# bderembl/msom

Measured on AMD Instinct MI355X. Metric: grid-point-updates/s (timesteps/s x N^2 x nl), multi-layer QG RK2 step at 4096x4096x6 per GPU, higher is better.
Workload: dtype f64; 1 GPU; C4: msqg double gyre (Verron 1992 params), 4096x4096x6 fp64, tiles 1x1 of 4096x4096, TOLERANCE 1e-3, RK2 step = 2 inversions + 2 tendencies + 2 advances; mg_nrelax=4

## Files before the change

include/msom.h:

```cpp
#ifndef MSOM_H
#define MSOM_H

#ifdef __cplusplus
extern "C" {
#endif

#define MSOM_OK 0
#define MSOM_ERR_ARG (-1)
#define MSOM_ERR_IO (-2)
#define MSOM_ERR_CONFIG (-3)
#define MSOM_ERR_HIP (-4)
#define MSOM_ERR_COMM (-5)
#define MSOM_ERR_STATE (-6)

#define MSOM_MAXNL 16
#define MSOM_FASTNL 8

enum {
  MSOM_PSI = 0,
  MSOM_Q = 1,
  MSOM_ZETA = 2,
  MSOM_PSIPG = 3,
  MSOM_ZETAPG = 4,
  MSOM_QFORC = 5,
// ... 89 lines not shown
int msom_modes_energy(msom_t *m, double *ke, double *pe);
int msom_modes_set_rd(msom_t *m, int mode);

int msom_modes_mgstats(msom_t *m, int mode, msom_mgstats *st);

int msom_spec_layout(int nx, int ny, int *nbins, long *count);
int msom_spec_bins(msom_t *m);
int msom_spec_kr(msom_t *m, double *kr);
int msom_spec_2d(msom_t *m, const double *a, const double *b, int layers, double *out);
int msom_spec_cross(msom_t *m, const double *a, const double *b, int layers, double *spec, double *flux);
int msom_spec_fields(msom_t *m, int field_a, int field_b, double *spec, double *flux);
int msom_spec_energy(msom_t *m, double *ke, double *pe);

int msom_step(msom_t *m, double *dt_used);
int msom_set_tnext(msom_t *m, double tnext);
double msom_time(msom_t *m);
int msom_iter(msom_t *m);
double msom_ke(msom_t *m);
int msom_last_mgstats(msom_t *m, msom_mgstats *st);
int msom_run(msom_t *m, const char *workdir, long nsteps_max);

int msom_write_bas(msom_t *m, int field, const char *path);
int msom_read_bas(msom_t *m, int field, const char *path);

int msom_write_nc(msom_t *m, const char *path);
int msom_read_nc(msom_t *m, int field, const char *path, const char *varname, int record);

int msom_wavelet_filter(msom_t *m, double dtflt);
int msom_energy_tend(msom_t *m, double dt);
int msom_filter_de(msom_t *m, int pm_field, double dtflt);
int msom_reset_de(msom_t *m);
int pystep_de(msom_t *m, const double *po_py, int len1, int len2, int len3, double *de_bf_py, int len4, int len5, int len6,
              double *de_vd_py, int len7, int len8, int len9, double *de_j1_py, int len10, int len11, int len12,
              double *de_j2_py, int len13, int len14, int len15, double *de_j3_py, int len16, int len17, int len18,
              double *de_ft_py, int len19, int len20, int len21, int onlyKE);

int msom_dbg_wavelet_levels(msom_t *m);
int msom_dbg_siglev(msom_t *m, int level, double *out);
int msom_dbg_wavelet_apply(msom_t *m, int field);

msom_t *msom_create_newqg(const char *params_path);
msom_t *msom_create_newqg_str(const char *params_text);

int msom_set_device(int device);

int msom_comm_unique_id(void *id128);
msom_t *msom_create_tiled(const char *params_text, int px, int py, int rank, const void *id128);
int msom_tile_info(msom_t *m, int *px, int *py, int *ix, int *iy, int *nx_local, int *ny_local);

int msom_dbg_nlevels(msom_t *m);
int msom_dbg_level_dims(msom_t *m, int lev, int *nx, int *ny);
int msom_dbg_relax(msom_t *m, int lev, double *da, const double *res, int nsweeps);
int msom_dbg_residual(msom_t *m, const double *a, const double *b, double *res, double *maxres);
int msom_dbg_helm_relax(msom_t *m, int lev, double *da, const double *res, int nhalf, const int *count_per_mode);
int msom_dbg_helm_residual(msom_t *m, const double *a, const double *b, double *res, double *maxres_per_mode);
int msom_dbg_restrict(msom_t *m, int lev_fine, const double *fine, double *coarse);
int msom_dbg_prolong(msom_t *m, int lev_coarse, const double *coarse, double *fine);
int msom_dbg_op(msom_t *m, const char *op, int f_in, int f_out, double add, double fac);

int msom_profile_read(msom_t *m, const char *kernel, double *avg_ms, long *launches);
int msom_profile_reset(msom_t *m);
int msom_sync(msom_t *m);
int msom_bench_kernel(msom_t *m, const char *kernel, int reps, double *avg_ms);
int msom_dbg_rccl_selftest(void);

enum {
  MSOMN_PSI = 0,
  MSOMN_Q = 1,
  MSOMN_ZETA = 2,
  MSOMN_TMP = 3,
  MSOMN_PSIPG = 4,
  MSOMN_S2 = 5,
  MSOMN_TOPO = 6,
  MSOMN_QFORC = 7,
  MSOMN_MASK = 8,
  MSOMN_DQ = 9,
  MSOMN_QPRED = 10,
  MSOMN_QFORC3D = 11,
  MSOMN_BS = 12,
  MSOMN_S2S = 13,
  MSOMN_PSIF = 14,
  MSOMN_NFIELDS = 15
};
typedef struct msomn msomn_t;

msomn_t *msomn_create(const char *params_path);
msomn_t *msomn_create_str(const char *params_text);
void msomn_destroy(msomn_t *m);
int msomn_set_option(msomn_t *m, const char *key, double value);
double msomn_get_param(msomn_t *m, const char *key);
int msomn_field_layers(msomn_t *m, int field);
int msomn_set_field(msomn_t *m, int field, const double *a);
int msomn_get_field(msomn_t *m, int field, double *a);
int msomn_set_const(msomn_t *m);
int msomn_update(msomn_t *m, int qfield, int dqfield, double dtmax, double *dt_out);
int msomn_advance(msomn_t *m, int out, int in, int dq, double dt);
int msomn_invert_q(msomn_t *m, int qfield, msom_mgstats *stats);
int msomn_comp_q(msomn_t *m, int psifield, int qfield);
int msomn_rhs_pv(msomn_t *m, int qfield, int dqfield);
int msomn_forcing(msomn_t *m);
int msomn_step(msomn_t *m, int with_forcing_event);
int msomn_set_tnext(msomn_t *m, double tnext);
double msomn_time(msomn_t *m);
double msomn_dt(msomn_t *m);
int msomn_iter(msomn_t *m);
int msomn_ke(msomn_t *m, double *ke);
// ... 25 lines not shown
```

msom_amd/api.py:

```python
import ctypes as C
import os

import numpy as np

_HERE = os.path.dirname(os.path.abspath(__file__))
_LIBDIR = os.path.join(_HERE, "lib")

FIELDS = dict(PSI=0, Q=1, ZETA=2, PSIPG=3, ZETAPG=4, QFORC=5, TMP=6, FR=7, S=8, DQ=9, RO=10, TOPO=11,
              QPRED=12, NOISE=13, SIGMA=14, PTR=15, PTR_RELAX=16, DPTR=17, PTR_PRED=18, RD=19, QOF=20,
              DE_BF=21, DE_VD=22, DE_J1=23, DE_J2=24, DE_J3=25, DE_FT=26, TMP2=27, PO_MFT=28,
              BFN_F1=29, BFN_F2=30, BFN_F3=31, BFN_OBS=32, BFN_GAIN=33)

STATS = dict(PSI=0, Q=1, PSI2=2, Q2=3, KE=4, UQ=5, VQ=6, NACC=7, EKE=16, UQ_EDDY=17, VQ_EDDY=18, QME=32)

MODES = dict(IBU=0, RD=1, M2L=2, L2M=3, N=4)


class MsomError(RuntimeError):
    pass


class MGStats(C.Structure):
    _fields_ = [("i", C.c_int), ("resb", C.c_double), ("resa", C.c_double), ("sum", C.c_double), ("nrelax", C.c_int)]

# ... 31 lines not shown
        "msom_remove_mean": (ci, [vp, ci]),
        "msom_set_const": (ci, [vp]),
        "msom_read_inputs": (ci, [vp, cs]),
        "msom_update": (cd, [vp, vp, vp, cd]),
        "msom_advance": (ci, [vp, vp, vp, vp, cd]),
        "msom_invertq": (ci, [vp, vp, vp, C.POINTER(MGStats)]),
        "msom_comp_q": (ci, [vp, vp, vp]),
        "pystep_bfn": (ci, [vp, vp, ci, ci, ci, vp, ci, ci, ci, cd, ci]),
        "pyq2p": (ci, [vp, vp, ci, ci, ci, vp, ci, ci, ci]),
        "pyp2q": (ci, [vp, vp, ci, ci, ci, vp, ci, ci, ci]),
        "msom_bfn_begin": (ci, [vp]),
        "msom_bfn_steps": (ci, [vp, ci, cd, cd, cd]),
        "msom_bfn_misfit": (ci, [vp, _dp]),
        "msom_stats_begin": (ci, [vp, C.c_uint]),
        "msom_stats_accumulate": (ci, [vp, cd]),
        "msom_stats_weight": (ci, [vp, _dp]),
        "msom_stats_get": (ci, [vp, ci, vp]),
        "msom_time_filter": (ci, [vp, cd]),
        "msom_modes_compute": (ci, [vp]),
        "msom_modes_layers": (ci, [vp, ci]),
        "msom_modes_get": (ci, [vp, ci, vp]),
        "msom_modes_project": (ci, [vp, ci, vp, vp]),
        "msom_modes_energy": (ci, [vp, _dp, _dp]),
        "msom_modes_set_rd": (ci, [vp, ci]),
        "msom_modes_mgstats": (ci, [vp, ci, C.POINTER(MGStats)]),
        "msom_spec_layout": (ci, [ci, ci, C.POINTER(ci), C.POINTER(C.c_long)]),
        "msom_spec_bins": (ci, [vp]),
        "msom_spec_kr": (ci, [vp, _dp]),
        "msom_spec_2d": (ci, [vp, vp, vp, ci, vp]),
        "msom_spec_cross": (ci, [vp, vp, vp, ci, _dp, _dp]),
        "msom_spec_fields": (ci, [vp, ci, ci, _dp, _dp]),
        "msom_spec_energy": (ci, [vp, _dp, _dp]),
        "msom_dbg_helm_relax": (ci, [vp, ci, vp, vp, ci, C.POINTER(ci)]),
        "msom_dbg_helm_residual": (ci, [vp, vp, vp, vp, _dp]),
        "msom_step": (ci, [vp, _dp]),
        "msom_set_tnext": (ci, [vp, cd]),
        "msom_time": (cd, [vp]),
        "msom_iter": (ci, [vp]),
        "msom_ke": (cd, [vp]),
        "msom_last_mgstats": (ci, [vp, C.POINTER(MGStats)]),
        "msom_run": (ci, [vp, cs, C.c_long]),
        "msom_write_bas": (ci, [vp, ci, cs]),
        "msom_read_bas": (ci, [vp, ci, cs]),
        "msom_write_nc": (ci, [vp, cs]),
        "msom_read_nc": (ci, [vp, ci, cs, cs, ci]),
        "msom_set_device": (ci, [ci]),
        "msom_comm_unique_id": (ci, [vp]),
        "msom_create_tiled": (vp, [cs, ci, ci, ci, vp]),
        "msom_tile_info": (ci, [vp] + [C.POINTER(ci)] * 6),
        "msom_dbg_nlevels": (ci, [vp]),
        "msom_dbg_level_dims": (ci, [vp, ci, C.POINTER(ci), C.POINTER(ci)]),
        "msom_dbg_relax": (ci, [vp, ci, vp, vp, ci]),
        "msom_dbg_residual": (ci, [vp, vp, vp, vp, _dp]),
        "msom_dbg_restrict": (ci, [vp, ci, vp, vp]),
        "msom_dbg_prolong": (ci, [vp, ci, vp, vp]),
        "msom_dbg_op": (ci, [vp, cs, ci, ci, cd, cd]),
        "msom_profile_read": (ci, [vp, cs, _dp, C.POINTER(C.c_long)]),
        "msom_profile_reset": (ci, [vp]),
        "msom_sync": (ci, [vp]),
        "msom_bench_kernel": (ci, [vp, cs, ci, _dp]),
        "msom_dbg_rccl_selftest": (ci, []),
        "msom_wavelet_filter": (ci, [vp, cd]),
        "msom_energy_tend": (ci, [vp, cd]),
        "msom_filter_de": (ci, [vp, ci, cd]),
        "msom_reset_de": (ci, [vp]),
        "pystep_de": (ci, [vp] + [vp, ci, ci, ci] * 7 + [ci]),
        "msom_dbg_wavelet_levels": (ci, [vp]),
        "msom_dbg_siglev": (ci, [vp, ci, vp]),
        "msom_dbg_wavelet_apply": (ci, [vp, ci]),
        "msomn_create": (vp, [cs]),
        "msomn_create_str": (vp, [cs]),
        "msomn_destroy": (None, [vp]),
        "msomn_set_option": (ci, [vp, cs, cd]),
        "msomn_get_param": (cd, [vp, cs]),
        "msomn_field_layers": (ci, [vp, ci]),
        "msomn_set_field": (ci, [vp, ci, vp]),
        "msomn_get_field": (ci, [vp, ci, vp]),
        "msomn_set_const": (ci, [vp]),
        "msomn_update": (ci, [vp, ci, ci, cd, _dp]),
        "msomn_advance": (ci, [vp, ci, ci, ci, cd]),
        "msomn_invert_q": (ci, [vp, ci, C.POINTER(MGStats)]),
        "msomn_comp_q": (ci, [vp, ci, ci]),
        "msomn_rhs_pv": (ci, [vp, ci, ci]),
        "msomn_forcing": (ci, [vp]),
        "msomn_step": (ci, [vp, ci]),
        "msomn_set_tnext": (ci, [vp, cd]),
        "msomn_time": (cd, [vp]),
        "msomn_dt": (cd, [vp]),
        "msomn_iter": (ci, [vp]),
        "msomn_ke": (ci, [vp, _dp]),
        "msomn_last_mgstats": (ci, [vp, C.POINTER(MGStats)]),
        "msomn_profile_read": (ci, [vp, cs, _dp, C.POINTER(C.c_long)]),
        "msomn_profile_reset": (ci, [vp]),
        "msomn_diag1d": (ci, [vp, _dp]),
        "msomn_write_nc": (ci, [vp, cs]),
        "msomn_read_nc": (ci, [vp, ci, cs, cs, ci]),
        "msomn_run": (ci, [vp, cs, C.c_long]),
        "msomn_dbg_relax": (ci, [vp, ci, vp, vp, ci]),
        "msomn_dbg_residual": (ci, [vp, vp, vp, vp, _dp]),
        "msomn_dbg_restrict": (ci, [vp, ci, vp, vp]),
        "msomn_dbg_prolong": (ci, [vp, ci, vp, vp]),
        "msomn_dbg_level_mask": (ci, [vp, ci, vp]),
        "msomn_dbg_del2_zeta": (ci, [vp]),
        "msomn_dbg_noise": (ci, [vp, vp, ci, vp]),
        "msomn_dbg_csig": (ci, [vp, ci, vp]),
        "msomn_noise_draw": (ci, [vp, ci]),
# ... 310 lines not shown
        arrs = [_f64(po, (self.nl, self.ny, self.nx))] + [a for a in (bf, vd, j1, j2, j3, ft)]
        args = []
        for a in arrs:
            args += [_ptr(a), self.nl, self.ny, self.nx]
        self._chk(self.L.pystep_de(self.h, *args, int(onlyKE)))

    def wavelet_levels(self):
        n = self.L.msom_dbg_wavelet_levels(self.h)
        if n < 0:
            self._chk(n)
        return n

    def siglev(self, level):
        a = np.empty((1, self.ny >> level, self.nx >> level))
        self._chk(self.L.msom_dbg_siglev(self.h, level, _ptr(a)))
        return a

    def wavelet_apply(self, field):
        self._chk(self.L.msom_dbg_wavelet_apply(self.h, field))

    def write_bas(self, field, path):
        self._chk(self.L.msom_write_bas(self.h, field, path.encode()))

    def read_bas(self, field, path):
        self._chk(self.L.msom_read_bas(self.h, field, path.encode()))

    def write_nc(self, path):
        self._chk(self.L.msom_write_nc(self.h, path.encode()))

    def read_nc(self, field, path, varname, record=-1):
        self._chk(self.L.msom_read_nc(self.h, field, path.encode(), varname.encode(), record))

    def nlevels(self):
        return self.L.msom_dbg_nlevels(self.h)

    def level_dims(self, lev):
        nx, ny = C.c_int(), C.c_int()
        self._chk(self.L.msom_dbg_level_dims(self.h, lev, C.byref(nx), C.byref(ny)))
        return nx.value, ny.value

    def relax(self, lev, da, res, nsweeps=1):
        da = np.array(da, dtype=np.float64, order="C")
        res = _f64(res)
        self._chk(self.L.msom_dbg_relax(self.h, lev, _ptr(da), _ptr(res), nsweeps))
        return da

    def residual(self, a, b):
        a, b = _f64(a), _f64(b)
        res = np.empty_like(a)
        m = C.c_double()
        self._chk(self.L.msom_dbg_residual(self.h, _ptr(a), _ptr(b), _ptr(res), C.byref(m)))
        return res, m.value

    def restrict(self, lev_fine, fine):
        fine = _f64(fine)
        nl, ny, nx = fine.shape
        coarse = np.empty((nl, ny // 2, nx // 2))
        self._chk(self.L.msom_dbg_restrict(self.h, lev_fine, _ptr(fine), _ptr(coarse)))
        return coarse

    def prolong(self, lev_coarse, coarse):
        coarse = _f64(coarse)
        nl, ny, nx = coarse.shape
        fine = np.empty((nl, ny * 2, nx * 2))
        self._chk(self.L.msom_dbg_prolong(self.h, lev_coarse, _ptr(coarse), _ptr(fine)))
        return fine

    def op(self, name, f_in, f_out, add=0.0, fac=1.0):
        self._chk(self.L.msom_dbg_op(self.h, name.encode(), f_in, f_out, add, fac))

    def profile_read(self, kernel):
        ms, n = C.c_double(), C.c_long()
        self._chk(self.L.msom_profile_read(self.h, kernel.encode(), C.byref(ms), C.byref(n)))
        return ms.value, n.value

    def profile_reset(self):
        self._chk(self.L.msom_profile_reset(self.h))

    def sync(self):
        self._chk(self.L.msom_sync(self.h))

    def bench_kernel(self, kernel, reps=20):
        ms = C.c_double()
        self._chk(self.L.msom_bench_kernel(self.h, kernel.encode(), reps, C.byref(ms)))
        return ms.value


class NewQG:

    FIELD_IDS = tuple(FIELDS[k] for k in ("PSI", "Q", "ZETA", "DQ", "QPRED", "QFORC"))

    def __init__(self, params=None, path=None, strict=False):
        self.L = load_library(strict)
        self.h = self.L.msom_create_newqg(path.encode()) if path is not None else self.L.msom_create_newqg_str(params.encode())
        if not self.h:
            raise MsomError(self.L.msom_last_error().decode())
        self.nl = 1
        self.nx, self.ny = int(self.param("nx")), int(self.param("ny"))

    close, __del__, _chk = QG.close, QG.__del__, QG._chk
    param, option = QG.param, QG.option
    set_const = QG.set_const
    update, advance, invertq, comp_q = QG.update, QG.advance, QG.invertq, QG.comp_q
    step, set_tnext, t, iter, ke, mgstats = QG.step, QG.set_tnext, QG.t, QG.iter, QG.ke, QG.mgstats
    write_nc, read_nc = QG.write_nc, QG.read_nc
    profile_read, profile_reset, sync, bench_kernel = QG.profile_read, QG.profile_reset, QG.sync, QG.bench_kernel
# ... 281 lines not shown
```

msom_amd/csrc/kernels.h:

```cpp
#ifndef MSOM_KERNELS_H
#define MSOM_KERNELS_H

#include <stdio.h>
#include <stdlib.h>

#include <type_traits>
#include <utility>

#include "msom_internal.h"
#include "modes_inl.h"

template <int LO, int HI, class F>
static inline bool with_int(int v, F &&f) {
  if constexpr (LO > HI) return false;
  else {
    if (v == LO) { f(std::integral_constant<int, LO>{}); return true; }
    return with_int<LO + 1, HI>(v, std::forward<F>(f));
  }
}
template <class F>
static inline void with_bool(bool b, F &&f) {
  if (b) f(std::true_type{});
  else f(std::false_type{});
}
// ... 56 lines not shown
void launch_bfn_ab3(hipStream_t st, double *q, double *f1, const double *f2, const double *f3, const double *obs, const double *gain,
                    const NatGeom &g, int nl, double dt12, double k);
int bfn_misfit_blocks(const NatGeom &g);
void launch_bfn_misfit(hipStream_t st, const double *q, const double *obs, const double *gain, double *partial, double *out2, const NatGeom &g,
                       int nl);
struct StatsAcc {
  double *s[MSOM_ST_NACC];
};
void launch_stats_acc(hipStream_t st, unsigned mask, const double *psi, const double *q, const StatsAcc &a, const NatGeom &g, int nl,
                      const double *w_dev, double w, double D2, double *W);
void launch_stats_mean(hipStream_t st, double *out, const double *s, const double *W, const NatGeom &g, int nl);
void launch_stats_derive(hipStream_t st, double *out, const double *pm, const double *sa, const double *sq, const double *W, const NatGeom &g,
                         int nl, int which, double D2);
void launch_time_filter(hipStream_t st, double *me, const double *q, const NatGeom &g, int nl, double a);
int partial_count(const NatGeom &g);
void launch_sum_final(hipStream_t st, const double *partial, double *out, int n);
void launch_ke(hipStream_t st, const double *po, double *partial, double *out, const NatGeom &g, double D);
void launch_sum_layers(hipStream_t st, const double *f, double *partial, double *out, const NatGeom &g, int nl);
void launch_sub_layer_const(hipStream_t st, double *f, const double *sums, const NatGeom &g, int nl, double inv_count);
void launch_make_S(hipStream_t st, const double *Fr, const double *Ro, double *S, const NatGeom &g, int nlm);

void launch_noise(hipStream_t st, double *n, const double *sigma, const NatGeom &g, int nl, double amp, unsigned seed, unsigned draw, int gx0,
                  int gy0, int gnx);

void launch_ptr_rhs(hipStream_t st, const double *psi, const double *c, const double *rel, double *dp, const NatGeom &g, int nl, int np,
                    const double *iPe, const double *ptr_ir, double D);

void launch_advection_de(hipStream_t st, const double *zeta, const double *psi, const double *psipg, const double *zetapg, const double *S, double *j1,
                         double *j2, double *j3, const NatGeom &g, int nl, double D, double beta, double dt, double ediag, const LayerCoef &lc);
void launch_dissip_de(hipStream_t st, const double *p4, const double *str, const double *po, double *dq, const NatGeom &g, int nl, double iRe,
                      double iRe4, double dt, double ediag, double D, int stage);
void launch_ekman_de(hipStream_t st, const double *zeta, const double *po, double *dq, const NatGeom &g, int nl, double cs, double cb, double dt,
                     double ediag);
void launch_running_mean(hipStream_t st, double *pm, const double *po, const NatGeom &g, int nl, int n);
void launch_filter_de(hipStream_t st, double *ft, const double *tmp2, double *pm, const NatGeom &g, int nl, double dtflt, double ediag);

struct RhsResid {
  double *res, *res_c;
  double *res_max;
  double *bsum_partial;
  SplitGeom sg, cg;
};
int rhs_fused_blocks(const NatGeom &g);
void launch_rhs_fused(hipStream_t st, const KernelOpts &o, const double *psi, const double *S, const double *qforc, const double *wind, double *dq,
                      double *umax_partial, double *umax_out, const NatGeom &g, int nl, int walls, int uniformS, const double *Su,
                      int have_qforc, double D, double beta, double iRe, double iRe4, double cs, double cb, double slip_c,
                      const LayerCoef &lc, int variant, const double *q_in = nullptr, double *q_out = nullptr, double dt = 0.,
                      const RhsResid *rr = nullptr, int region = 0, const double *dt_ptr = nullptr);
int rhs_pipe_blocks(const NatGeom &g);
void launch_rhs_lpw(hipStream_t st, const KernelOpts &o, const double *psi, const double *S, const double *qforc, const double *wind, double *dq,
                    const NatGeom &g, int nl, int walls, int uniformS, const double *Su, int have_qforc, double D, double beta, double iRe, double iRe4,
                    double cs, double cb, double slip_c, const LayerCoef &lc, const double *q_in, double *q_out, double dt, int stoch = 0,
                    const double *q_stage = nullptr, const double *noise = nullptr, double crelax = 0., double dts = 0., int region = 0,
                    const double *dt_ptr = nullptr);

#define MGC_MAXLEV 8
#define MGC_MAXDIM 32
#define MGC_NT 512
struct CoarseLev { double *da, *res; const double *S; SplitGeom g; RelaxCoef rc; };
struct CoarseArgs { CoarseLev lev[MGC_MAXLEV]; int n, walls, prolong_fused, lds; };
void launch_mg_coarse(hipStream_t st, const CoarseArgs *d_args, int nrelax, int nl, int uniformS, int lean = 0);
size_t mg_coarse_lean_doubles(const CoarseArgs &h, int nl);
#define MGC_POOL 19200
size_t mg_coarse_static_lds();
void launch_nat_to_split(hipStream_t st, const double *nat, const NatGeom &g, double *sp, const SplitGeom &sg, int nl);
void launch_split_to_nat(hipStream_t st, const double *sp, const SplitGeom &sg, double *nat, const NatGeom &g, int nl);
void launch_split_pack(hipStream_t st, const double *src, double *sp, const SplitGeom &sg, int nl, int bc, int walls);
void launch_split_unpack(hipStream_t st, const double *sp, const SplitGeom &sg, double *dst, int nl);
void launch_residual(hipStream_t st, const double *a, const double *b, const double *S, const NatGeom &g, double *res, const SplitGeom &sg,
                     int nl, const RelaxCoef &rc, int uniformS, double *maxres, double *sum_partial, int want_sum);
int residual2_blocks(const NatGeom &g);
void launch_residual2(hipStream_t st, const KernelOpts &o, int mode, const double *a, const double *da, double *a_out, const double *b, const double *S,
                      const NatGeom &g, double *res, const SplitGeom &sg, double *res_c, const SplitGeom &cg, int nl, const RelaxCoef &rc,
                      int uniformS, int walls, double *maxres, double *sum_partial, int want_sum, double *umax_partial, double *umax_out,
                      int umax_clean = 0,
                      double *res_c2 = nullptr, const SplitGeom *cg2 = nullptr);
void launch_restrict(hipStream_t st, const double *fine, const SplitGeom &fg, double *coarse, const SplitGeom &cg, int nl);
void launch_restrict_pyramid(hipStream_t st, const double *fine, double *const *out, const SplitGeom *g, int n, int nl);
void launch_prolong(hipStream_t st, const double *coarse, const SplitGeom &cg, double *fine, const SplitGeom &fg, int nl, int walls);
void launch_relax_color(hipStream_t st, double *da, const double *res, const double *S, const SplitGeom &sg, int nl, const RelaxCoef &rc,
                        int uniformS, int color, int walls, int fine, int region = 0);
void launch_relax_ring(hipStream_t st, double *da, const double *res, const double *S, const SplitGeom &sg, int nl, const RelaxCoef &rc,
                       int uniformS, int color, int walls);
int launch_relax_block8(hipStream_t st, const KernelOpts &o, const double *da_in, const double *coarse, const SplitGeom &cg, const double *res, double *da_out,
                        const SplitGeom &sg, int nl, const RelaxCoef &rc, int walls, int nh, int c0, const double *S = nullptr);
void launch_relax_block2(hipStream_t st, const KernelOpts &o, const double *da_in, const double *coarse, const SplitGeom &cg, const double *res, double *da_out,
                         const SplitGeom &sg, int nl, const RelaxCoef &rc, int walls, int fine);
void launch_relax_red_prolong(hipStream_t st, const KernelOpts &o, double *da, const double *coarse, const SplitGeom &cg, const double *res, const double *S,
                              const SplitGeom &sg, int nl, const RelaxCoef &rc, int uniformS, int walls);
void launch_correct(hipStream_t st, double *a, const NatGeom &g, const double *da, const SplitGeom &sg, int nl, int walls);

struct VisitRingBands { int s0[4], ns[4], c0[4], nc[4], n; };
struct MarchCorrect { const double *psi; double *psi_out; NatGeom g; };
struct MarchHalo { const double *in_s, *in_n, *res_s, *res_n; size_t ls; int rows; };
int launch_relax_march(hipStream_t st, const KernelOpts &o, const double *in, double *out, const double *res, const SplitGeom &sg, int nl, const RelaxCoef &rc, int c1,
                       int K, int walls, int chunk_rows = 0, const MarchHalo *h = nullptr, const double *coarse = nullptr, const SplitGeom *cg = nullptr,
                       const MarchCorrect *mc = nullptr, int more_follow = 0, const MarchHalo *coarse_halo = nullptr, int region = 0,
                       const int *skip = nullptr, int skip_compact = 0);
int launch_relax_visit(hipStream_t st, const KernelOpts &o, double *da, double *da_alt, const double *res, const SplitGeom &sg, int nl, const RelaxCoef &rc,
                       int walls, const double *coarse, const SplitGeom &cg, const MarchCorrect &mc);
bool relax_visit_fits(int nl, const SplitGeom &sg, int rows, int pairs);
extern "C" int msom_visit_ring(int hk, int ny, int march_rows, int visit_rows, int pairs, int corr, int *geom, int *bands);
bool march_lean_fits(int nl, const SplitGeom &sg, const NatGeom *ng);

struct ModeCoef {
  double m2l[MSOM_MAXNL * MSOM_MAXNL], ibu[MSOM_MAXNL];
};
// ... 128 lines not shown
```

msom_amd/csrc/kernels_fused.hip:

```cpp
#include "rhs_inl.h"

#define FTX 64
#define PW (FTX + 6)
#define ZW (FTX + 4)
#define TW (FTX + 2)

struct RhsArgs {
  const double *psi, *S, *qforc, *wind, *q_in;
  double *dq, *umax_partial, *q_out;
  double dt;
  int dbg;
  NatGeom g;
  int nl, walls, uniformS, have_qforc;
  double D, beta, iRe, iRe4, cs, cb, slip_c;
  LayerCoef lc;
  double Su[MSOM_MAXNL];
  double *res, *res_c, *res_max, *bsum_partial;
  SplitGeom sg, cg;
};

__device__ __forceinline__ double lane_next(double v) {
  const long long b = __double_as_longlong(v);
  const int lo = __builtin_amdgcn_update_dpp(0, (int)b, 0x101, 0xf, 0xf, true);
  const int hi = __builtin_amdgcn_update_dpp(0, (int)(b >> 32), 0x101, 0xf, 0xf, true);
// ... 486 lines not shown
  __syncthreads();
  for (int l = 0; l < nl; l++) {
    const double *P0 = sP[l % 3], *P1 = sP[(l + 1) % 3];
    const double *Z = sZ[l & 1], *T = sT[l & 1];
    const bool more = l + 1 < nl;
    if (qdma) asm volatile("s_waitcnt vmcnt(0)" ::: "memory");
    if (qdma && l > 0) q_prefetch(l - 1, 1);
    if (!late) {
      if (l + 2 < nl) fetch(l + 2);
      if (more) lds_lap<ZW, ZH, 2, PW, 3, FNT>(sZ[(l + 1) & 1], P1, bc, x0, y0, nx, ny, a.walls, a.slip_c, D2, rD2);
      if (l + 2 < nl) stash(sP[(l + 2) % 3]);
    }
    centre(l, 0, P0, P1, Z, T);
    if (late) {
      if (l + 2 < nl) fetch(l + 2);
      if (more) lds_lap<ZW, ZH, 2, PW, 3, FNT>(sZ[(l + 1) & 1], P1, bc, x0, y0, nx, ny, a.walls, a.slip_c, D2, rD2);
      if (l + 2 < nl) stash(sP[(l + 2) % 3]);
    }
    __syncthreads();
    if (qdma) {
      asm volatile("s_waitcnt vmcnt(0)" ::: "memory");
      if (more) q_prefetch(l, 0);
    }
    if (!late && more) lds_lap<TW, TH, 1, ZW, 2, FNT>(sT[(l + 1) & 1], sZ[(l + 1) & 1], bc, x0, y0, nx, ny, a.walls, a.slip_c, D2, rD2);
    centre(l, HALF, P0, P1, Z, T);
    if (late && more) lds_lap<TW, TH, 1, ZW, 2, FNT>(sT[(l + 1) & 1], sZ[(l + 1) & 1], bc, x0, y0, nx, ny, a.walls, a.slip_c, D2, rD2);
    __syncthreads();
  }
  if (want_res) {
    double *red = sT[0];
    const double wm = wave_max_f(res_m);
    double ws = res_bs;
    for (int o = 32; o > 0; o >>= 1) ws += __shfl_down(ws, o, 64);
    if (lane == 0) { red[wv] = wm; red[NW + wv] = ws; }
    __syncthreads();
    if (tid == 0) {
      double mm = red[0], ss = red[NW];
      for (int k = 1; k < NW; k++) { mm = fmax(mm, red[k]); ss += red[NW + k]; }
      atomicMax((unsigned long long *)a.res_max, (unsigned long long)__double_as_longlong(mm));
      a.bsum_partial[blockIdx.y * gridDim.x + blockIdx.x] = ss;
    }
  }
}

int rhs_pipe_blocks(const NatGeom &g) { return ((g.nx + FTX - 1) / FTX) * ((g.ny + 31) / 32); }
int rhs_fused_blocks(const NatGeom &g) { return ((g.nx + FTX - 1) / FTX) * ((g.ny + 7) / 8); }

void launch_rhs_fused(hipStream_t st, const KernelOpts &o, const double *psi, const double *S, const double *qforc, const double *wind, double *dq,
                      double *umax_partial, double *umax_out, const NatGeom &g, int nl, int walls, int uniformS, const double *Su,
                      int have_qforc, double D, double beta, double iRe, double iRe4, double cs, double cb, double slip_c,
                      const LayerCoef &lc, int variant, const double *q_in, double *q_out, double dt, const RhsResid *rr, int region, const double *dt_ptr) {
  if (variant == 6) {
    launch_rhs_lpw(st, o, psi, S, qforc, wind, dq, g, nl, walls, uniformS, Su, have_qforc, D, beta, iRe, iRe4, cs, cb, slip_c, lc, q_in, q_out, dt,
                   0, nullptr, nullptr, 0., 0., region, dt_ptr);
    return;
  }
  RhsArgs a;
  a.dbg = o.rhs_dbg;
  a.res = a.res_c = a.res_max = a.bsum_partial = nullptr;
  if (rr && variant == 1 && q_out) {
    a.res = rr->res; a.res_c = rr->res_c; a.res_max = rr->res_max; a.bsum_partial = rr->bsum_partial; a.sg = rr->sg; a.cg = rr->cg;
    (void)hipMemsetAsync(rr->res_max, 0, sizeof(double), st);
  } else {
    a.sg = SplitGeom(); a.cg = SplitGeom();
  }
  a.q_in = q_in; a.q_out = q_out; a.dt = dt;
  a.psi = psi; a.S = S; a.qforc = qforc; a.wind = wind; a.dq = dq; a.umax_partial = umax_partial;
  a.g = g; a.nl = nl; a.walls = walls; a.uniformS = uniformS; a.have_qforc = have_qforc;
  a.D = D; a.beta = beta; a.iRe = iRe; a.iRe4 = iRe4; a.cs = cs; a.cb = cb; a.slip_c = slip_c; a.lc = lc;
  for (int l = 0; l < MSOM_MAXNL; l++) a.Su[l] = Su ? Su[l] : 0.;
  int fty = (variant == 2 || variant == 4) ? 16 : (variant == 3 || variant == 5) ? 8 : 32;
  dim3 gr((g.nx + FTX - 1) / FTX, (g.ny + fty - 1) / fty);
  switch (variant) {
    case 1:
      if (a.res) hipLaunchKernelGGL((k_rhs_fused_pipe<32, 512, true>), gr, dim3(512), 0, st, a);
      else hipLaunchKernelGGL((k_rhs_fused_pipe<32, 512, false>), gr, dim3(512), 0, st, a);
      break;
    case 2: hipLaunchKernelGGL((k_rhs_fused<16, 512, 2>), gr, dim3(512), 0, st, a); break;
    case 3: hipLaunchKernelGGL((k_rhs_fused<8, 256, 2>), gr, dim3(256), 0, st, a); break;
    case 4: hipLaunchKernelGGL((k_rhs_fused<16, 512, 4>), gr, dim3(512), 0, st, a); break;
    case 5: hipLaunchKernelGGL((k_rhs_fused<8, 256, 4>), gr, dim3(256), 0, st, a); break;
    default: hipLaunchKernelGGL((k_rhs_fused<32, 512, 2>), gr, dim3(512), 0, st, a); break;
  }
  if (umax_partial) {
    (void)hipMemsetAsync(umax_out, 0, nl * sizeof(double), st);
    hipLaunchKernelGGL(k_max_final2, dim3(64), dim3(256), 0, st, umax_partial, umax_out, (int)(gr.x * gr.y), nl);
  }
}
```

msom_amd/csrc/kernels_lpw.hip:

```cpp
#include "rhs_inl.h"

#pragma clang fp contract(off)

#define LPW_W 58
#define LPW_R 4
#ifdef MSOM_STRICT
#define LPW_NV 3
#define LPW_MAXW 8
#else
#define LPW_NV 2
#define LPW_MAXW 12
#endif

struct LpwArgs {
  const double *psi, *S, *qforc, *wind, *q_in;
  const double *q_stage, *noise;
  double crelax, dts;
  double *dq, *q_out;
  double dt;
  const double *dt_ptr;
  NatGeom g;
  int nl, walls, uniformS, have_qforc, H, NS;
  int noedge_off;
  int region;
  int dbg;
  double D, beta, iRe, iRe4, cs, cb, slip_c;
  LayerCoef lc;
  double Su[MSOM_MAXNL];
};

template <int R, bool UNI, bool QF, bool ADV, bool STOCH, bool EDGE>
__device__ __forceinline__ void lpw_body(const LpwArgs &a, double (&ring)[2][LPW_MAXW][R][LPW_NV][64]) {
  const int lane = threadIdx.x & 63;
  const int wv = __builtin_amdgcn_readfirstlane((int)(threadIdx.x >> 6));
  const int nl = a.nl, nx = a.g.nx, ny = a.g.ny;
  const int l = wv % nl;
  const ptrdiff_t pitch = a.g.pitch;
  const int strip = blockIdx.x * a.NS + wv / nl, nstrips = (nx + LPW_W - 1) / LPW_W;
  const int x0 = min(strip, nstrips - 1) * LPW_W, y0 = blockIdx.y * a.H, y1 = min(ny, y0 + a.H);
  const int gi = x0 - 3 + lane, gic = min(gi, nx + 2);
  const double dtv = a.dt_ptr ? *a.dt_ptr : a.dt;
  const double D = a.D, D2 = D * D, rD2 = 1. / D2, D12 = 12. * D * D, rD12 = 1. / D12, D2x = 2 * D, rD2x = 1. / D2x;
  const bool lower = l + 1 < nl, upper = l > 0;
  const int lW = ((a.walls & WALL_W) && x0 == 0) ? 2 : -1;
  const int eL = nx - x0 + 3;
  const int lE = ((a.walls & WALL_E) && eL <= 63) ? eL : -1;
  const bool bcx = EDGE && (lW >= 0 || lE >= 0);
  const bool south = (a.walls & WALL_S) != 0, north = (a.walls & WALL_N) != 0;
  const bool slip = a.slip_c > 0.;
  const bool out_ok = lane >= 3 && lane <= 60 && gi < nx && strip < nstrips;
  const double *pP = a.psi + nat_idx(a.g, l, 0, gic);
  const double *pQ = lower ? pP + a.g.ls : pP;
  const double idh0 = a.lc.idh0[l], idh1 = a.lc.idh1[l];
  const double su0 = (nl > 1 && upper) ? a.Su[l - 1] : 0., su1 = (nl > 1 && lower) ? a.Su[l] : 0.;
  const double windv = l == 0 ? a.wind[min(y0 + lane, ny - 1)] : 0.;
  auto wind_row = [&](int j) -> double {
    const long long b = __double_as_longlong(windv);
    const int lo = __builtin_amdgcn_readlane((int)b, j - y0), hi = __builtin_amdgcn_readlane((int)(b >> 32), j - y0);
    return __longlong_as_double(((long long)hi << 32) | (unsigned int)lo);
  };

  double P[5], PL[4], PR[4], Z[4], ZL[4], ZR[4], T[3], TL[2], TR[2], Q[3], QL[3], QR[3];
#pragma unroll
  for (int k = 0; k < 5; k++) P[k] = 0.;
#pragma unroll
  for (int k = 0; k < 4; k++) PL[k] = PR[k] = Z[k] = ZL[k] = ZR[k] = 0.;
#pragma unroll
  for (int k = 0; k < 3; k++) T[k] = Q[k] = QL[k] = QR[k] = 0.;
  TL[0] = TL[1] = TR[0] = TR[1] = 0.;

#ifdef MSOM_STRICT
  double abA[R], jdA[R], lapTA[R], zcA[R], tcA[R];
#else
  double tlA[R];
#endif
  double pnext[R], qnext[R], qreg[R], fqreg[R], qsreg[STOCH ? R : 1], nzreg[STOCH ? R : 1];
#pragma unroll
  for (int r = 0; r < R; r++) {
#ifdef MSOM_STRICT
    abA[r] = jdA[r] = lapTA[r] = zcA[r] = tcA[r] = 0.;
#else
    tlA[r] = 0.;
#endif
    pnext[r] = qnext[r] = qreg[r] = fqreg[r] = 0.;
  }

  auto ld = [&](const double *base, int j) -> double { return base[(ptrdiff_t)((a.dbg & 2) ? y0 : (EDGE ? min(j, ny + 2) : j)) * pitch]; };
#ifdef MSOM_STRICT
  auto lap5 = [&](double c, double w, double e, double n, double s) -> double { return DIVC(e + w + n + s - 4 * c, D2, rD2); };
#else
  auto lap5 = [&](double c, double w, double e, double n, double s) -> double { return fma(-4., c, e + w + n + s) * rD2; };
#endif
  auto xfix = [&](double raw, double so, double sw, double se) -> double {
    if (bcx) {
      if (slip) {
        if (lane == lW) raw = a.slip_c * (se - so);
        if (lane == lE) raw = a.slip_c * (sw - so);
      } else {
        const double re = lane_above(raw), rw = lane_below(raw);
        if (lane == lW) raw = -re;
        if (lane == lE) raw = -rw;
      }
    }
    return raw;
  };
  auto yghost = [&](double dm, double dmw, double dme, double sm, double sg) -> double {
    double v = slip ? a.slip_c * (sm - sg) : -dm;
    if (lane == lW) v = dme;
    if (lane == lE) v = dmw;
    return v;
  };

  auto row = [&](int j, double pnew, double qnew, bool centre, bool yedge, int b, int r) {
#pragma unroll
    for (int k = 0; k < 4; k++) P[k] = P[k + 1];
    P[4] = pnew;
#pragma unroll
    for (int k = 0; k < 3; k++) { PL[k] = PL[k + 1]; PR[k] = PR[k + 1]; Z[k] = Z[k + 1]; ZL[k] = ZL[k + 1]; ZR[k] = ZR[k + 1]; }
    T[0] = T[1]; T[1] = T[2]; TL[0] = TL[1]; TR[0] = TR[1];
#pragma unroll
    for (int k = 0; k < 2; k++) { Q[k] = Q[k + 1]; QL[k] = QL[k + 1]; QR[k] = QR[k + 1]; }
    Q[2] = qnew; QL[2] = lane_below(qnew); QR[2] = lane_above(qnew);
    PL[3] = lane_below(P[3]); PR[3] = lane_above(P[3]);
    double z = xfix(lap5(P[3], PL[3], PR[3], P[4], P[2]), P[3], PL[3], PR[3]);
    if (yedge && north && j + 2 == ny) z = yghost(Z[2], ZL[2], ZR[2], P[2], P[3]);
    Z[3] = z; ZL[3] = lane_below(z); ZR[3] = lane_above(z);
    if (yedge && south && j + 2 == 0) {
      Z[2] = yghost(Z[3], ZL[3], ZR[3], P[3], P[2]);
      ZL[2] = lane_below(Z[2]); ZR[2] = lane_above(Z[2]);
    }
    double t = xfix(lap5(Z[2], ZL[2], ZR[2], Z[3], Z[1]), Z[2], ZL[2], ZR[2]);
    if (yedge && north && j + 1 == ny) t = yghost(T[1], TL[0], TR[0], Z[1], Z[2]);
    T[2] = t; TL[1] = lane_below(t); TR[1] = lane_above(t);
    if (yedge && south && j + 1 == 0) T[1] = yghost(T[2], TL[1], TR[1], Z[2], Z[1]);
    if (!centre) return;

    double p[3][3], zz[3][3], p1[3][3];
#pragma unroll
    for (int k = 0; k < 3; k++) {
      p[k][0] = PL[k]; p[k][1] = P[k]; p[k][2] = PR[k];
      zz[k][0] = ZL[k]; zz[k][1] = Z[k]; zz[k][2] = ZR[k];
      p1[k][0] = QL[k]; p1[k][1] = Q[k]; p1[k][2] = QR[k];
    }
    const double adv = (STOCH && l == 0) ? 0. : mjac9(p, zz, D12, rD12);
    const double be = DIVC(a.beta * (p[1][0] - p[1][2]), D2x, rD2x);
    const double jd = (lower && !STOCH) ? mjac9(p, p1, D12, rD12) : 0.;
    const double zc = Z[1], tc = T[1];
    const double lapT = lap5(tc, TL[0], TR[0], T[2], T[0]);
#ifdef MSOM_STRICT
    abA[r] = adv + be; jdA[r] = jd; lapTA[r] = lapT; zcA[r] = zc; tcA[r] = tc;
    ring[b][wv][r][0][lane] = zc;
    ring[b][wv][r][1][lane] = tc;
    ring[b][wv][r][2][lane] = jd;
#else
    double tl = fma(tc, a.iRe, fma(a.iRe4, lapT, adv + be));
    if (l == 0) tl -= fma(a.cs, zc, wind_row(j));
    if (l == nl - 1) tl = fma(-a.cb, zc, tl);
    tlA[r] = tl;
    ring[b][wv][r][0][lane] = fma(a.iRe, zc, a.iRe4 * tc);
    ring[b][wv][r][1][lane] = jd;
#endif
  };

  auto finish = [&](int j, int b, int r, double s0, double s1, double fq) -> double {
#ifdef MSOM_STRICT
    const double zc = zcA[r], tc = tcA[r];
    double zm = 0., tm = 0., zp = 0., tp = 0., ju = 0.;
    if (upper) { zm = ring[b][wv - 1][r][0][lane]; tm = ring[b][wv - 1][r][1][lane]; ju = -ring[b][wv - 1][r][2][lane]; }
    if (lower) { zp = ring[b][wv + 1][r][0][lane]; tp = ring[b][wv + 1][r][1][lane]; }
    double t = abA[r];
    if (nl > 1) {
      if (upper) t = t + s0 * ju * idh0;
      if (lower) t = t + s1 * jdA[r] * idh1;
    }
    t = 0. + t;
    double dq = t;
    auto stretch = [&](double fac, double pm, double pc, double pp) -> double {
      if (l == 0) return fac * s1 * (pp - pc) * idh1;
      if (l < nl - 1) return fac * (s0 * (pm - pc) * idh0 + s1 * (pp - pc) * idh1);
      return fac * s0 * (pm - pc) * idh0;
    };
    if (a.iRe != 0.) {
      if (nl > 1) dq = 1. * dq + stretch(a.iRe, zm, zc, zp);
      dq += tc * a.iRe;
    }
    if (a.iRe4 != 0.) {
      if (nl > 1) dq = 1. * dq + stretch(a.iRe4, tm, tc, tp);
      dq = 1. * dq + a.iRe4 * lapTA[r];
    }
    if (l == 0) dq -= a.cs * zc;
    if (l == nl - 1) dq -= a.cb * zc;
    if (l == 0) dq -= wind_row(j);
#else
    double dq = tlA[r];
    const double xc = ring[b][wv][r][0][lane];
    if (nl > 1) {
      if (upper) dq = fma(s0 * idh0, (ring[b][wv - 1][r][0][lane] - xc) - ring[b][wv - 1][r][1][lane], dq);
      if (lower) dq = fma(s1 * idh1, (ring[b][wv + 1][r][0][lane] - xc) + ring[b][wv][r][1][lane], dq);
    }
#endif
    if (QF) dq += fq;
#ifdef MSOM_STRICT
    if (STOCH) return (qreg[r] + qsreg[r] * a.crelax + nzreg[r] * a.dts) + dq * a.dt;
    return ADV ? qreg[r] + dq * dtv : dq;
#else
    if (STOCH) return fma(dq, a.dt, fma(nzreg[r], a.dts, fma(qsreg[r], a.crelax, qreg[r])));
    return ADV ? fma(dq, dtv, qreg[r]) : dq;
#endif
  };

#pragma unroll
  for (int r = 0; r < R; r++) {
    pnext[r] = ld(pP, y0 + r + 3);
    qnext[r] = ld(pQ, y0 + r + 1);
  }
  {
    double wp[6], wq[2];
#pragma unroll
    for (int k = 0; k < 6; k++) wp[k] = ld(pP, y0 - 3 + k);
    wq[0] = ld(pQ, y0 - 1); wq[1] = ld(pQ, y0);
#pragma unroll
    for (int k = 0; k < 6; k++) row(y0 - 6 + k, wp[k], k >= 4 ? wq[k - 4] : 0., false, EDGE, 0, 0);
  }

  double *const outp = ADV ? a.q_out : a.dq;
  const int nblk = (y1 - y0 + R - 1) / R;
  __builtin_amdgcn_s_waitcnt(0x0F70);
  for (int k = 0; k <= nblk; k++) {
    const int b = k & 1;
    if (k > 0) {
      const int jb = y0 + (k - 1) * R;
      double s0[R], s1[R], val[R];
#pragma unroll
      for (int r = 0; r < R; r++) {
        s0[r] = su0; s1[r] = su1;
        if (!UNI && nl > 1) {
          const size_t c = nat_idx(a.g, l, min(jb + r, ny - 1), gic);
          if (upper) s0[r] = a.S[c - a.g.ls];
          if (lower) s1[r] = a.S[c];
        }
      }
#pragma unroll
      for (int r = 0; r < R; r++) {
        val[r] = finish(jb + r, b ^ 1, r, s0[r], s1[r], fqreg[r]);
        asm volatile("" : "+v"(val[r]));
      }
#pragma unroll
      for (int r = 0; r < R; r++)
        if (out_ok && jb + r < y1 && !(a.dbg & 1)) outp[nat_idx(a.g, l, jb + r, gic)] = val[r];
    }
    if (k < nblk) {
      const int j0 = y0 + k * R;
      const bool yedge = EDGE && j0 + R + 2 > ny;
#pragma unroll
      for (int r = 0; r < R; r++) {
        const size_t c = nat_idx(a.g, l, (a.dbg & 2) ? y0 : (EDGE ? min(j0 + r, ny - 1) : j0 + r), gic);
        if (ADV) qreg[r] = a.q_in[c];
        if (QF) fqreg[r] = a.qforc[c];
        if (STOCH) { qsreg[r] = a.q_stage[c]; nzreg[r] = a.noise[c]; }
      }
#pragma unroll
      for (int r = 0; r < R; r++) {
        const int j = j0 + r;
        double pn, qn;
        asm volatile("v_mov_b64 %0, %1" : "=v"(pn) : "v"(pnext[r]));
        asm volatile("v_mov_b64 %0, %1" : "=v"(qn) : "v"(qnext[r]));
        pnext[r] = ld(pP, j + R + 3);
        qnext[r] = ld(pQ, j + R + 1);
        row(j, pn, qn, true, yedge, b, r);
      }
    }
    __syncthreads();
  }
}

template <int R, bool UNI, bool QF, bool ADV, bool STOCH = false>
__global__ void __launch_bounds__(64 * LPW_MAXW) k_rhs_lpw(LpwArgs a) {
  __shared__ double ring[2][LPW_MAXW][R][LPW_NV][64];
  const int wv = __builtin_amdgcn_readfirstlane((int)(threadIdx.x >> 6));
  const int nx = a.g.nx, ny = a.g.ny;
  const int strip = blockIdx.x * a.NS + wv / a.nl, nstrips = (nx + LPW_W - 1) / LPW_W;
  const int x0 = min(strip, nstrips - 1) * LPW_W, y0 = blockIdx.y * a.H, y1 = min(ny, y0 + a.H);
  const bool xwall = ((a.walls & WALL_W) && x0 == 0) || ((a.walls & WALL_E) && nx - x0 + 3 <= 63);
  const int nblk = (y1 - y0 + R - 1) / R;
  const bool ywall = y0 == 0 || y0 + nblk * R + R > ny;
  if (a.region) {
    const bool inner = strip < nstrips && x0 - 3 >= 0 && x0 + 60 < nx && y0 - 3 >= 0 && y0 + nblk * R + R + 2 < ny;
    if ((a.region == 1) != inner) return;
  }
  if (xwall || ywall || a.noedge_off) lpw_body<R, UNI, QF, ADV, STOCH, true>(a, ring);
  else lpw_body<R, UNI, QF, ADV, STOCH, false>(a, ring);
}

void launch_rhs_lpw(hipStream_t st, const KernelOpts &o, const double *psi, const double *S, const double *qforc, const double *wind, double *dq,
                    const NatGeom &g, int nl, int walls, int uniformS, const double *Su, int have_qforc, double D, double beta, double iRe, double iRe4,
                    double cs, double cb, double slip_c, const LayerCoef &lc, const double *q_in, double *q_out, double dt, int stoch,
                    const double *q_stage, const double *noise, double crelax, double dts, int region, const double *dt_ptr) {
  LpwArgs a;
  a.region = region;
  a.dt_ptr = dt_ptr;
  a.q_stage = q_stage; a.noise = noise; a.crelax = crelax; a.dts = dts;
  a.psi = psi; a.S = S; a.qforc = qforc; a.wind = wind; a.q_in = q_in; a.dq = dq; a.q_out = q_out; a.dt = dt;
  a.dbg = o.lpw_dbg & 3;
  a.noedge_off = (o.lpw_dbg & 4) != 0;
  a.g = g; a.nl = nl; a.walls = walls; a.uniformS = uniformS; a.have_qforc = have_qforc;
  a.D = D; a.beta = beta; a.iRe = iRe; a.iRe4 = iRe4; a.cs = cs; a.cb = cb; a.slip_c = slip_c; a.lc = lc;
  for (int l = 0; l < MSOM_MAXNL; l++) a.Su[l] = Su ? Su[l] : 0.;
  const int strips = (g.nx + LPW_W - 1) / LPW_W;
  int H = o.rhs_dbg >> 8;
  a.NS = LPW_MAXW / nl < 1 ? 1 : LPW_MAXW / nl;
  if (a.NS > strips) a.NS = strips;
  if (H <= 0) {
    const int ncu = device_cu_count();
    const int wgx = (strips + a.NS - 1) / a.NS;
    double best = -1.;
    for (int h = 64; h >= 8; h -= 8) {
      const double r = (double)wgx * ((g.ny + h - 1) / h) / ncu, cost = (r <= 3. ? ceil(r) : r + 0.5) * (h + 6);
      if (best < 0. || cost < best) { best = cost; H = h; }
    }
  }
  if (H < 8) H = 8;
  a.H = H;
  const dim3 gr((strips + a.NS - 1) / a.NS, (g.ny + H - 1) / H), bl(64 * nl * a.NS);
  if (stoch && !q_out) {
    fprintf(stderr, "msom: launch_rhs_lpw: stochastic variant needs q_out\n");
    abort();
  }
  with_bool(uniformS, [&](auto U) {
    with_bool(have_qforc, [&](auto Q) {
      constexpr bool UNI = decltype(U)::value, QF = decltype(Q)::value;
      if (stoch) hipLaunchKernelGGL((k_rhs_lpw<LPW_R, UNI, QF, true, true>), gr, bl, 0, st, a);
      else if (q_out) hipLaunchKernelGGL((k_rhs_lpw<LPW_R, UNI, QF, true>), gr, bl, 0, st, a);
      else hipLaunchKernelGGL((k_rhs_lpw<LPW_R, UNI, QF, false>), gr, bl, 0, st, a);
    });
  });
}
```

msom_amd/csrc/msom_api.hip:

```cpp
#include <math.h>
#include <stdio.h>
#include <stdlib.h>
#include <string.h>
#include <sys/stat.h>
#include <sys/types.h>
#include <time.h>

#include <algorithm>
#include <cmath>
#include <string>
#include <utility>
#include <functional>
#include <map>
#include <vector>

#include "comm.h"
#include "kernels.h"
#include "spec_inl.h"
#include "helm_inl.h"

#define HIPCHK(x)                                                                          \
  do {                                                                                     \
    hipError_t e__ = (x);                                                                  \
    if (e__ != hipSuccess) {                                                               \
      msom_set_error("HIP error %s at %s:%d (%s)", hipGetErrorString(e__), __FILE__, __LINE__, #x); \
      return MSOM_ERR_HIP;                                                                 \
    }                                                                                      \
  } while (0)

enum { SC_BSUM = 2, SC_KE = 3, SC_SCRATCH = 4, SC_RES0 = 6, SC_RES1 = 7, SC_UMAX = 8 , SC_RESF = 8 + MSOM_MAXNL , SC_LSUM = 32 , SC_SPEC = 48 , SC_COUNT = 64 };
static_assert(SC_RESF < SC_LSUM && SC_LSUM + MSOM_MAXNL <= SC_SPEC && SC_SPEC + 4 <= SC_COUNT, "scalar slots overlap");

#define MARCH_HALO 4
struct ProfSlot {
  std::vector<hipEvent_t> ev;
  size_t used = 0;
  double total_ms = 0;
  long launches = 0;
};

struct msom {
  Params p;
  std::string params_text;
  int px = 1, py = 1, ix = 0, iy = 0, rank = 0, nranks = 1;
  int gnx = 0, gny = 0;
  int nx = 0, ny = 0;
  int walls = WALL_ALL;
  Comm *comm = nullptr;
  int sticky = MSOM_OK;
  int comm_hold = 0;
  int dbg_nosync = 0;
  KernelOpts opt;
  int async_solve = 1;
  int step_sync = -1;
  std::function<void(const std::function<void()> &)> spec_hook;
  int spec_launched = 0, spec_valid = 0;
  hipEvent_t ev_spec = nullptr;
  double *h_pub = nullptr, *d_pub = nullptr;
  long pub_seq = 0;
  double *q_alt = nullptr;
  double *adv_out_override = nullptr;
  const double *dt_dev = nullptr;
  int nb[8];
  int nl = 1, nlm = 1;
  int bc = BC_DIRICHLET0;
  double dhf[MSOM_MAXARR], dhc[MSOM_MAXARR];
  LayerCoef lc;
  NatGeom g;
  double *f[MSOM_NFIELDS];
  int flayers[MSOM_NFIELDS];
  int fbc[MSOM_NFIELDS];
  int nlev = 0;
  std::vector<SplitGeom> sg;
  std::vector<double *> da, da_alt, res, S;
  std::vector<double *> mh_da_s, mh_da_n, mh_res_s, mh_res_n;
  std::vector<RelaxCoef> rc;
  size_t max_split = 0;
  int agg_level = -1, agglomerate = 1, agg_size = 256;
  int mg_global_sum = 0;
  std::vector<SplitGeom> gsg;
  std::vector<double *> gda, gda_alt, gres;
  double *agg_send = nullptr, *agg_recv = nullptr;
  double *staging = nullptr;
  double *partial = nullptr;
  double *partial_rr = nullptr;
  double *partial_umax = nullptr;
  double *d_scal = nullptr, *h_scal = nullptr;
  double *d_wind = nullptr;
  double umax_pg[MSOM_MAXNL];
  int umax_ready = 0;
  hipStream_t st = nullptr;
  hipStream_t st2 = nullptr;
  hipEvent_t ev_c2x = nullptr, ev_x2c = nullptr;
  int overlap = 1;
  int const_set = 0, flag_topo = 0, have_pg = 0, have_zpg = 0, have_qforc = 0;
  int fr_uniform = 1, uniformS = 0, uniform_opt = -1 ;
  int stochastic = 0, corrector_step = 0, noise_mode = 0, stoch_fused = 1;
  int prolong_fused = 1;
  int block_sweeps = 0;
  int restrict_pyr = 1;
  int restrict2 = 1;
  int block8 = 1;
  int block8_max = 1024;
  int block_small = 0;
  int march = 1;
  int march_k = 4;
  int use_graph = 0;
  std::map<long, hipGraphExec_t> cyc_graph;
  int march_partial = 1;
  int march_min_tiled = 22;
  int march_min = 23;
  int march_correct = 1;
  int corr_req = 0, corr_done = 0;
  int march_visit = 1;
  int march_visit_min = 25;
  int march_prolong = 1;
  int mg_fused = 1;
  double *psi_alt = nullptr;
  int rhs_variant = 6;
  int fused = 1;
  unsigned seed = 1, noise_draw = 0;
  int quiet = 0;
  int wv_nlev = 0, wv_ready = 0;
  int wv_kt = 0, wv_gx = 0, wv_gy = 0;
  std::vector<std::vector<double>> wv_top_sig;
  double *wv_gsend = nullptr, *wv_grecv = nullptr;
  int nme_ft = 0;
  CoarseArgs *d_cargs = nullptr;
  int mgc_dim = MGC_MAXDIM;
  int mgc_pfused = 1;
  int umax_clean = 0;
  int mgc_first = -1, mgc_opt = 4;
  int mgc_lean = 0;
  int res_ready = -1;
  int adv_fused = 1;
  int rhs_resid = 0;
  int bfn_begun = 0;
  int bfn_obs_set = 0, bfn_gain_set = 0;
  double *bfn_partial = nullptr;
  unsigned stats_mask = 0;
  StatsAcc stats = {};
  double *stats_W = nullptr;
  double *stats_qme = nullptr;
  int stats_on = 0, stats_every = 1;
  long stats_count = 0;
  long stats_ndev = 0;
  double tau_f = 20;
  int modes_ready = 0;
  int modes_compact = 0;
  int modes_compact_opt = -1;
  ModeCoef modes_mc = {};
  double *modes_md = nullptr;
  double *modes_dev = nullptr;
  int *modes_flag = nullptr;
  double *modes_partial = nullptr;
  int mode_pv_invert = 0;
  std::vector<double *> helm_ibu;
  double *helm_pm = nullptr, *helm_qm = nullptr;
  double *helm_scal = nullptr;
  double *helm_partial = nullptr;
  HelmSolve helm = {};
  int helm_solved = 0;
  ProfSlot prof_helm_relax, prof_helm_resid, prof_helm_coarse;
  int spc_batch = 0;
  int spc_smax = 0;
  double2 *spc_z = nullptr, *spc_zt = nullptr;
  double2 *spc_tw = nullptr;
  double *spc_v = nullptr;
  double *spc_te = nullptr, *spc_res = nullptr;
  double *spc_hin = nullptr;
  double *spc_o2d = nullptr;
  size_t spc_bytes = 0;
  std::vector<long> spc_count;
  int s_zero = 0;
  std::vector<NatGeom> wv_g;
  std::vector<double *> wv_s, wv_r, wv_sig;
  int model = 0;
  NewqgParams nq = {};
  int nq_fused = 1;
  int nq_adv_fused = 1;
  int nq_rows = 0;
  double t = 0, dt = 1., tnext = HUGE_VAL, previous = 0;
  int iter = 0;
  msom_mgstats mg = {0, 0, 0, 0, 0};
  int profile = 0;
  ProfSlot prof_sweep, prof_resid, prof_block, prof_march[5];
  ProfSlot prof_march_pl;
  ProfSlot prof_march_visit;
  ProfSlot prof_march_corr, prof_resmax;
// ... 270 lines not shown
    HIPCHK(hipDeviceGetStreamPriorityRange(&lo, &hi));
    HIPCHK(hipStreamCreateWithPriority(&m->st2, hipStreamNonBlocking, hi));
    HIPCHK(hipEventCreateWithFlags(&m->ev_c2x, hipEventDisableTiming));
    HIPCHK(hipEventCreateWithFlags(&m->ev_x2c, hipEventDisableTiming));
  }
  m->g = make_nat(m->nx, m->ny);
  for (int k = 0; k < MSOM_NFIELDS; k++) {
    m->f[k] = nullptr;
    m->flayers[k] = m->nl;
    m->fbc[k] = m->bc;
  }
  m->flayers[MSOM_FR] = m->flayers[MSOM_S] = m->nlm;
  m->flayers[MSOM_RO] = m->flayers[MSOM_TOPO] = 1;
  m->fbc[MSOM_FR] = m->fbc[MSOM_S] = m->fbc[MSOM_RO] = m->fbc[MSOM_TOPO] = m->bc == BC_PERIODIC ? BC_PERIODIC : BC_NEUMANN;
  if (m->bc == BC_PERIODIC) m->fbc[MSOM_PSIPG] = BC_DIRICHLET_LIN;
  for (int k = MSOM_PTR; k <= MSOM_PTR_PRED; k++) {
    m->flayers[k] = m->nl * (m->p.nptr > 0 ? m->p.nptr : 1);
    m->fbc[k] = m->bc == BC_PERIODIC ? BC_PERIODIC : BC_NEUMANN;
  }
  m->flayers[MSOM_RD] = 1;
  m->fbc[MSOM_RD] = m->bc == BC_PERIODIC ? BC_PERIODIC : BC_NEUMANN;
  for (int k = 0; k < MSOM_NFIELDS; k++) {
    if (k == MSOM_NOISE || k == MSOM_SIGMA || k == MSOM_QOF || k >= MSOM_DE_BF) continue;
    if (k >= MSOM_PTR && k <= MSOM_PTR_PRED && m->p.nptr <= 0) continue;
    if (m->model && !nq_has_field(k)) continue;
    size_t bytes = m->g.ls * m->flayers[k] * sizeof(double);
    HIPCHK(hipMalloc(&m->f[k], bytes));
    HIPCHK(hipMemsetAsync(m->f[k], 0, bytes, m->st));
  }
  int n = 0;
  while ((m->nx >> n) >= 2 && (m->ny >> n) >= 2 && ((m->nx >> n) << n) == m->nx && ((m->ny >> n) << n) == m->ny) n++;
  if (m->p.mglevels > 0 && m->p.mglevels < n) n = m->p.mglevels;
  m->nlev = n;
  m->sg.resize(n); m->da.resize(n); m->da_alt.resize(n); m->res.resize(n); m->S.resize(n); m->rc.resize(n);
  for (int k = 0; k < n; k++) {
    m->sg[k] = make_split(m->nx >> k, m->ny >> k);
    size_t bytes = m->sg[k].ls * m->nl * sizeof(double);
    HIPCHK(hipMalloc(&m->da[k], bytes));
    HIPCHK(hipMalloc(&m->res[k], bytes));
    HIPCHK(hipMemsetAsync(m->da[k], 0, bytes, m->st));
    HIPCHK(hipMemsetAsync(m->res[k], 0, bytes, m->st));
    if (m->model) continue;
    HIPCHK(hipMalloc(&m->da_alt[k], bytes));
    HIPCHK(hipMemsetAsync(m->da_alt[k], 0, bytes, m->st));
    HIPCHK(hipMalloc(&m->S[k], m->sg[k].ls * m->nlm * sizeof(double)));
    HIPCHK(hipMemsetAsync(m->S[k], 0, m->sg[k].ls * m->nlm * sizeof(double), m->st));
  }
  if (!m->model) {
    HIPCHK(hipMalloc(&m->psi_alt, m->g.ls * m->nl * sizeof(double)));
    HIPCHK(hipMemsetAsync(m->psi_alt, 0, m->g.ls * m->nl * sizeof(double), m->st));
  }
  HIPCHK(hipMalloc(&m->staging, (size_t)m->nl * (m->p.nptr > 1 ? m->p.nptr : 1) * m->nx * m->ny * sizeof(double)));
  HIPCHK(hipMalloc(&m->partial, ((size_t)partial_count(m->g) * m->nl + 64) * sizeof(double)));
  HIPCHK(hipMalloc(&m->partial_rr, ((size_t)rhs_pipe_blocks(m->g) + 64) * sizeof(double)));
  {
    size_t nb = (size_t)rhs_fused_blocks(m->g);
    if (nb < 2048) nb = 2048;
    HIPCHK(hipMalloc(&m->partial_umax, nb * MSOM_MAXNL * sizeof(double)));
  }
  HIPCHK(hipMalloc(&m->d_scal, SC_COUNT * sizeof(double)));
  HIPCHK(hipMemsetAsync(m->d_scal, 0, SC_COUNT * sizeof(double), m->st));
  HIPCHK(hipHostMalloc(&m->h_scal, SC_COUNT * sizeof(double)));
  HIPCHK(hipMalloc(&m->d_wind, (size_t)m->ny * sizeof(double)));
  return MSOM_OK;
}

static int set_vars(msom *m) {
  const Params &p = m->p;
  for (int l = 0; l < m->nl; l++) m->dhf[l] = p.dhu[l];
  std::vector<double> h((size_t)m->nl * m->nx * m->ny);
  const double D = p.L0 / m->gnx;
  for (int l = 0; l < m->nlm; l++)
    for (size_t k = 0; k < (size_t)m->nx * m->ny; k++) h[(size_t)l * m->nx * m->ny + k] = l < m->nl - 1 ? p.Frm[l] : 0.;
  int r = msom_set_field(m, MSOM_FR, h.data());
  if (r) return r;
  m->fr_uniform = 1;
  m->have_pg = 0;
  for (int l = 0; l < m->nl; l++) {
    if (p.upg[l] != 0 || p.vpg[l] != 0) m->have_pg = 1;
    for (int j = 0; j < m->ny; j++)
      for (int i = 0; i < m->nx; i++) {
        const double x = (m->ix * m->nx + i + 0.5) * D, y = (m->iy * m->ny + j + 0.5) * D;
        h[((size_t)l * m->ny + j) * m->nx + i] = p.vpg[l] * x - p.upg[l] * y;
      }
  }
  int hp = m->have_pg;
  r = msom_set_field(m, MSOM_PSIPG, h.data());
  if (r) return r;
  m->have_pg = hp;
  for (size_t k = 0; k < (size_t)m->nx * m->ny; k++) h[k] = p.Rom;
  r = msom_set_field(m, MSOM_RO, h.data());
  if (r) return r;
  for (size_t k = 0; k < (size_t)m->nx * m->ny; k++) h[k] = 1.;
  r = msom_set_field(m, MSOM_RD, h.data());
  m->fr_uniform = 1;
  return r;
}

static int nq_alloc(msom *m);
static msom *create_common(const Params &p0, int px, int py, int rank, const void *id128, const NewqgParams *nq = nullptr) {
  Params p = p0;
  if (p.Ny <= 0) p.Ny = p.N;
  msom_params_derive(&p);
  if (p.nl < 1 || p.nl > MSOM_MAXNL) {
    msom_set_error("nl = %d outside the supported range 1..%d", p.nl, MSOM_MAXNL);
    return nullptr;
  }
// ... 90 lines not shown
  for (size_t k = 0; k < m->wv_sig.size(); k++) {
    if (k == 0) { if (m->wv_gsend) hipFree(m->wv_gsend); if (m->wv_grecv) hipFree(m->wv_grecv); }
    if (k > 0 && m->wv_s[k]) hipFree(m->wv_s[k]);
    if (k > 0 && m->wv_r[k]) hipFree(m->wv_r[k]);
    if (m->wv_sig[k]) hipFree(m->wv_sig[k]);
  }
  if (m->psi_alt) hipFree(m->psi_alt);
  if (m->q_alt) hipFree(m->q_alt);
  if (m->ev_spec) hipEventDestroy(m->ev_spec);
  if (m->h_pub) hipHostFree(m->h_pub);
  if (m->staging) hipFree(m->staging);
  if (m->partial) hipFree(m->partial);
  if (m->partial_rr) hipFree(m->partial_rr);
  if (m->bfn_partial) hipFree(m->bfn_partial);
  stats_drop(m);
  modes_drop(m);
  spec_drop(m);
  if (m->modes_dev) hipFree(m->modes_dev);
  if (m->modes_flag) hipFree(m->modes_flag);
  if (m->modes_partial) hipFree(m->modes_partial);
  for (double *p : {m->helm_pm, m->helm_qm, m->helm_scal, m->helm_partial})
    if (p) hipFree(p);
  if (m->d_cargs) hipFree(m->d_cargs);
  if (m->partial_umax) hipFree(m->partial_umax);
  if (m->d_scal) hipFree(m->d_scal);
  if (m->h_scal) hipHostFree(m->h_scal);
  if (m->d_wind) hipFree(m->d_wind);
  for (auto *ps : {&m->prof_sweep, &m->prof_resid, &m->prof_block, &m->prof_march[2], &m->prof_march[3], &m->prof_march[4], &m->prof_rhs, &m->prof_redprol, &m->prof_rescorr, &m->prof_respre, &m->prof_march_pl, &m->prof_march_corr, &m->prof_march_visit, &m->prof_resmax, &m->prof_helm_relax, &m->prof_helm_resid, &m->prof_helm_coarse})
    for (auto e : ps->ev) hipEventDestroy(e);
  if (m->comm) comm_destroy(m->comm);
  if (m->ev_c2x) hipEventDestroy(m->ev_c2x);
  if (m->ev_x2c) hipEventDestroy(m->ev_x2c);
  if (m->st2) hipStreamDestroy(m->st2);
  if (m->st) hipStreamDestroy(m->st);
  delete m;
  return MSOM_OK;
}

static int build_coefs(msom *m);
static void free_agglomeration(msom *m);

static void clear_graphs(msom *m);
static int *kernel_opt(KernelOpts &o, const char *key) {
#define KOPT(f) {#f, &KernelOpts::f}
  static const struct { const char *key; int KernelOpts::*f; } keys[] = {
      KOPT(march_rows), KOPT(march_xcd), KOPT(march_flip), KOPT(march_dbg), KOPT(march_lean), KOPT(march_dma),
      KOPT(march_visit_rows), KOPT(march_visit_pairs), KOPT(march_visit_ring), KOPT(march_visit_split), KOPT(resmax_rows), KOPT(block_variant), KOPT(rhs_dbg), KOPT(lpw_dbg)};
#undef KOPT
  for (const auto &k : keys)
    if (!strcmp(key, k.key)) return &(o.*k.f);
  return nullptr;
}
extern "C" int msom_set_option(msom_t *m, const char *key, double v) {
  if (!m || !key) return MSOM_ERR_ARG;
  if (m->model) return nq_set_option(m, key, v);
  clear_graphs(m);
  if (!strcmp(key, "graph")) { m->use_graph = (int)v; return MSOM_OK; }
  if (!strcmp(key, "TOLERANCE")) m->p.tolerance = v;
  else if (!strcmp(key, "NITERMAX")) m->p.nitermax = (int)v;
  else if (!strcmp(key, "NITERMIN")) m->p.nitermin = (int)v;
  else if (!strcmp(key, "DT")) m->p.DT = v;
  else if (!strcmp(key, "flag_topo")) m->flag_topo = (int)v;
  else if (!strcmp(key, "quiet")) m->quiet = (int)v;
  else if (!strcmp(key, "uniform_S")) {
    m->uniform_opt = (int)v;
    if (m->const_set) return build_coefs(m);
  }
  else if (!strcmp(key, "profile")) m->profile = (int)v;
  else if (!strcmp(key, "fused")) m->fused = (int)v;
  else if (!strcmp(key, "mg_fused")) m->mg_fused = (int)v;
  else if (!strcmp(key, "march")) m->march = (int)v;
  else if (!strcmp(key, "march_min")) m->march_min = (int)v;
  else if (!strcmp(key, "march_min_tiled")) m->march_min_tiled = (int)v;
  else if (!strcmp(key, "march_partial")) m->march_partial = (int)v;
  else if (!strcmp(key, "march_prolong")) m->march_prolong = (int)v;
  else if (!strcmp(key, "march_correct")) m->march_correct = (int)v;
  else if (!strcmp(key, "march_visit")) m->march_visit = (int)v;
  else if (!strcmp(key, "march_visit_min")) m->march_visit_min = (int)v;
  else if (!strcmp(key, "dbg_nosync")) m->dbg_nosync = (int)v;
  else if (!strcmp(key, "async_solve")) m->async_solve = (int)v;
  else if (!strcmp(key, "step_sync")) m->step_sync = (int)v;
  else if (!strcmp(key, "march_k")) m->march_k = (int)v < 2 ? 2 : ((int)v > 4 ? 4 : (int)v);
  else if (!strcmp(key, "block_small")) m->block_small = (int)v;
  else if (!strcmp(key, "block8")) m->block8 = (int)v;
  else if (!strcmp(key, "restrict2")) m->restrict2 = (int)v;
  else if (!strcmp(key, "restrict_pyr")) m->restrict_pyr = (int)v;
  else if (!strcmp(key, "block8_max")) m->block8_max = (int)v;
  else if (!strcmp(key, "block_sweeps")) { m->block_sweeps = (int)v; if (m->const_set) return build_coefs(m); }
  else if (!strcmp(key, "mg_global_sum")) m->mg_global_sum = (int)v;
  else if (!strcmp(key, "agglomerate")) { m->agglomerate = (int)v; if (m->const_set) return build_coefs(m); }
  else if (!strcmp(key, "agg_size")) { m->agg_size = (int)v; if (m->const_set) return build_coefs(m); }
  else if (!strcmp(key, "prolong_fused")) { m->prolong_fused = (int)v; if (m->const_set) return build_coefs(m); }
  else if (!strcmp(key, "mg_coarse")) { m->mgc_opt = (int)v; if (m->const_set) return build_coefs(m); }
  else if (!strcmp(key, "mgc_pfused")) { m->mgc_pfused = (int)v; if (m->const_set) return build_coefs(m); }
  else if (!strcmp(key, "mg_coarse_dim")) { m->mgc_dim = (int)v; if (m->const_set) return build_coefs(m); }
  else if (int *o = kernel_opt(m->opt, key)) *o = (int)v;
  else if (!strcmp(key, "rhs_variant")) m->rhs_variant = (int)v;
  else if (!strcmp(key, "adv_fused")) m->adv_fused = (int)v;
  else if (!strcmp(key, "overlap")) m->overlap = (int)v;
  else if (!strcmp(key, "rhs_resid")) { m->rhs_resid = (int)v; m->res_ready = -1; }
  else if (!strcmp(key, "seed")) { m->seed = (unsigned)v; srand(m->seed); }
  else if (!strcmp(key, "noise_mode")) m->noise_mode = (int)v;
  else if (!strcmp(key, "stoch_fused")) m->stoch_fused = (int)v;
  else if (!strcmp(key, "stats")) {
    if ((int)v && !m->stats_mask) { msom_set_error("option stats = 1 before msom_stats_begin"); return MSOM_ERR_STATE; }
    m->stats_on = (int)v != 0;
  }
  else if (!strcmp(key, "stats_every")) {
    if (!(v >= 1)) { msom_set_error("option stats_every = %g", v); return MSOM_ERR_ARG; }
    m->stats_every = (int)v;
  }
  else if (!strcmp(key, "tau_f")) {
    if (!(v > 0) || !std::isfinite(v)) { msom_set_error("option tau_f = %g", v); return MSOM_ERR_ARG; }
    m->tau_f = v;
  }
  else if (!strcmp(key, "modes_compact")) {
    if ((int)v != -1 && (int)v != 0) { msom_set_error("option modes_compact = %g (-1 or 0)", v); return MSOM_ERR_ARG; }
    m->modes_compact_opt = (int)v;
  }
  else if (!strcmp(key, "mode_pv_invert")) {
    if ((int)v != 0 && (int)v != 1) { msom_set_error("option mode_pv_invert = %g (0 or 1)", v); return MSOM_ERR_ARG; }
    if ((int)v && m->nranks > 1) {
      msom_set_error("option mode_pv_invert: the modal inversion runs on a single tile, this handle is one of %d", m->nranks);
      return MSOM_ERR_CONFIG;
    }
    m->mode_pv_invert = (int)v;
    m->res_ready = -1;
  }
  else if (!strcmp(key, "stochastic")) {
    m->stochastic = (int)v;
    if (m->stochastic && !m->f[MSOM_NOISE]) {
      for (int k : {MSOM_NOISE, MSOM_SIGMA}) {
        size_t bytes = m->g.ls * m->nl * sizeof(double);
        HIPCHK(hipMalloc(&m->f[k], bytes));
        HIPCHK(hipMemsetAsync(m->f[k], 0, bytes, m->st));
      }
    }
  } else {
    msom_set_error("unknown option %s", key);
    return MSOM_ERR_ARG;
  }
  return MSOM_OK;
}

static int march_levels(const msom *m);
static int march_kmax(const msom *m);
static bool march_lean_fine(const msom *m);
static bool fine_visit_fused(const msom *m);
static int level_path(const msom *m, int k);
static bool restrict2_ok(const msom *m);
extern "C" double msom_get_param(msom_t *m, const char *key) {
  if (!m || !key) return NAN;
  if (!strcmp(key, "model")) return m->model;
  if (m->model) return nq_get_param(m, key);
  const Params &p = m->p;
  if (!strcmp(key, "N") || !strcmp(key, "nx")) return m->gnx;
  if (!strcmp(key, "ny")) return m->gny;
  if (!strcmp(key, "nl")) return m->nl;
  if (!strcmp(key, "nptr")) return p.nptr;
  if (!strcmp(key, "L0")) return p.L0;
  if (!strcmp(key, "DT")) return p.DT;
  if (!strcmp(key, "iRe")) return p.iRe;
  if (!strcmp(key, "iRe4")) return p.iRe4;
  if (!strcmp(key, "CFL")) return p.CFL;
  if (!strcmp(key, "Rom")) return p.Rom;
  if (!strcmp(key, "tend")) return p.tend;
  if (!strcmp(key, "dtout")) return p.dtout;
  if (!strcmp(key, "beta")) return p.beta;
  if (!strcmp(key, "tau0")) return p.tau0;
  if (!strcmp(key, "Ekb")) return p.Ekb;
  if (!strcmp(key, "Eks")) return p.Eks;
  if (!strcmp(key, "sbc")) return p.sbc;
  if (!strcmp(key, "TOLERANCE")) return p.tolerance;
  if (!strcmp(key, "nlevels")) return m->nlev;
  if (!strcmp(key, "uniform_S")) return m->uniformS;
  if (!strcmp(key, "agg_level")) return m->agg_level;
  if (!strcmp(key, "overlap")) return m->overlap;
  if (!strcmp(key, "stats_mask")) return m->stats_mask;
  if (!strcmp(key, "stats_dev_samples")) return (double)m->stats_ndev;
  if (!strcmp(key, "stats_bytes")) {
    int n = m->stats_qme ? 1 : 0;
    for (int k = 0; k < MSOM_ST_NACC; k++) n += m->stats.s[k] ? 1 : 0;
    return (double)n * m->nl * m->nx * m->ny * sizeof(double);
  }
  if (!strcmp(key, "mode_pv_invert")) return m->mode_pv_invert;
  if (!strcmp(key, "modes_ready")) return m->const_set && m->modes_ready;
  if (!strcmp(key, "modes_compact")) return m->const_set && m->modes_ready ? m->modes_compact : (m->modes_compact_opt != 0 && m->fr_uniform);
  if (!strcmp(key, "spec_bytes")) return (double)m->spc_bytes;
  if (!strcmp(key, "spec_batch")) return m->spc_batch;
  if (!strcmp(key, "modes_bytes"))
    return m->modes_md ? (double)(m->nl * m->nl + m->nl) * m->nx * m->ny * sizeof(double) : 0.;
  if (!strcmp(key, "resmax_marching")) return m->uniformS && m->nl <= MSOM_FASTNL && m->g.nx >= 64 && m->g.ny >= 16 && m->opt.resmax_rows >= 0;
  if (!strcmp(key, "march_visit_ring")) return !fine_visit_fused(m) ? -1 : (m->opt.march_visit_ring >= 2 ? 2 : (m->opt.march_visit_ring == 1 ? 1 : 0));
  if (const int *o = kernel_opt(m->opt, key)) return *o;
  if (!strcmp(key, "restrict2")) return restrict2_ok(m);
  if (!strcmp(key, "mg_coarse_lean")) return m->mgc_first >= 0 && m->mgc_lean;
  if (!strcmp(key, "march_levels")) return march_levels(m);
  if (!strcmp(key, "march_min")) return m->march_min;
  if (!strcmp(key, "march_kmax")) return march_kmax(m);
  if (!strcmp(key, "march_lean_fine")) return march_lean_fine(m);
  if (!strcmp(key, "march_visit")) return fine_visit_fused(m);
  if (!strncmp(key, "relax_path_", 11)) { const int k = atoi(key + 11); return k >= 0 && k < m->nlev ? level_path(m, k) : NAN; }
  if (!strcmp(key, "split_ls")) return m->nlev > 0 ? (double)m->sg[0].ls : NAN;
  auto idx = [](const char *s, int n) { const int k = atoi(s); return k >= 0 && k < n ? k : -1; };
  if (!strncmp(key, "idh0_", 5)) { const int k = idx(key + 5, MSOM_MAXNL); return k < 0 ? NAN : m->lc.idh0[k]; }
  if (!strncmp(key, "idh1_", 5)) { const int k = idx(key + 5, MSOM_MAXNL); return k < 0 ? NAN : m->lc.idh1[k]; }
  if (!strncmp(key, "Fr_", 3)) { const int k = idx(key + 3, MSOM_MAXARR); return k < 0 ? NAN : p.Frm[k]; }
  if (!strncmp(key, "dh_", 3)) { const int k = idx(key + 3, MSOM_MAXARR); return k < 0 ? NAN : m->dhf[k]; }
  return NAN;
}


static int check_field(msom *m, int field) {
  if (!m || field < 0 || field >= MSOM_NFIELDS || !m->f[field]) {
    msom_set_error("bad field id %d", field);
    return MSOM_ERR_ARG;
  }
  return MSOM_OK;
}

static int fill_bc(msom *m, int field) {
  if (m->nranks > 1 && field != MSOM_Q && field != MSOM_DQ && field != MSOM_QPRED && field != MSOM_NOISE && field != MSOM_SIGMA &&
      !(field >= MSOM_BFN_F1 && field <= MSOM_BFN_GAIN)) {
    int r = exch_nat(m, m->f[field], m->flayers[field], m->fbc[field], 1);
    if (!r && m->fbc[field] == BC_DIRICHLET_LIN) {
      const int sides = (m->ix == 0 ? WALL_W : 0) | (m->ix == m->px - 1 ? WALL_E : 0) | (m->iy == 0 ? WALL_S : 0) | (m->iy == m->py - 1 ? WALL_N : 0);
      launch_fill_lin_dirichlet(m->st, m->f[field], m->g, m->flayers[field], m->p.upg, m->p.vpg, m->p.L0 / m->gnx, m->p.L0,
                                m->p.L0 * m->gny / m->gnx, m->ix * m->nx, m->iy * m->ny, sides);
    }
    return r;
  }
  if (m->fbc[field] == BC_PERIODIC) launch_fill_periodic(m->st, m->f[field], m->g, m->flayers[field], 1);
  else if (m->fbc[field] == BC_DIRICHLET_LIN)
    launch_fill_lin_dirichlet(m->st, m->f[field], m->g, m->flayers[field], m->p.upg, m->p.vpg, m->p.L0 / m->gnx, m->p.L0,
                              m->p.L0 * m->gny / m->gnx);
  else launch_fill_ghost(m->st, m->f[field], m->g, m->flayers[field], m->fbc[field], m->walls);
  return MSOM_OK;
}

static int upload(msom *m, int field, const double *a) {
  m->res_ready = -1;
  const size_t n = (size_t)m->flayers[field] * m->nx * m->ny;
  HIPCHK(hipMemcpyAsync(m->staging, a, n * sizeof(double), hipMemcpyDefault, m->st));
  launch_pack(m->st, m->staging, m->f[field], m->g, m->flayers[field]);
  fill_bc(m, field);
  return MSOM_OK;
}
// ... 170 lines not shown
  memset(&m->lc, 0, sizeof m->lc);
  for (int l = 0; l < nl - 1; l++) m->dhc[l] = 0.5 * (m->dhf[l] + m->dhf[l + 1]);
  if (nl > 1) {
    m->lc.idh0[0] = 0.;
    m->lc.idh1[0] = 1. / (m->dhc[0] * m->dhf[0]);
    for (int l = 1; l < nl - 1; l++) {
      m->lc.idh0[l] = 1. / (m->dhc[l - 1] * m->dhf[l]);
      m->lc.idh1[l] = 1. / (m->dhc[l] * m->dhf[l]);
    }
    m->lc.idh0[nl - 1] = 1. / (m->dhc[nl - 2] * m->dhf[nl - 1]);
    m->lc.idh1[nl - 1] = 0.;
  }
  const double D = p.L0 / m->gnx;
  if (p.varRo > 0) {
    std::vector<double> h((size_t)m->nx * m->ny);
    for (int j = 0; j < m->ny; j++) {
      const double y = (m->iy * m->ny + j + 0.5) * D;
      for (int i = 0; i < m->nx; i++) h[(size_t)j * m->nx + i] = p.Rom / (1 + p.Rom * p.beta * (y - 0.5 * p.L0));
    }
    int r = upload(m, MSOM_RO, h.data());
    if (r) return r;
    m->fr_uniform = 0;
  }
  launch_make_S(m->st, m->f[MSOM_FR], m->f[MSOM_RO], m->f[MSOM_S], m->g, m->nlm);
  if (m->s_zero) HIPCHK(hipMemsetAsync(m->f[MSOM_S], 0, m->g.ls * m->nlm * sizeof(double), m->st));
  fill_bc(m, MSOM_S);
  launch_nat_to_split(m->st, m->f[MSOM_S], m->g, m->S[0], m->sg[0], m->nlm);
  for (int k = 1; k < m->nlev; k++) launch_restrict(m->st, m->S[k - 1], m->sg[k - 1], m->S[k], m->sg[k], m->nlm);
#ifdef MSOM_STRICT
  const int auto_uniform = 0;
#else
  const int auto_uniform = 1;
#endif
  m->uniformS = (m->uniform_opt < 0 ? auto_uniform : m->uniform_opt) && m->fr_uniform && nl > 1;
  for (int k = 0; k < m->nlev; k++) make_relax_coef(m, k);
  {
    int r = setup_agglomeration(m);
    if (r) return r;
    if ((r = setup_mg_coarse(m))) return r;
  }
  {
    std::vector<double> w(m->ny);
    for (int j = 0; j < m->ny; j++) {
      const double y = (m->iy * m->ny + j + 0.5) * D;
      w[j] = p.tau0 / (p.Rom * m->dhf[0]) * sin(2 * M_PI * y / p.L0) * sin(M_PI * y / p.L0);
    }
    HIPCHK(hipMemcpyAsync(m->d_wind, w.data(), m->ny * sizeof(double), hipMemcpyHostToDevice, m->st));
    HIPCHK(hipStreamSynchronize(m->st));
  }
  return MSOM_OK;
}

extern "C" int msom_set_const(msom_t *m) {
  if (!m) return MSOM_ERR_ARG;
  if (m->model) return nq_set_const(m);
  m->s_zero = 0;
  int rr = build_coefs(m);
  if (rr) return rr;
  m->wv_ready = 0;
  const Params &p = m->p;
  const int nl = m->nl;
  const double D = p.L0 / m->gnx;
  launch_del2(m->st, m->f[MSOM_PSI], m->f[MSOM_Q], m->g, nl, 0., 1., D);
  launch_stretch(m->st, m->f[MSOM_PSI], m->f[MSOM_Q], m->f[MSOM_S], m->g, nl, 1., 1., m->lc);
  fill_bc(m, MSOM_Q);
  if (p.flsrv == 1) {
    launch_del2(m->st, m->f[MSOM_PSIPG], m->f[MSOM_ZETAPG], m->g, nl, 0., 1., D);
    fill_bc(m, MSOM_ZETAPG);
    m->have_zpg = 1;
  }
  for (int l = 0; l < MSOM_MAXNL; l++) m->umax_pg[l] = 0.;
  if (m->have_pg) {
    launch_umax(m->st, m->f[MSOM_PSIPG], m->partial_umax, m->d_scal + SC_UMAX, m->g, nl, D);
    int r = reduce_scal(m, SC_UMAX, nl, RED_MAX);
    if (r) return r;
    for (int l = 0; l < nl; l++) m->umax_pg[l] = m->h_scal[SC_UMAX + l];
  }
  m->const_set = 1;
  m->bfn_begun = 0;
  stats_drop(m);
  modes_drop(m);
  spec_drop(m);
  m->helm_solved = 0;
  if (m->helm_pm) HIPCHK(hipMemsetAsync(m->helm_pm, 0, m->g.ls * nl * sizeof(double), m->st));
  if (m->mode_pv_invert) {
    if ((rr = msom_modes_compute(m))) return rr;
    if (nl > 1 && (rr = msom_modes_set_rd(m, 1))) return rr;
  }
  return sync_stream(m);
}


struct Lev {
  double **da, **da_alt;
  double *res;
  const double *S;
  const SplitGeom *sg;
  const RelaxCoef *rc;
  int walls;
  bool tiled;
  bool fine;
  int k;
};
static Lev tile_lev(const msom *m, int k) {
  return Lev{const_cast<double **>(&m->da[k]), const_cast<double **>(&m->da_alt[k]), m->res[k], m->S[k], &m->sg[k], &m->rc[k], m->walls, m->nranks > 1, k == 0, k};
}
static Lev glob_lev(const msom *m, int k) {
  const int q = k - m->agg_level;
  return Lev{const_cast<double **>(&m->gda[q]), const_cast<double **>(&m->gda_alt[q]), m->gres[q], nullptr, &m->gsg[q], &m->rc[k], m->bc == BC_PERIODIC ? WALL_PER : WALL_ALL, false, false, -1};
}

enum { RP_COLOUR = 0, RP_BLOCK2 = 1, RP_BLOCK8 = 2, RP_MARCH = 3, RP_COARSE = 4, RP_GATHERED = 8 };
static bool layered_fusions(const msom *m) { return !m->mode_pv_invert; }
static int sweep_path(const msom *m, const Lev &L) {
  const SplitGeom &g = *L.sg;
  if (!layered_fusions(m)) return RP_COLOUR;
  if (m->march && !m->block_sweeps && (m->uniformS || m->nl == 1) && m->nl <= MSOM_FASTNL && g.nx >= 512 && g.ny >= 64 &&
      (L.tiled || L.walls == WALL_ALL || (L.walls == WALL_PER && L.k >= 0)) &&
      (m->march >= 2 || (size_t)g.nx * g.ny * m->nl >= ((size_t)1 << (L.tiled ? m->march_min_tiled : m->march_min))))
    return RP_MARCH;
  if (m->block8 && !m->block_sweeps && (m->uniformS || m->nl == 1 || L.S) && m->nl <= MSOM_FASTNL && !L.tiled && g.nx >= 64 && g.ny >= 16 &&
      g.nx <= m->block8_max && (L.walls == WALL_ALL || (L.walls == WALL_PER && L.k >= 0 && g.ny >= 64)))
    return RP_BLOCK8;
  if ((m->block_sweeps || (m->block_small && g.nx <= m->block_small)) && m->uniformS && m->nl <= MSOM_FASTNL && !L.tiled &&
      !(m->walls & WALL_PER) && g.nx >= 64 && g.ny >= 16)
    return RP_BLOCK2;
  return RP_COLOUR;
}
static int level_path(const msom *m, int k) {
  if (m->mgc_first >= 0 && k >= m->mgc_first) return RP_COARSE;
  if (m->agg_level >= 0 && k >= m->agg_level) return RP_GATHERED + sweep_path(m, glob_lev(m, k));
  return sweep_path(m, tile_lev(m, k));
}
static int march_levels(const msom *m) {
  int n = 0;
  for (int k = 0; k < m->nlev; k++) n += level_path(m, k) == RP_MARCH;
  return n;
}
static bool march_lean_fine(const msom *m) {
  return m->nlev > 0 && m->opt.march_lean && level_path(m, 0) == RP_MARCH && march_lean_fits(m->nl, m->sg[0], &m->g);
}
static bool fuse_prolong(const msom *m, const Lev &L, int nrelax) {
  const int path = sweep_path(m, L);
  if (path == RP_BLOCK2 && nrelax >= 2) return true;
  if (path == RP_BLOCK8 && nrelax >= 1) return true;
  return m->prolong_fused && m->nl <= MSOM_FASTNL && nrelax >= 1 && L.sg->nx >= 4 && L.sg->ny >= 4;
}
static bool corr_wanted(const msom *m) { return m->mg_fused && m->nlev > 1 && m->march_correct; }

static int march_kmax(const msom *m) { return m->nl >= 7 && m->march_k > 3 ? 3 : m->march_k; }

enum { MA_DONE, MA_VISIT, MA_PL, MA_REDPROL, MA_PASS, MA_HALF };
struct MarchAct { int kind, K; bool corr, partial; };
static MarchAct march_next(const msom *m, const Lev &L, const Lev *coarse, int n, bool corr_req) {
  const int kmax = march_kmax(m), nl = m->nl;
  const bool deep = L.tiled || (L.walls & WALL_PER);
  auto pass = [&](int kind, int kmin, bool corr_ok) {
    int K = n < kmax ? n : kmax;
    if (n - K == 1 && K > kmin) K--;
    return MarchAct{kind, K, corr_ok && n == K, m->march_partial && n - K >= 1};
  };
  if (coarse && n > 0) {
    const bool pl_tiled = coarse->k >= 0 && nl <= 6 && m->march_prolong >= 1 && coarse->sg->nx >= 2 * MARCH_HALO && coarse->sg->ny >= 2 * MARCH_HALO;
    if (n < 3 || kmax < 3 || !m->march_prolong || (deep && !pl_tiled)) return MarchAct{MA_REDPROL, 1, false, false};
    if (n == 8 && kmax == 4 && L.fine && corr_req && m->march_visit && m->opt.march_dma && m->uniformS && nl >= 2 && m->march_partial &&
        (m->march_visit >= 2 || (size_t)L.sg->nx * L.sg->ny * nl >= ((size_t)1 << m->march_visit_min)) && !L.tiled && L.walls == WALL_ALL &&
// ... 257 lines not shown
static bool restrict2_ok(const msom *m) { return m->restrict2 && m->mg_fused && m->nlev > 2 && m->g.ny % 4 == 0 && m->sg[0].hk % 2 == 0; }
static void residual2(msom *m, int mode, const double *b, int slot, int want_sum) {
  ProfSlot &which = (mode & 8) ? m->prof_resmax : (mode & 1) ? m->prof_rescorr : m->prof_respre;
  if (m->profile) { prof_begin(m, m->prof_resid); prof_begin(m, which); }
  const bool r2 = (mode & 4) && restrict2_ok(m);
  launch_residual2(m->st, m->opt, mode, m->f[MSOM_PSI], m->da[0], m->psi_alt, b, m->f[MSOM_S], m->g, m->res[0], m->sg[0],
                   m->nlev > 1 ? m->res[1] : nullptr, m->sg[m->nlev > 1 ? 1 : 0], m->nl, m->rc[0], m->uniformS, m->walls, m->d_scal + slot,
                   m->partial, want_sum, m->partial_umax, m->d_scal + SC_UMAX, m->umax_clean, r2 ? m->res[2] : nullptr, r2 ? &m->sg[2] : nullptr);
  if (mode & (1 | 8)) m->umax_clean = 0;
  if (m->profile) { prof_end(m, m->prof_resid); prof_end(m, which); }
}

static int read_residuals(msom *m) {
  if (m->nranks == 1) {
    if (m->dbg_nosync) return MSOM_OK;
    if (m->spec_launched) {
      volatile long *seq = reinterpret_cast<volatile long *>(m->h_pub + SC_COUNT);
      const double t0 = wall_seconds();
      while (*seq != m->pub_seq) {
        if (wall_seconds() - t0 > 5.) {
          HIPCHK(hipStreamSynchronize(m->st));
          if (*seq != m->pub_seq) { msom_set_error("the device did not publish the solver's scalars"); return MSOM_ERR_HIP; }
        }
      }
      __atomic_thread_fence(__ATOMIC_ACQUIRE);
      memcpy(m->h_scal, m->h_pub, SC_COUNT * sizeof(double));
      return MSOM_OK;
    }
    HIPCHK(hipMemcpyAsync(m->h_scal, m->d_scal, SC_COUNT * sizeof(double), hipMemcpyDeviceToHost, m->st));
    HIPCHK(hipStreamSynchronize(m->st));
    return MSOM_OK;
  }
  int r = reduce_scal(m, SC_RES0, 2 + m->nl, RED_MAX);
  if (r) return r;
  if (m->nranks > 1 && !m->mg_global_sum) {
    HIPCHK(hipMemcpyAsync(m->h_scal + SC_BSUM, m->d_scal + SC_BSUM, sizeof(double), hipMemcpyDeviceToHost, m->st));
    HIPCHK(hipStreamSynchronize(m->st));
    return MSOM_OK;
  }
  return reduce_scal(m, SC_BSUM, 1, RED_SUM);
}

static int mg_solve(msom *m, const double *b, msom_mgstats *s) {
  const Params &p = m->p;
  const bool fused = m->mg_fused && m->nlev > 1;
  s->i = 0; s->nrelax = 4;
  HIPCHK(hipMemsetAsync(m->d_scal, 0, (SC_UMAX + MSOM_MAXNL) * sizeof(double), m->st));
  m->umax_clean = 1;
  m->umax_ready = 0;
  const bool have_res = fused && m->res_ready >= 0 && b == m->f[m->res_ready];
  m->res_ready = -1;
  if (have_res) {
    HIPCHK(hipMemcpyAsync(m->d_scal + SC_RES0, m->d_scal + SC_RESF, sizeof(double), hipMemcpyDeviceToDevice, m->st));
    launch_sum_final(m->st, m->partial_rr, m->d_scal + SC_BSUM, rhs_pipe_blocks(m->g));
  } else if (fused) {
    residual2(m, 2 | 4, b, SC_RES0, 1);
    launch_sum_final(m->st, m->partial, m->d_scal + SC_BSUM, residual2_blocks(m->g));
  } else {
    residual(m, m->f[MSOM_PSI], b, SC_RES0, 1);
    launch_sum_final(m->st, m->partial, m->d_scal + SC_BSUM, partial_count(m->g));
  }
  bool have_first = false;
  double resb = 0;
  if (p.nitermin < 1) {
    int rr = read_residuals(m);
    if (rr) return rr;
    resb = s->resb = s->resa = m->h_scal[SC_RES0];
    s->sum = m->h_scal[SC_BSUM];
    have_first = true;
  }
  for (s->i = 0; s->i < p.nitermax && (s->i < p.nitermin || s->resa > p.tolerance); s->i++) {
    m->corr_req = corr_wanted(m);
    m->corr_done = 0;
    mg_cycle(m, s->nrelax, fused ? ((restrict2_ok(m) && !(have_res && s->i == 0)) ? 3 : 2) : 1);
    m->corr_req = 0;
    if (s->i > 0) HIPCHK(hipMemsetAsync(m->d_scal + SC_RES1, 0, sizeof(double), m->st));
    if (m->corr_done) {
      std::swap(m->f[MSOM_PSI], m->psi_alt);
      if (m->nranks > 1) STICKY(m, exch_nat(m, m->f[MSOM_PSI], m->nl, m->bc, 1));
      else if (m->bc == BC_PERIODIC) launch_fill_periodic(m->st, m->f[MSOM_PSI], m->g, m->nl, 1);
      else launch_fill_ghost(m->st, m->f[MSOM_PSI], m->g, m->nl, m->bc, m->walls);
      residual2(m, 8, b, SC_RES1, 0);
      m->umax_ready = 1;
    } else if (fused) {
      residual2(m, 1, b, SC_RES1, 0);
      std::swap(m->f[MSOM_PSI], m->psi_alt);
      m->umax_ready = 1;
      if (m->nranks > 1) STICKY(m, exch_nat(m, m->f[MSOM_PSI], m->nl, m->bc, 1));
    } else {
      launch_correct(m->st, m->f[MSOM_PSI], m->g, m->da[0], m->sg[0], m->nl, m->walls);
      if (m->nranks > 1) STICKY(m, exch_nat(m, m->f[MSOM_PSI], m->nl, m->bc, 1));
      residual(m, m->f[MSOM_PSI], b, SC_RES1, 0);
    }
    if (s->i == 0 && m->spec_hook && m->umax_ready && m->nranks == 1) {
      m->spec_hook([&]() {});
      m->spec_launched = 1;
    }
    int rr = read_residuals(m);
    if (rr) { m->spec_launched = 0; return rr; }
    if (m->spec_launched) {
      const double ra = m->h_scal[SC_RES1];
      m->spec_valid = !(s->i + 1 < p.nitermax && (s->i + 1 < p.nitermin || ra > p.tolerance));
      m->spec_launched = 0;
    }
    if (!have_first) {
      resb = s->resb = m->h_scal[SC_RES0];
      s->sum = m->h_scal[SC_BSUM];
// ... 169 lines not shown
  int r = helm_ensure(m);
  if (r) return r;
  m->res_ready = -1;
  m->umax_ready = 0;
  m->spec_valid = 0;
  if ((r = helm_project(m, q, m->helm_qm, 1))) return r;
  if ((r = helm_run(m, m->helm_pm, m->helm_qm))) return r;
  m->helm_solved = 1;
  if ((r = helm_project(m, m->helm_pm, m->f[MSOM_PSI], 0))) return r;
  fill_bc(m, MSOM_PSI);
  return m->sticky;
}

static int invertq(msom *m, const double *q) {
  if (m->mode_pv_invert) return helm_solve(m, q);
  return mg_solve(m, q, &m->mg);
}


static double limiter(msom *m, double umax, double dtmax) {
  const double D = m->p.L0 / m->gnx;
  dtmax /= m->p.CFL;
  if (umax != 0.) {
    const double dt = D / umax;
    if (dt < dtmax) dtmax = dt;
  }
  dtmax *= m->p.CFL;
  if (dtmax > m->previous) dtmax = (m->previous + 0.1 * dtmax) / 1.1;
  m->previous = dtmax;
  return dtmax;
}

static void comp_del2(msom *m, int in, int out, double add, double fac) {
  const double D = m->p.L0 / m->gnx;
  launch_del2(m->st, m->f[in], m->f[out], m->g, m->nl, add, fac, D);
  fill_bc(m, out);
  if (m->p.sbc > 0) launch_slip_bc(m->st, m->f[in], m->f[out], m->g, m->nl, m->p.sbc / ((0.5 * m->p.sbc + 1) * D * D), m->walls);
}
static void comp_stretch(msom *m, int in, int out, double add, double fac) {
  launch_stretch(m->st, m->f[in], m->f[out], m->f[MSOM_S], m->g, m->nl, add, fac, m->lc);
  fill_bc(m, out);
}

static int stoch_prepare(msom *m, double dt, double *dts);
static int rhs_terms(msom *m, int qfield, int dqfield, int with_qforcing, double iRe, double iRe4, double Eks, double Ekb, int adv_out = -1,
                     int adv_in = -1, double adv_dt = 0., int *advanced = nullptr) {
  if (advanced) *advanced = 0;
  const Params &p = m->p;
  const double D = p.L0 / m->gnx;
  const int nl = m->nl;
#ifdef MSOM_STRICT
  const bool stoch_fused = false;
#else
  const bool stoch_fused = m->stochastic && m->stoch_fused && m->adv_fused && adv_out >= 0 && m->rhs_variant == 6 && !m->rhs_resid;
#endif
  if (m->fused && m->nl <= MSOM_FASTNL && !m->have_pg && !m->have_zpg && !m->flag_topo && (!m->stochastic || stoch_fused) &&
      (m->nranks == 1 || (m->nx >= 4 && m->ny >= 4))) {
    if (m->bc == BC_PERIODIC && m->nranks == 1) launch_fill_periodic(m->st, m->f[MSOM_PSI], m->g, nl, 3);
    if (!m->adv_fused) adv_out = -1;
    const int variant = (m->rhs_resid && m->rhs_variant == 6) ? 1 : m->rhs_variant;
    const bool use_rr = adv_out >= 0 && layered_fusions(m) && m->rhs_resid && variant == 1 && m->mg_fused && m->nlev > 1 && m->bc != BC_PERIODIC;
    RhsResid rr;
    if (use_rr) {
      rr.res = m->res[0]; rr.res_c = m->res[1]; rr.res_max = m->d_scal + SC_RESF; rr.bsum_partial = m->partial_rr;
      rr.sg = m->sg[0]; rr.cg = m->sg[1];
    }
    auto with_psi_halo = [&](bool splittable, auto launch) {
      if (m->nranks > 1 && m->overlap && splittable) {
        comm_begin(m); m->comm_hold = 1;
        launch(1);
        STICKY(m, exch_nat(m, m->f[MSOM_PSI], nl, m->bc, 3));
        m->comm_hold = 0; comm_end(m);
        launch(2);
      } else {
        if (m->nranks > 1) STICKY(m, exch_nat(m, m->f[MSOM_PSI], nl, m->bc, 3));
        launch(0);
      }
    };
    if (stoch_fused) {
      double dts;
      int r = stoch_prepare(m, adv_dt, &dts);
      if (r) return r;
      m->res_ready = -1;
      prof_begin(m, m->prof_rhs);
      with_psi_halo(true, [&](int region) {
        launch_rhs_lpw(m->st, m->opt, m->f[MSOM_PSI], m->f[MSOM_S], m->f[MSOM_QFORC], m->d_wind, nullptr, m->g, nl, m->walls & WALL_ALL, m->uniformS,
                       m->rc[0].S, with_qforcing && m->have_qforc, D, p.beta, iRe, iRe4, Eks / (p.Rom * 2 * m->dhf[0]),
                       Ekb / (p.Rom * 2 * m->dhf[nl - 1]), p.sbc > 0 ? p.sbc / ((0.5 * p.sbc + 1) * D * D) : 0., m->lc, m->f[adv_in],
                       m->f[adv_out], adv_dt, 1, m->f[qfield], m->f[MSOM_NOISE], -adv_dt * p.itr_stoch, dts, region);
      });
      prof_end(m, m->prof_rhs);
      if (advanced) *advanced = 1;
      return MSOM_OK;
    }
    prof_begin(m, m->prof_rhs);
    with_psi_halo(variant == 6, [&](int region) {
      launch_rhs_fused(m->st, m->opt, m->f[MSOM_PSI], m->f[MSOM_S], m->f[MSOM_QFORC], m->d_wind, m->f[dqfield], nullptr,
                       nullptr, m->g, nl, m->walls & WALL_ALL, m->uniformS, m->rc[0].S, with_qforcing && m->have_qforc, D, p.beta, iRe,
                       iRe4, Eks / (p.Rom * 2 * m->dhf[0]), Ekb / (p.Rom * 2 * m->dhf[nl - 1]),
                       p.sbc > 0 ? p.sbc / ((0.5 * p.sbc + 1) * D * D) : 0., m->lc, variant, adv_out >= 0 ? m->f[adv_in] : nullptr,
                       adv_out >= 0 ? (m->adv_out_override ? m->adv_out_override : m->f[adv_out]) : nullptr, adv_dt, use_rr ? &rr : nullptr, region,
                       variant == 6 ? m->dt_dev : nullptr);
    });
    prof_end(m, m->prof_rhs);
    if (use_rr) m->res_ready = adv_out;
    if (advanced && adv_out >= 0) *advanced = 1;
    return MSOM_OK;
  }
  HIPCHK(hipMemsetAsync(m->f[dqfield], 0, m->g.ls * nl * sizeof(double), m->st));
  comp_del2(m, MSOM_PSI, MSOM_ZETA, 0., 1.0);
  launch_advection(m->st, m->f[MSOM_ZETA], m->f[MSOM_PSI], m->f[MSOM_PSIPG], m->f[MSOM_ZETAPG], m->f[MSOM_S], m->f[qfield], m->f[dqfield],
                   m->g, nl, m->have_pg, m->have_zpg, m->stochastic, D, p.beta, p.itr_stoch, m->lc);
  if (iRe != 0) comp_stretch(m, MSOM_ZETA, dqfield, 1., iRe);
  if (iRe != 0 || iRe4 != 0) comp_del2(m, MSOM_ZETA, MSOM_TMP, 0., 1.);
  if (iRe != 0) launch_axpy(m->st, m->f[dqfield], m->f[MSOM_TMP], m->g, nl, iRe);
  if (iRe4 != 0) {
    comp_stretch(m, MSOM_TMP, dqfield, 1., iRe4);
    comp_del2(m, MSOM_TMP, dqfield, 1., iRe4);
  }
  launch_forcing(m->st, m->f[MSOM_ZETA], m->f[MSOM_PSI], m->f[MSOM_QFORC], m->f[MSOM_TOPO], m->f[MSOM_RO], m->d_wind, m->f[dqfield], m->g,
                 nl, with_qforcing && m->have_qforc, m->flag_topo, Eks / (p.Rom * 2 * m->dhf[0]), Ekb / (p.Rom * 2 * m->dhf[nl - 1]), D,
                 m->dhf[nl - 1]);
  return MSOM_OK;
}

static int tracer_update(msom *m, int cfield);

struct StepDtArgs { double umax_pg[MSOM_MAXNL]; double D, CFL, previous, dtmax, t, tnext; int nl, with_dt; long seq; };
__global__ void __launch_bounds__(64) k_step_dt(double *scal, StepDtArgs a, double *pub) {
#pragma clang fp contract(off)
  if (threadIdx.x == 0 && a.with_dt) {
  const double *umax = scal + SC_UMAX;
  double *out = scal + SC_SPEC;
  double dtmax = a.dtmax, previous = a.previous;
  for (int k = 0; k < 2 * a.nl; k++) {
    const double u = (k & 1) ? a.umax_pg[k >> 1] : umax[k >> 1];
    dtmax /= a.CFL;
    if (u != 0.) {
      const double dt = a.D / u;
      if (dt < dtmax) dtmax = dt;
    }
    dtmax *= a.CFL;
    if (dtmax > previous) dtmax = (previous + 0.1 * dtmax) / 1.1;
    previous = dtmax;
  }
  double dt = dtmax, tnext = a.tnext;
  if (tnext != HUGE_VAL && tnext > a.t) {
    const unsigned int n = (unsigned int)((tnext - a.t) / dt);
    if (n == 0) dt = tnext - a.t;
    else {
      const double dt1 = (tnext - a.t) / n;
      if (dt1 > dt * (1. + 1e-9)) dt = (tnext - a.t) / (n + 1);
      else if (dt1 < dt) dt = dt1;
      tnext = a.t + dt;
    }
  } else
    tnext = a.t + dt;
  out[0] = dtmax; out[1] = dt; out[2] = tnext; out[3] = dt / 2.;
// ... 47 lines not shown
      for (int l = 0; l < nl; l++) {
        const double a = sqrt(-2. * log(((double)(rand()) + 1.) / ((double)(RAND_MAX) + 2.)));
        const double nn = a * cos(2 * M_PI * rand() / (double)RAND_MAX);
        const size_t k = ((size_t)l * ny + j) * nx + i;
        n[k] = m->p.amp_stoch * sig[k] * nn;
      }
  return upload(m, MSOM_NOISE, n.data());
}

static int stoch_prepare(msom *m, double dt, double *dts) {
  if (m->noise_mode == 0 && m->nranks > 1) {
    msom_set_error("stochastic forcing on tiles: the serial rand() stream (noise_mode = 0) exists on a single tile only, use noise_mode = 1");
    return MSOM_ERR_STATE;
  }
  m->corrector_step = (m->corrector_step + 1) % 2;
  float fdts = sqrt(dt);
  if (m->corrector_step) {
    if (m->noise_mode == 0) {
      int r = generate_noise_host(m);
      if (r) return r;
    } else
      launch_noise(m->st, m->f[MSOM_NOISE], m->f[MSOM_SIGMA], m->g, m->nl, m->p.amp_stoch, m->seed, m->noise_draw++, m->ix * m->nx,
                   m->iy * m->ny, m->gnx);
    fdts = fdts / sqrt(2);
  }
  *dts = fdts;
  return MSOM_OK;
}

static int advance_qg(msom *m, int out, int in, int dq, double dt) {
  m->res_ready = -1;
  const double *noise = nullptr;
  double dts = 0;
  if (m->stochastic) {
    int r = stoch_prepare(m, dt, &dts);
    if (r) return r;
    noise = m->f[MSOM_NOISE];
  }
  launch_advance(m->st, m->f[out], m->f[in], m->f[dq], noise, m->g, m->nl, dt, dts);
  fill_bc(m, out);
  return MSOM_OK;
}

#define NEED_CONST(m)                                                    \
  do {                                                                   \
    if (!(m)) return MSOM_ERR_ARG;                                       \
    if (!(m)->const_set) {                                               \
      int r__ = msom_set_const(m);                                       \
      if (r__) return r__;                                               \
    }                                                                    \
  } while (0)

extern "C" double msom_update(msom_t *m, const double *q, double *dqdt, double dtmax) {
  if (!m) return -1;
  if (m->model) return nq_update(m, q, dqdt, dtmax);
  if (!m->const_set && msom_set_const(m)) return -1;
  int qf = MSOM_Q;
  if (q) {
    if (upload(m, MSOM_QPRED, q)) return -1;
    qf = MSOM_QPRED;
  }
  double d = update_qg(m, qf, MSOM_DQ, dtmax);
  if (d < 0) return d;
  if (dqdt && download(m, MSOM_DQ, dqdt)) return -1;
  return d;
}

extern "C" int msom_advance(msom_t *m, double *qout, const double *qin, const double *dqdt, double dt) {
  if (m && m->model) return nq_advance(m, qout, qin, dqdt, dt);
  NEED_CONST(m);
  int in = MSOM_Q, out = MSOM_Q, r;
  if (qin) {
    if ((r = upload(m, MSOM_QPRED, qin))) return r;
    in = out = MSOM_QPRED;
  }
  if (dqdt && (r = upload(m, MSOM_DQ, dqdt))) return r;
  if ((r = advance_qg(m, out, in, MSOM_DQ, dt))) return r;
  if (qout) return download(m, out, qout);
  return sync_stream(m);
}

extern "C" int msom_invertq(msom_t *m, const double *q, double *psi, msom_mgstats *st) {
  if (m && m->model) return nq_invertq(m, q, psi, st);
  NEED_CONST(m);
  int qf = MSOM_Q, r;
  if (q) {
    if ((r = upload(m, MSOM_QPRED, q))) return r;
    qf = MSOM_QPRED;
  }
  if (psi && (r = upload(m, MSOM_PSI, psi))) return r;
  if ((r = invertq(m, m->f[qf]))) return r;
  if (st) *st = m->mg;
  if (psi) return download(m, MSOM_PSI, psi);
  return sync_stream(m);
}

extern "C" int msom_comp_q(msom_t *m, const double *psi, double *q) {
  if (m && m->model) return nq_comp_q_api(m, psi, q);
  NEED_CONST(m);
  int r;
  if (psi && (r = upload(m, MSOM_PSI, psi))) return r;
  comp_del2(m, MSOM_PSI, MSOM_Q, 0., 1.);
  comp_stretch(m, MSOM_PSI, MSOM_Q, 1., 1.);
  if (q) return download(m, MSOM_Q, q);
  return sync_stream(m);
}

extern "C" int msom_last_mgstats(msom_t *m, msom_mgstats *st) {
  if (!m || !st) return MSOM_ERR_ARG;
  *st = m->mg;
  return MSOM_OK;
}

extern "C" int msom_modes_mgstats(msom_t *m, int mode, msom_mgstats *st) {
  MSQG_ONLY(m);
  if (!m || !st) return MSOM_ERR_ARG;
  if (!m->const_set || !m->helm_solved) { msom_set_error("msom_modes_mgstats: no modal solve since msom_set_const"); return MSOM_ERR_STATE; }
  if (mode < 0 || mode >= m->nl) { msom_set_error("msom_modes_mgstats: mode %d outside 0 .. %d", mode, m->nl - 1); return MSOM_ERR_ARG; }
  *st = m->helm.s[mode];
  return MSOM_OK;
}


static int check_shape(msom *m, int a, int b, int c) {
  if (a != m->nl || b != m->ny || c != m->nx) {
    msom_set_error("array shape (%d,%d,%d) != (nl,N,N) = (%d,%d,%d)", a, b, c, m->nl, m->ny, m->nx);
    return MSOM_ERR_ARG;
  }
  return MSOM_OK;
}

extern "C" int pystep_bfn(msom_t *m, double *varin_py, int len1, int len2, int len3, double *tend_py, int len4, int len5, int len6,
                          double direction, int vartype) {
  MSQG_ONLY(m);
  NEED_CONST(m);
  if (check_shape(m, len1, len2, len3) || check_shape(m, len4, len5, len6)) return MSOM_ERR_ARG;
  Params &p = m->p;
  int r;
  if (direction > 0) {
    p.iRe = p.Re == 0 ? 0. : 1 / p.Re;
    p.iRe4 = p.Re4 == 0 ? 0. : -1 / p.Re4;
    p.Eks = fabs(p.Eks); p.Ekb = fabs(p.Ekb);
  } else {
    p.iRe = p.Re == 0 ? 0. : -1 / p.Re;
    p.iRe4 = p.Re4 == 0 ? 0. : 1 / p.Re4;
    p.Eks = -fabs(p.Eks); p.Ekb = -fabs(p.Ekb);
  }
  if (vartype != 1) HIPCHK(hipMemsetAsync(m->f[MSOM_DQ], 0, m->g.ls * m->nl * sizeof(double), m->st));
  if (vartype == 1) {
    if ((r = upload(m, MSOM_Q, varin_py))) return r;
    if (solve_and_dt(m, MSOM_Q, p.DT) < 0) return MSOM_ERR_HIP;
    if ((r = rhs_terms(m, MSOM_Q, MSOM_DQ, 0, p.iRe, p.iRe4, p.Eks, p.Ekb))) return r;
  } else if (!m->quiet)
    fprintf(stdout, "temporary disabled psi tendency\n");
  return download(m, MSOM_DQ, tend_py);
}
extern "C" int pyq2p(msom_t *m, double *po_py, int len7, int len8, int len9, double *qo_py, int len10, int len11, int len12) {
  MSQG_ONLY(m);
  NEED_CONST(m);
  if (check_shape(m, len7, len8, len9) || check_shape(m, len10, len11, len12)) return MSOM_ERR_ARG;
  int r;
  HIPCHK(hipMemsetAsync(m->f[MSOM_PSI], 0, m->g.ls * m->nl * sizeof(double), m->st));
  if ((r = upload(m, MSOM_Q, qo_py))) return r;
  if ((r = invertq(m, m->f[MSOM_Q]))) return r;
  return download(m, MSOM_PSI, po_py);
}
extern "C" int pyp2q(msom_t *m, double *po_py, int len13, int len14, int len15, double *qo_py, int len16, int len17, int len18) {
  MSQG_ONLY(m);
  NEED_CONST(m);
  if (check_shape(m, len13, len14, len15) || check_shape(m, len16, len17, len18)) return MSOM_ERR_ARG;
  return msom_comp_q(m, po_py, qo_py);
}


static int ensure_field(msom *m, int field);
extern "C" int msom_bfn_begin(msom_t *m) {
  MSQG_ONLY(m);
  NEED_CONST(m);
  int r;
  for (int k = MSOM_BFN_F1; k <= MSOM_BFN_F3; k++) {
    if ((r = ensure_field(m, k))) return r;
    HIPCHK(hipMemsetAsync(m->f[k], 0, m->g.ls * m->nl * sizeof(double), m->st));
  }
  m->bfn_begun = 1;
  return sync_stream(m);
}

extern "C" int msom_bfn_steps(msom_t *m, int nsteps, double dt, double direction, double k) {
  MSQG_ONLY(m);
  if (!m) return MSOM_ERR_ARG;
  if (nsteps < 0) { msom_set_error("msom_bfn_steps: nsteps = %d", nsteps); return MSOM_ERR_ARG; }
  if (!m->const_set || !m->bfn_begun) { msom_set_error("msom_bfn_steps before msom_bfn_begin"); return MSOM_ERR_STATE; }
  if (k != 0 && !m->bfn_obs_set) { msom_set_error("msom_bfn_steps: k != 0 and MSOM_BFN_OBS was never set"); return MSOM_ERR_STATE; }
  if (nsteps == 0) return MSOM_OK;
  Params &p = m->p;
  int r;
  if (direction > 0) {
    p.iRe = p.Re == 0 ? 0. : 1 / p.Re;
    p.iRe4 = p.Re4 == 0 ? 0. : -1 / p.Re4;
    p.Eks = fabs(p.Eks); p.Ekb = fabs(p.Ekb);
  } else {
    p.iRe = p.Re == 0 ? 0. : -1 / p.Re;
    p.iRe4 = p.Re4 == 0 ? 0. : 1 / p.Re4;
    p.Eks = -fabs(p.Eks); p.Ekb = -fabs(p.Ekb);
  }
  const double dt12 = dt / 12;
  const double *obs = k != 0 ? m->f[MSOM_BFN_OBS] : nullptr, *gain = (k != 0 && m->bfn_gain_set) ? m->f[MSOM_BFN_GAIN] : nullptr;
  for (int n = 0; n < nsteps; n++) {
    if (solve_and_dt(m, MSOM_Q, p.DT) < 0) return m->sticky ? m->sticky : MSOM_ERR_HIP;
    if ((r = rhs_terms(m, MSOM_Q, MSOM_BFN_F1, 0, p.iRe, p.iRe4, p.Eks, p.Ekb))) return r;
    launch_bfn_ab3(m->st, m->f[MSOM_Q], m->f[MSOM_BFN_F1], m->f[MSOM_BFN_F2], m->f[MSOM_BFN_F3], obs, gain, m->g, m->nl, dt12, k);
    fill_bc(m, MSOM_Q);
    m->res_ready = -1;
    m->umax_ready = 0;
    m->spec_valid = 0;
    double *f1 = m->f[MSOM_BFN_F1];
    m->f[MSOM_BFN_F1] = m->f[MSOM_BFN_F3];
    m->f[MSOM_BFN_F3] = m->f[MSOM_BFN_F2];
    m->f[MSOM_BFN_F2] = f1;
  }
  return sync_stream(m);
}

extern "C" int msom_bfn_misfit(msom_t *m, double *misfit) {
  MSQG_ONLY(m);
  if (!m || !misfit) return MSOM_ERR_ARG;
  if (!m->bfn_obs_set) { msom_set_error("msom_bfn_misfit: MSOM_BFN_OBS was never set"); return MSOM_ERR_STATE; }
  if (!m->bfn_partial) HIPCHK(hipMalloc(&m->bfn_partial, 2 * ((size_t)bfn_misfit_blocks(m->g) + 64) * sizeof(double)));
  launch_bfn_misfit(m->st, m->f[MSOM_Q], m->f[MSOM_BFN_OBS], m->bfn_gain_set ? m->f[MSOM_BFN_GAIN] : nullptr, m->bfn_partial,
                    m->d_scal + SC_LSUM, m->g, m->nl);
  int r = reduce_scal(m, SC_LSUM, 2, RED_SUM);
  if (r) return r;
  *misfit = sqrt(m->h_scal[SC_LSUM] / m->h_scal[SC_LSUM + 1]);
  return MSOM_OK;
}


static void stats_drop(msom *m) {
  for (int k = 0; k < MSOM_ST_NACC; k++) {
    if (m->stats.s[k]) hipFree(m->stats.s[k]);
    m->stats.s[k] = nullptr;
  }
  if (m->stats_W) hipFree(m->stats_W);
  if (m->stats_qme) hipFree(m->stats_qme);
  m->stats_W = m->stats_qme = nullptr;
  m->stats_mask = 0;
  m->stats_count = m->stats_ndev = 0;
}
static void stats_sample(msom *m, const double *w_dev, double w) {
  launch_stats_acc(m->st, m->stats_mask, m->f[MSOM_PSI], m->f[MSOM_Q], m->stats, m->g, m->nl, w_dev, w, 2. * (m->p.L0 / m->gnx), m->stats_W);
}
#define NEED_STATS(m, fn)                                                                   \
  do {                                                                                      \
    if (!(m)->const_set || !(m)->stats_mask) {                                              \
      msom_set_error(fn ": no msom_stats_begin since msom_set_const");                      \
      return MSOM_ERR_STATE;                                                                \
    }                                                                                       \
  } while (0)

extern "C" int msom_stats_begin(msom_t *m, unsigned mask) {
  MSQG_ONLY(m);
  if (!m) return MSOM_ERR_ARG;
  if (mask == 0 || mask >> MSOM_ST_NACC) { msom_set_error("msom_stats_begin: mask 0x%x", mask); return MSOM_ERR_ARG; }
  if (!m->const_set) { msom_set_error("msom_stats_begin before msom_set_const"); return MSOM_ERR_STATE; }
  HIPCHK(hipStreamSynchronize(m->st));
  const size_t bytes = m->g.ls * m->nl * sizeof(double);
  for (int k = 0; k < MSOM_ST_NACC; k++) {
    const bool want = (mask >> k) & 1u;
    if (!want && m->stats.s[k]) { HIPCHK(hipFree(m->stats.s[k])); m->stats.s[k] = nullptr; }
    if (want && !m->stats.s[k]) HIPCHK(hipMalloc(&m->stats.s[k], bytes));
    if (want) HIPCHK(hipMemsetAsync(m->stats.s[k], 0, bytes, m->st));
  }
  if (!m->stats_W) HIPCHK(hipMalloc(&m->stats_W, sizeof(double)));
  HIPCHK(hipMemsetAsync(m->stats_W, 0, sizeof(double), m->st));
  m->stats_mask = mask;
  m->stats_count = m->stats_ndev = 0;
  return sync_stream(m);
}

extern "C" int msom_stats_accumulate(msom_t *m, double w) {
  MSQG_ONLY(m);
  if (!m) return MSOM_ERR_ARG;
  if (!std::isfinite(w)) { msom_set_error("msom_stats_accumulate: w = %g", w); return MSOM_ERR_ARG; }
  NEED_STATS(m, "msom_stats_accumulate");
  stats_sample(m, nullptr, w);
  return m->sticky;
}

extern "C" int msom_stats_weight(msom_t *m, double *W) {
  MSQG_ONLY(m);
  if (!m || !W) return MSOM_ERR_ARG;
  NEED_STATS(m, "msom_stats_weight");
  HIPCHK(hipMemcpyAsync(W, m->stats_W, sizeof(double), hipMemcpyDeviceToHost, m->st));
  return sync_stream(m);
}

extern "C" int msom_stats_get(msom_t *m, int which, double *out) {
  MSQG_ONLY(m);
  if (!m || !out) return MSOM_ERR_ARG;
  const size_t n = (size_t)m->nl * m->nx * m->ny;
  if (which == MSOM_ST_QME) {
    if (!m->const_set || !m->stats_qme) { msom_set_error("msom_stats_get: no msom_time_filter since msom_set_const"); return MSOM_ERR_STATE; }
    launch_unpack(m->st, m->stats_qme, m->staging, m->g, m->nl);
    HIPCHK(hipMemcpyAsync(out, m->staging, n * sizeof(double), hipMemcpyDefault, m->st));
    return sync_stream(m);
  }
  unsigned need;
  int sa = -1;
  if (which >= 0 && which < MSOM_ST_NACC) need = 1u << which;
  else if (which == MSOM_ST_EKE) need = 1u << MSOM_ST_PSI | 1u << (sa = MSOM_ST_KE);
  else if (which == MSOM_ST_UQ_EDDY) need = 1u << MSOM_ST_PSI | 1u << MSOM_ST_Q | 1u << (sa = MSOM_ST_UQ);
  else if (which == MSOM_ST_VQ_EDDY) need = 1u << MSOM_ST_PSI | 1u << MSOM_ST_Q | 1u << (sa = MSOM_ST_VQ);
  else { msom_set_error("msom_stats_get: unknown id %d", which); return MSOM_ERR_ARG; }
  NEED_STATS(m, "msom_stats_get");
  if ((m->stats_mask & need) != need) { msom_set_error("msom_stats_get: id %d needs accumulators 0x%x, the mask is 0x%x", which, need, m->stats_mask); return MSOM_ERR_ARG; }
  double W = 0;
  int r = msom_stats_weight(m, &W);
  if (r) return r;
  if (W == 0) { msom_set_error("msom_stats_get: the sum of the weights is 0"); return MSOM_ERR_STATE; }
  launch_stats_mean(m->st, m->f[MSOM_TMP], m->stats.s[sa < 0 ? which : MSOM_ST_PSI], m->stats_W, m->g, m->nl);
  if (sa < 0) return download(m, MSOM_TMP, out);
  if ((r = fill_bc(m, MSOM_TMP))) return r;
  launch_stats_derive(m->st, m->staging, m->f[MSOM_TMP], m->stats.s[sa], m->stats.s[MSOM_ST_Q], m->stats_W, m->g, m->nl, which,
                      2. * (m->p.L0 / m->gnx));
  HIPCHK(hipMemcpyAsync(out, m->staging, n * sizeof(double), hipMemcpyDefault, m->st));
  return sync_stream(m);
}

extern "C" int msom_time_filter(msom_t *m, double dt) {
  MSQG_ONLY(m);
  if (!m) return MSOM_ERR_ARG;
  if (!std::isfinite(dt)) { msom_set_error("msom_time_filter: dt = %g", dt); return MSOM_ERR_ARG; }
  if (!m->const_set) { msom_set_error("msom_time_filter before msom_set_const"); return MSOM_ERR_STATE; }
  if (!m->stats_qme) {
    const size_t bytes = m->g.ls * m->nl * sizeof(double);
    HIPCHK(hipMalloc(&m->stats_qme, bytes));
    HIPCHK(hipMemsetAsync(m->stats_qme, 0, bytes, m->st));
  }
  launch_time_filter(m->st, m->stats_qme, m->f[MSOM_Q], m->g, m->nl, dt / m->tau_f);
  return sync_stream(m);
}


static void modes_drop(msom *m) {
  if (m->modes_md) hipFree(m->modes_md);
  m->modes_md = nullptr;
  helm_drop_pyramid(m);
  m->modes_ready = m->modes_compact = 0;
}
static ModesLayers modes_layers(const msom *m) {
  ModesLayers l = {};
  for (int k = 0; k < m->nl; k++) l.dhf[k] = m->dhf[k];
  for (int k = 0; k < m->nl - 1; k++) l.dhc[k] = m->dhc[k];
  return l;
}
static const ModeCoef *modes_mc(const msom *m) { return m->modes_compact ? &m->modes_mc : nullptr; }
static bool is_device_ptr(const void *p) {
  hipPointerAttribute_t a;
  if (hipPointerGetAttributes(&a, p) != hipSuccess) { (void)hipGetLastError(); return false; }
  return a.type == hipMemoryTypeDevice;
}
#define NEED_MODES(m, fn)                                                                   \
  do {                                                                                      \
    if (!(m)->const_set || !(m)->modes_ready) {                                             \
      msom_set_error(fn ": no successful msom_modes_compute since msom_set_const");         \
      return MSOM_ERR_STATE;                                                                \
    }                                                                                       \
  } while (0)

extern "C" int msom_modes_compute(msom_t *m) {
  MSQG_ONLY(m);
  NEED_CONST(m);
  const int nl = m->nl, na = nl * nl + nl;
  const int compact = m->modes_compact_opt != 0 && m->fr_uniform;
  modes_drop(m);
  if (!m->modes_flag) HIPCHK(hipMalloc(&m->modes_flag, sizeof(int)));
  if (!m->modes_dev) HIPCHK(hipMalloc(&m->modes_dev, sizeof(ModeCoef)));
  HIPCHK(hipMemsetAsync(m->modes_flag, 0, sizeof(int), m->st));
  int r;
  if (compact) {
    r = launch_modes_eig(m->st, m->f[MSOM_S], m->g, nl, 1, 1, m->modes_dev, 1, 0, modes_layers(m), m->modes_flag);
  } else {
    const size_t bytes = (size_t)na * m->g.ls * sizeof(double);
    HIPCHK(hipMalloc(&m->modes_md, bytes));
    HIPCHK(hipMemsetAsync(m->modes_md, 0, bytes, m->st));
    r = launch_modes_eig(m->st, m->f[MSOM_S], m->g, nl, m->nx, m->ny, m->modes_md, m->g.ls, 1, modes_layers(m), m->modes_flag);
  }
  if (r) { modes_drop(m); msom_set_error("msom_modes_compute: no kernel for nl = %d", nl); return MSOM_ERR_CONFIG; }
  int flag = 0;
  double h[MSOM_MAXNL * MSOM_MAXNL + MSOM_MAXNL];
  HIPCHK(hipMemcpyAsync(&flag, m->modes_flag, sizeof(int), hipMemcpyDeviceToHost, m->st));
  if (compact) HIPCHK(hipMemcpyAsync(h, m->modes_dev, na * sizeof(double), hipMemcpyDeviceToHost, m->st));
  if ((r = sync_stream(m))) { modes_drop(m); return r; }
  if (flag) {
    modes_drop(m);
    if (flag & MODES_BAD_S) msom_set_error("msom_modes_compute: S = (Fr/Ro)^2 is not positive and finite on every interface: the spectrum is degenerate");
    else msom_set_error("msom_modes_compute: the Jacobi iteration did not converge within %d sweeps", MODES_MAXSWEEP);
    return MSOM_ERR_CONFIG;
  }
  if (compact) {
    memset(&m->modes_mc, 0, sizeof m->modes_mc);
    for (int k = 0; k < nl * nl; k++) m->modes_mc.m2l[k] = h[k];
    for (int k = 0; k < nl; k++) m->modes_mc.ibu[k] = h[nl * nl + k];
  }
  m->modes_compact = compact;
  m->modes_ready = 1;
  return MSOM_OK;
}

extern "C" int msom_modes_layers(msom_t *m, int which) {
  MSQG_ONLY(m);
  if (!m || which < 0 || which >= MSOM_MD_N) return MSOM_ERR_ARG;
  NEED_MODES(m, "msom_modes_layers");
  return which == MSOM_MD_IBU || which == MSOM_MD_RD ? m->nl : m->nl * m->nl;
}

extern "C" int msom_modes_get(msom_t *m, int which, double *out) {
  MSQG_ONLY(m);
  if (!m || which < 0 || which >= MSOM_MD_N || !out) return MSOM_ERR_ARG;
  NEED_MODES(m, "msom_modes_get");
  const int nl = m->nl, n = which == MSOM_MD_IBU || which == MSOM_MD_RD ? nl : nl * nl;
  const size_t cells = (size_t)m->nx * m->ny;
  for (int first = 0; first < n; first += nl) {
    const int cnt = std::min(nl, n - first);
    if (launch_modes_get(m->st, m->staging, m->modes_md, modes_mc(m), m->g, nl, modes_layers(m), which, first, cnt)) return MSOM_ERR_CONFIG;
    HIPCHK(hipMemcpyAsync(out + first * cells, m->staging, cnt * cells * sizeof(double), hipMemcpyDefault, m->st));
  }
  return sync_stream(m);
}

extern "C" int msom_modes_project(msom_t *m, int to_modes, const double *in, double *out) {
  MSQG_ONLY(m);
  if (!m || !in || !out) return MSOM_ERR_ARG;
  NEED_MODES(m, "msom_modes_project");
  const size_t bytes = (size_t)m->nl * m->nx * m->ny * sizeof(double);
  if (is_device_ptr(in) && is_device_ptr(out)) {
    if (launch_modes_project(m->st, in, out, m->modes_md, modes_mc(m), m->g, m->nl, modes_layers(m), to_modes != 0)) return MSOM_ERR_CONFIG;
    return m->sticky;
  }
  HIPCHK(hipMemcpyAsync(m->staging, in, bytes, hipMemcpyDefault, m->st));
  if (launch_modes_project(m->st, m->staging, m->staging, m->modes_md, modes_mc(m), m->g, m->nl, modes_layers(m), to_modes != 0)) return MSOM_ERR_CONFIG;
  HIPCHK(hipMemcpyAsync(out, m->staging, bytes, hipMemcpyDefault, m->st));
  return sync_stream(m);
}

static int modes_energy_launch(msom *m) {
  if (!m->modes_partial) HIPCHK(hipMalloc(&m->modes_partial, (size_t)2 * MSOM_MAXNL * modes_energy_stride(m->g) * sizeof(double)));
  if (launch_modes_energy(m->st, m->f[MSOM_PSI], m->modes_md, modes_mc(m), m->g, m->nl, modes_layers(m), m->modes_partial, m->modes_dev,
                          m->p.L0 / m->gnx))
    return MSOM_ERR_CONFIG;
  return MSOM_OK;
}
extern "C" int msom_modes_energy(msom_t *m, double *ke, double *pe) {
  MSQG_ONLY(m);
  if (!m || (!ke && !pe)) return MSOM_ERR_ARG;
  NEED_MODES(m, "msom_modes_energy");
  const int nl = m->nl;
  int r = modes_energy_launch(m);
  if (r) return r;
  double *dst[2] = {ke, pe};
  for (int part = 0; part < 2; part++) {
    HIPCHK(hipMemcpyAsync(m->d_scal + SC_LSUM, m->modes_dev + part * nl, nl * sizeof(double), hipMemcpyDeviceToDevice, m->st));
    if ((r = reduce_scal(m, SC_LSUM, nl, RED_SUM))) return r;
    if (dst[part]) for (int k = 0; k < nl; k++) dst[part][k] = m->h_scal[SC_LSUM + k];
  }
  return sync_stream(m);
}

extern "C" int msom_modes_set_rd(msom_t *m, int mode) {
  MSQG_ONLY(m);
  if (!m || mode < 1 || mode > m->nl - 1) return MSOM_ERR_ARG;
  NEED_MODES(m, "msom_modes_set_rd");
  if (launch_modes_rd(m->st, m->f[MSOM_RD], m->modes_md, modes_mc(m), m->g, m->nl, mode)) return MSOM_ERR_CONFIG;
  fill_bc(m, MSOM_RD);
  m->wv_ready = 0;
  return sync_stream(m);
}


static bool spec_pow2(int n) { return n > 0 && (n & (n - 1)) == 0; }
extern "C" int msom_spec_layout(int nx, int ny, int *nbins, long *count) {
  if (!spec_pow2(nx) || !spec_pow2(ny) || std::min(nx, ny) < SPEC_MINN || std::max(nx, ny) > 32768) {
    msom_set_error("msom_spec_layout: %d x %d: both sides must be powers of two, 8 .. 32768", nx, ny);
    return MSOM_ERR_CONFIG;
  }
  const int nmax = std::max(nx, ny), sx = nmax / nx, sy = nmax / ny, nb = nmax / 2 - 2, hx = nx / 2, hy = ny / 2;
  if (nbins) *nbins = nb;
  if (!count) return MSOM_OK;
  for (int r = 0; r < nb; r++) count[r] = 0;
  for (int i = 0; i <= hx; i++) {
    const long wi = (i == 0 || i == hx) ? 1 : 2;
    int s = i * sx;
    for (int j = 0; j <= hy; j++) {
      const long w = wi * ((j == 0 || j == hy) ? 1 : 2);
      const long R2 = (long)(i * sx) * (i * sx) + (long)(j * sy) * (j * sy);
      while ((long)(s + 1) * (s + 1) <= R2) s++;
      if (s < nb) count[s] += w;
      if ((long)s * s == R2 && s >= 1 && s - 1 < nb) count[s - 1] += w;
    }
  }
  return MSOM_OK;
}

static void spec_drop(msom *m) {
  for (void *p : {(void *)m->spc_z, (void *)m->spc_zt, (void *)m->spc_tw, (void *)m->spc_v, (void *)m->spc_te, (void *)m->spc_res, (void *)m->spc_hin,
                  (void *)m->spc_o2d})
    if (p) hipFree(p);
  m->spc_z = m->spc_zt = m->spc_tw = nullptr;
  m->spc_v = m->spc_te = m->spc_res = m->spc_hin = m->spc_o2d = nullptr;
  m->spc_batch = 0;
  m->spc_bytes = 0;
}
static int spec_guard(msom *m, const char *fn) {
  if (m->nranks > 1) { msom_set_error("%s: the spectra run on a single tile, this handle is one of %d", fn, m->nranks); return MSOM_ERR_CONFIG; }
  if (!m->const_set) { msom_set_error("%s: call msom_set_const first", fn); return MSOM_ERR_STATE; }
  if (!spec_pow2(m->nx) || !spec_pow2(m->ny) || std::min(m->nx, m->ny) < SPEC_MINN || std::max(m->nx, m->ny) > SPEC_MAXN) {
    msom_set_error("%s: %d x %d: both sides must be powers of two, %d .. %d", fn, m->nx, m->ny, SPEC_MINN, SPEC_MAXN);
    return MSOM_ERR_CONFIG;
  }
  return MSOM_OK;
}
#define SPEC_SCRATCH_CAP ((size_t)1 << 30)
// ... 154 lines not shown
  return spec_run(m, spec_in_nat(m, SPEC_IN_AB, m->f[field_a], same ? nullptr : m->f[field_b]), nullptr, nullptr, m->flayers[field_a],
                  same ? SPEC_SUM : SPEC_CROSS, nullptr, spec, flux);
}
extern "C" int msom_spec_energy(msom_t *m, double *ke, double *pe) {
  MSQG_ONLY(m);
  if (!m || (!ke && !pe)) return MSOM_ERR_ARG;
  SPEC_ENTRY(m, "msom_spec_energy");
  const int nl = m->nl, nb = spec_nbins(m);
  int r;
  if (ke) {
    if ((r = spec_run(m, spec_in_nat(m, SPEC_IN_UV, m->f[MSOM_PSI], nullptr), nullptr, nullptr, nl, SPEC_SUM, nullptr, ke, nullptr))) return r;
    for (int l = 0; l < nl; l++)
      for (int k = 0; k < nb; k++) ke[(size_t)l * nb + k] = 0.5 * ke[(size_t)l * nb + k] * m->dhf[l];
  }
  if (pe && nl > 1) {
    if ((r = spec_run(m, spec_in_nat(m, SPEC_IN_G, m->f[MSOM_PSI], m->f[MSOM_S]), nullptr, nullptr, nl - 1, SPEC_SUM, nullptr, pe, nullptr))) return r;
    for (int l = 0; l < nl - 1; l++)
      for (int k = 0; k < nb; k++) pe[(size_t)l * nb + k] = 0.5 * pe[(size_t)l * nb + k] * m->dhc[l];
  }
  return MSOM_OK;
}


static double dtnext(msom *m, double dt, double *tnext_out) {
  double tnext = m->tnext, t = m->t;
  if (tnext != HUGE_VAL && tnext > t) {
    unsigned int n = (unsigned int)((tnext - t) / dt);
    if (n == 0) dt = tnext - t;
    else {
      double dt1 = (tnext - t) / n;
      if (dt1 > dt * (1. + 1e-9)) dt = (tnext - t) / (n + 1);
      else if (dt1 < dt) dt = dt1;
      tnext = t + dt;
    }
  } else
    tnext = t + dt;
  *tnext_out = tnext;
  return dt;
}

static int tracer_update(msom *m, int cfield) {
  const int nt = m->nl * m->p.nptr;
  HIPCHK(hipMemsetAsync(m->f[MSOM_DPTR], 0, m->g.ls * nt * sizeof(double), m->st));
  launch_ptr_rhs(m->st, m->f[MSOM_PSI], m->f[cfield], m->f[MSOM_PTR_RELAX], m->f[MSOM_DPTR], m->g, m->nl, m->p.nptr, m->p.iPe, m->p.ptr_ir,
                 m->p.L0 / m->gnx);
  return MSOM_OK;
}
static int tracer_advance(msom *m, int out, int in, double dt) {
  launch_advance(m->st, m->f[out], m->f[in], m->f[MSOM_DPTR], nullptr, m->g, m->nl * m->p.nptr, dt, 0.);
  return fill_bc(m, out);
}

static bool spec_ok(msom *m) {
  return layered_fusions(m) && m->async_solve && m->nranks == 1 && m->fused && m->adv_fused && m->rhs_variant == 6 && !m->rhs_resid && m->mg_fused && m->nlev > 1 &&
         m->nl <= MSOM_FASTNL && !m->have_pg && !m->have_zpg && !m->flag_topo && !m->stochastic && m->p.nptr == 0 && m->p.nitermin >= 1 && !m->dbg_nosync;
}

extern "C" int msom_step(msom_t *m, double *dt_used) {
  if (m && m->model) return nq_step(m, dt_used);
  NEED_CONST(m);
  if (m->stats_on && !m->stats_mask) { msom_set_error("msom_step: option stats = 1 and no msom_stats_begin since msom_set_const"); return MSOM_ERR_STATE; }
  const Params &p = m->p;
  double tnext;
  int r, advanced = 0;
  const bool spec = spec_ok(m);
  int spec_rc = 0;
  if (spec) {
    m->dt_dev = m->d_scal + SC_SPEC + 3;
    m->spec_hook = [&](const std::function<void()> &host_read) {
      StepDtArgs a;
      for (int l = 0; l < MSOM_MAXNL; l++) a.umax_pg[l] = m->umax_pg[l];
      a.D = p.L0 / m->gnx; a.CFL = p.CFL; a.previous = m->previous; a.dtmax = p.DT; a.t = m->t; a.tnext = m->tnext; a.nl = m->nl;
      a.with_dt = 1; a.seq = ++m->pub_seq;
      hipLaunchKernelGGL(k_step_dt, dim3(1), dim3(64), 0, m->st, m->d_scal, a, m->d_pub);
      host_read();
      int adv = 0;
      spec_rc = rhs_terms(m, MSOM_Q, MSOM_DQ, 1, p.iRe, p.iRe4, p.Eks, p.Ekb, MSOM_QPRED, MSOM_Q, 0., &adv);
      if (!adv && !spec_rc) spec_rc = MSOM_ERR_STATE;
    };
  }
  const double d = solve_and_dt(m, MSOM_Q, p.DT);
  m->spec_hook = nullptr;
  const bool hit1 = spec && m->spec_valid && !spec_rc;
  m->dt_dev = nullptr;
  if (d < 0) return m->sticky ? m->sticky : MSOM_ERR_HIP;
  if (hit1) {
    m->dt = m->h_scal[SC_SPEC + 1];
    tnext = m->h_scal[SC_SPEC + 2];
  } else {
    m->dt = dtnext(m, d, &tnext);
    if ((r = rhs_terms(m, MSOM_Q, MSOM_DQ, 1, p.iRe, p.iRe4, p.Eks, p.Ekb, MSOM_QPRED, MSOM_Q, m->dt / 2., &advanced))) return r;
    if (!advanced && (r = advance_qg(m, MSOM_QPRED, MSOM_Q, MSOM_DQ, m->dt / 2.))) return r;
  }
  if (m->stats_on && m->stats_count++ % m->stats_every == 0) {
    stats_sample(m, hit1 ? m->d_scal + SC_SPEC + 1 : nullptr, m->dt);
    m->stats_ndev += hit1;
  }
  const bool tracers = m->p.nptr > 0;
  if (tracers && ((r = tracer_update(m, MSOM_PTR)) || (r = tracer_advance(m, MSOM_PTR_PRED, MSOM_PTR, m->dt / 2.)))) return r;
  spec_rc = 0;
  if (spec) {
    if (!m->q_alt) {
      HIPCHK(hipMalloc(&m->q_alt, m->g.ls * m->nl * sizeof(double)));
      HIPCHK(hipMemcpyAsync(m->q_alt, m->f[MSOM_Q], m->g.ls * m->nl * sizeof(double), hipMemcpyDeviceToDevice, m->st));
    }
    m->spec_hook = [&](const std::function<void()> &host_read) {
      StepDtArgs a;
      memset(&a, 0, sizeof a);
      a.with_dt = 0; a.seq = ++m->pub_seq;
      hipLaunchKernelGGL(k_step_dt, dim3(1), dim3(64), 0, m->st, m->d_scal, a, m->d_pub);
      host_read();
      int adv = 0;
      m->adv_out_override = m->q_alt;
      spec_rc = rhs_terms(m, MSOM_QPRED, MSOM_DQ, 1, p.iRe, p.iRe4, p.Eks, p.Ekb, MSOM_Q, MSOM_Q, m->dt, &adv);
      m->adv_out_override = nullptr;
      if (!adv && !spec_rc) spec_rc = MSOM_ERR_STATE;
    };
  }
  const double d2 = solve_and_dt(m, MSOM_QPRED, m->dt);
  m->spec_hook = nullptr;
  if (d2 < 0) return m->sticky ? m->sticky : MSOM_ERR_HIP;
  if (spec && m->spec_valid && !spec_rc) std::swap(m->f[MSOM_Q], m->q_alt);
  else {
    if ((r = rhs_terms(m, MSOM_QPRED, MSOM_DQ, 1, p.iRe, p.iRe4, p.Eks, p.Ekb, MSOM_Q, MSOM_Q, m->dt, &advanced))) return r;
    if (!advanced && (r = advance_qg(m, MSOM_Q, MSOM_Q, MSOM_DQ, m->dt))) return r;
  }
  if (tracers && ((r = tracer_update(m, MSOM_PTR_PRED)) || (r = tracer_advance(m, MSOM_PTR, MSOM_PTR, m->dt)))) return r;
  const bool lazy = m->step_sync == 0 || (m->step_sync < 0 && (size_t)m->g.nx * m->g.ny * m->nl < ((size_t)1 << 23));
  if (!spec || !lazy) { if ((r = sync_stream(m))) return r; }
  else if (m->sticky) return m->sticky;
  m->t = tnext;
  m->iter++;
  if (dt_used) *dt_used = m->dt;
  return MSOM_OK;
}
extern "C" int msom_sync(msom_t *m) {
  if (!m) return MSOM_ERR_ARG;
  return sync_stream(m);
}
extern "C" int msom_set_tnext(msom_t *m, double tnext) {
  if (!m) return MSOM_ERR_ARG;
  m->tnext = tnext;
  return MSOM_OK;
}
extern "C" double msom_time(msom_t *m) { return m ? m->t : NAN; }
extern "C" int msom_iter(msom_t *m) { return m ? m->iter : -1; }

extern "C" double msom_ke(msom_t *m) {
  if (!m) return NAN;
  launch_ke(m->st, m->f[MSOM_PSI], m->partial, m->d_scal + SC_KE, m->g, m->p.L0 / m->gnx);
  if (reduce_scal(m, SC_KE, 1, RED_SUM)) return NAN;
  return -m->h_scal[SC_KE];
}


static int nq_alloc(msom *m) {
  for (int k = 0; k < m->nlev; k++) {
    memset(&m->rc[k], 0, sizeof m->rc[k]);
    m->rc[k].D = m->p.L0 / (double)(m->gnx >> k);
    m->rc[k].sqD = m->rc[k].D * m->rc[k].D;
  }
  HIPCHK(hipMalloc(&m->helm_scal, HS_COUNT * sizeof(double)));
  HIPCHK(hipMalloc(&m->helm_partial, (size_t)MSOM_MAXNL * helm_partial_stride(m) * sizeof(double)));
  return MSOM_OK;
}

static msom *nq_create(NewqgParams &q, const char *text) {
  if (msom_newqg_params_derive(&q)) return nullptr;
  Params p;
  msom_params_defaults(&p);
  p.N = q.N; p.Ny = q.Ny; p.nl = 1; p.L0 = q.L0; p.DT = q.DT; p.CFL = q.CFL; p.tolerance = q.TOLERANCE;
  p.nitermax = q.nitermax; p.nitermin = q.nitermin; p.sbc = q.sbc; p.beta = q.beta; p.tau0 = q.tau0; p.tend = q.tend; p.dtout = q.dtout;
  p.dhu[0] = q.dh[0];
  msom *m = create_common(p, 1, 1, 0, nullptr, &q);
  if (m) m->params_text = text;
  return m;
// ... 484 lines not shown
    double *s = k == 0 ? f : m->wv_s[k], *out = k == 0 ? f : m->wv_r[k];
    launch_wv_recon(m->st, s, m->wv_s[k + 1], m->wv_r[k + 1], m->wv_sig[k], out, m->wv_g[k], m->wv_g[k + 1], nl);
    wv_fill(m, out, m->wv_g[k]);
  }
  HIPCHK(hipGetLastError());
  return m->sticky;
}
static int wavelet_filter(msom *m, int qof_field, double dtflt) {
  NEED_CONST(m);
  int r;
  if ((r = wavelet_setup(m)) || (r = ensure_field(m, qof_field))) return r;
  const int nl = m->nl;
  HIPCHK(hipMemcpyAsync(m->f[MSOM_TMP], m->f[MSOM_Q], m->g.ls * nl * sizeof(double), hipMemcpyDeviceToDevice, m->st));
  if ((r = invertq(m, m->f[MSOM_Q]))) return r;
  if ((r = wavelet_apply(m, m->f[MSOM_PSI]))) return r;
  m->umax_ready = 0;
  comp_del2(m, MSOM_PSI, MSOM_Q, 0., 1.);
  comp_stretch(m, MSOM_PSI, MSOM_Q, 1., 1.);
  launch_wv_qof(m->st, m->f[qof_field], m->f[MSOM_Q], m->f[MSOM_TMP], m->g, nl, dtflt, 0, dtflt < 0.0);
  if (dtflt < 0.0) fill_bc(m, MSOM_Q);
  fill_bc(m, qof_field);
  return sync_stream(m);
}
extern "C" int msom_wavelet_filter(msom_t *m, double dtflt) {
  MSQG_ONLY(m);
  return wavelet_filter(m, MSOM_QOF, dtflt);
}


static int ensure_de_fields(msom *m) {
  for (int k = MSOM_DE_BF; k <= MSOM_PO_MFT; k++) {
    int r = ensure_field(m, k);
    if (r) return r;
  }
  return MSOM_OK;
}
static int de_terms(msom *m, double dt, double ediag) {
  const Params &p = m->p;
  const int nl = m->nl;
  const double D = p.L0 / m->gnx;
  launch_advection_de(m->st, m->f[MSOM_ZETA], m->f[MSOM_PSI], m->f[MSOM_PSIPG], m->f[MSOM_ZETAPG], m->f[MSOM_S], m->f[MSOM_DE_J1], m->f[MSOM_DE_J2],
                      m->f[MSOM_DE_J3], m->g, nl, D, p.beta, dt, ediag, m->lc);
  comp_del2(m, MSOM_ZETA, MSOM_TMP, 0., 1.);
  comp_stretch(m, MSOM_ZETA, MSOM_TMP2, 0., 1.);
  launch_dissip_de(m->st, m->f[MSOM_TMP], m->f[MSOM_TMP2], m->f[MSOM_PSI], m->f[MSOM_DE_VD], m->g, nl, p.iRe, p.iRe4, dt, ediag, D, 0);
  comp_stretch(m, MSOM_TMP, MSOM_TMP2, 0., 1.);
  launch_dissip_de(m->st, m->f[MSOM_TMP], m->f[MSOM_TMP2], m->f[MSOM_PSI], m->f[MSOM_DE_VD], m->g, nl, p.iRe, p.iRe4, dt, ediag, D, 1);
  launch_ekman_de(m->st, m->f[MSOM_ZETA], m->f[MSOM_PSI], m->f[MSOM_DE_BF], m->g, nl, p.Eks / (p.Rom * 2 * m->dhf[0]),
                  p.Ekb / (p.Rom * 2 * m->dhf[nl - 1]), dt, ediag);
  HIPCHK(hipGetLastError());
  return m->sticky;
}
extern "C" int msom_energy_tend(msom_t *m, double dt) {
  MSQG_ONLY(m);
  NEED_CONST(m);
  int r;
  if ((r = ensure_de_fields(m))) return r;
  comp_del2(m, MSOM_PSI, MSOM_ZETA, 0., 1.0);
  if ((r = de_terms(m, dt, (double)m->p.ediag))) return r;
  launch_running_mean(m->st, m->f[MSOM_PO_MFT], m->f[MSOM_PSI], m->g, m->nl, m->nme_ft);
  m->nme_ft += 1;
  return sync_stream(m);
}
static int filter_de(msom *m, int pm_field, double dtflt, double ediag) {
  int r;
  if ((r = ensure_de_fields(m))) return r;
  if ((r = wavelet_filter(m, MSOM_TMP2, -dtflt))) return r;
  launch_filter_de(m->st, m->f[MSOM_DE_FT], m->f[MSOM_TMP2], m->f[pm_field], m->g, m->nl, dtflt, ediag);
  m->nme_ft = 0;
  return sync_stream(m);
}
extern "C" int msom_filter_de(msom_t *m, int pm_field, double dtflt) {
  MSQG_ONLY(m);
  NEED_CONST(m);
  if (pm_field < 0 || pm_field >= MSOM_NFIELDS || m->flayers[pm_field] != m->nl) { msom_set_error("bad field id %d", pm_field); return MSOM_ERR_ARG; }
  int r = ensure_field(m, pm_field);
  return r ? r : filter_de(m, pm_field, dtflt, (double)m->p.ediag);
}
extern "C" int msom_reset_de(msom_t *m) {
  MSQG_ONLY(m);
  if (!m) return MSOM_ERR_ARG;
  int r;
  if ((r = ensure_de_fields(m))) return r;
  for (int k = MSOM_DE_BF; k <= MSOM_DE_FT; k++) HIPCHK(hipMemsetAsync(m->f[k], 0, m->g.ls * m->nl * sizeof(double), m->st));
  return sync_stream(m);
}
extern "C" int pystep_de(msom_t *m, const double *po_py, int len1, int len2, int len3, double *de_bf_py, int len4, int len5, int len6,
                         double *de_vd_py, int len7, int len8, int len9, double *de_j1_py, int len10, int len11, int len12,
                         double *de_j2_py, int len13, int len14, int len15, double *de_j3_py, int len16, int len17, int len18,
                         double *de_ft_py, int len19, int len20, int len21, int onlyKE) {
  MSQG_ONLY(m);
  NEED_CONST(m);
  if (check_shape(m, len1, len2, len3) || check_shape(m, len4, len5, len6) || check_shape(m, len7, len8, len9) || check_shape(m, len10, len11, len12) ||
      check_shape(m, len13, len14, len15) || check_shape(m, len16, len17, len18) || check_shape(m, len19, len20, len21))
    return MSOM_ERR_ARG;
  if (!po_py) return MSOM_ERR_ARG;
  const double ediag = 1., dt = 1.;
  int r;
  if ((r = upload(m, MSOM_PSI, po_py)) || (r = msom_reset_de(m))) return r;
  m->umax_ready = 0;
  comp_del2(m, MSOM_PSI, MSOM_ZETA, 0., 1.0);
  comp_del2(m, MSOM_PSI, MSOM_Q, 0., 1.);
  comp_stretch(m, MSOM_PSI, MSOM_Q, 1., 1.);
  if (onlyKE == 1 && !m->s_zero) {
    m->s_zero = 1;
    if ((r = build_coefs(m))) return r;
  }
  if ((r = de_terms(m, dt, ediag)) || (r = filter_de(m, MSOM_PSI, m->p.dtflt, ediag))) return r;
  double *outs[6] = {de_bf_py, de_vd_py, de_j1_py, de_j2_py, de_j3_py, de_ft_py};
  for (int k = 0; k < 6; k++)
    if (outs[k] && (r = download(m, MSOM_DE_BF + k, outs[k]))) return r;
  return MSOM_OK;
}

extern "C" int msom_dbg_wavelet_levels(msom_t *m) {
  MSQG_ONLY(m);
  if (!m) return MSOM_ERR_ARG;
  int r = wavelet_setup(m);
  return r ? r : m->wv_nlev;
}
extern "C" int msom_dbg_siglev(msom_t *m, int level, double *out) {
  MSQG_ONLY(m);
  if (!m || !out) return MSOM_ERR_ARG;
  int r = wavelet_setup(m);
  if (r) return r;
  if (level < 0 || level >= (int)m->wv_g.size()) { msom_set_error("bad level %d (tiles: only the levels that live on the tile)", level); return MSOM_ERR_ARG; }
  const NatGeom &g = m->wv_g[level];
  HIPCHK(hipMemcpy2DAsync(out, g.nx * sizeof(double), m->wv_sig[level] + nat_idx(g, 0, 0, 0), g.pitch * sizeof(double), g.nx * sizeof(double), g.ny,
                          hipMemcpyDefault, m->st));
  return sync_stream(m);
}
extern "C" int msom_dbg_wavelet_apply(msom_t *m, int field) {
  MSQG_ONLY(m);
  NEED_CONST(m);
  if (field < 0 || field >= MSOM_NFIELDS || !m->f[field] || m->flayers[field] != m->nl) { msom_set_error("bad field id %d", field); return MSOM_ERR_ARG; }
  int r = wavelet_apply(m, m->f[field]);
  return r ? r : sync_stream(m);
}


static int gather_global(msom *m, int field, std::vector<double> &g) {
  const int nlf = m->flayers[field];
  const size_t cnt = (size_t)nlf * m->nx * m->ny;
  g.resize((size_t)nlf * m->gnx * m->gny);
  if (m->nranks == 1) return download(m, field, g.data());
  double *recv = nullptr;
  HIPCHK(hipMalloc(&recv, cnt * m->nranks * sizeof(double)));
  launch_unpack(m->st, m->f[field], m->staging, m->g, nlf);
  comm_begin(m);
  int r = comm_allgather(m->comm, m->staging, recv, cnt);
  comm_end(m);
  std::vector<double> h(cnt * m->nranks);
  if (!r) {
    hipError_t e = hipMemcpyAsync(h.data(), recv, h.size() * sizeof(double), hipMemcpyDeviceToHost, m->st);
    if (e == hipSuccess) e = hipStreamSynchronize(m->st);
    if (e != hipSuccess) { msom_set_error("HIP error %s in gather_global", hipGetErrorString(e)); r = MSOM_ERR_HIP; }
  }
  (void)hipFree(recv);
  if (r) return r;
  for (int q = 0; q < m->nranks; q++) {
    const int tx = q % m->px, ty = q / m->px;
    for (int l = 0; l < nlf; l++)
      for (int j = 0; j < m->ny; j++)
        memcpy(&g[((size_t)l * m->gny + ty * m->ny + j) * m->gnx + (size_t)tx * m->nx], &h[q * cnt + ((size_t)l * m->ny + j) * m->nx], m->nx * sizeof(double));
  }
  return MSOM_OK;
}
static int scatter_global(msom *m, int field, const std::vector<double> &g) {
  const int nlf = m->flayers[field];
  if (m->nranks == 1) return msom_set_field(m, field, g.data());
  std::vector<double> t((size_t)nlf * m->nx * m->ny);
  for (int l = 0; l < nlf; l++)
    for (int j = 0; j < m->ny; j++)
      memcpy(&t[((size_t)l * m->ny + j) * m->nx], &g[((size_t)l * m->gny + m->iy * m->ny + j) * m->gnx + (size_t)m->ix * m->nx], m->nx * sizeof(double));
  return msom_set_field(m, field, t.data());
}

extern "C" int msom_write_bas(msom_t *m, int field, const char *path) {
  MSQG_ONLY(m);
  if (check_field(m, field) || !path) return MSOM_ERR_ARG;
  if (m->gnx != m->gny) { msom_set_error(".bas output needs a square grid"); return MSOM_ERR_STATE; }
  std::vector<double> h;
  int r = gather_global(m, field, h);
  if (r) return r;
  if (m->rank != 0) return MSOM_OK;
  return msom_bas_write(path, h.data(), m->flayers[field], m->gnx, m->p.L0) ? MSOM_ERR_IO : MSOM_OK;
}
extern "C" int msom_read_bas(msom_t *m, int field, const char *path) {
  MSQG_ONLY(m);
  if (check_field(m, field) || !path) return MSOM_ERR_ARG;
  if (m->gnx != m->gny) { msom_set_error(".bas input needs a square grid"); return MSOM_ERR_STATE; }
  std::vector<double> h((size_t)m->flayers[field] * m->gnx * m->gny);
  if (msom_bas_read(path, h.data(), m->flayers[field], m->gnx, m->p.L0)) return MSOM_ERR_IO;
  return scatter_global(m, field, h);
}

extern "C" int msom_write_nc(msom_t *m, const char *path) {
  if (!m || !path) return MSOM_ERR_ARG;
  static const char *names[2] = {"psi", "q"};
  std::vector<double> hp, hq;
  int r;
  if ((r = gather_global(m, MSOM_PSI, hp)) || (r = gather_global(m, MSOM_Q, hq))) return r;
  if (m->rank != 0) return MSOM_OK;
  struct stat sb;
  if (stat(path, &sb) != 0 && msom_nc_create(path, m->nl, m->gny, m->gnx, m->p.L0, 2, names)) return MSOM_ERR_IO;
  const double *f[2] = {hp.data(), hq.data()};
  return msom_nc_append(path, m->nl, m->gny, m->gnx, 2, names, m->t, f) < 0 ? MSOM_ERR_IO : MSOM_OK;
}
extern "C" int msom_read_nc(msom_t *m, int field, const char *path, const char *varname, int record) {
  if (check_field(m, field) || !path || !varname) return MSOM_ERR_ARG;
  std::vector<double> h((size_t)m->flayers[field] * m->gnx * m->gny);
  int r = msom_nc_read(path, varname, record, m->flayers[field], m->gny, m->gnx, h.data(), nullptr);
  if (r) return r == -2 ? MSOM_ERR_IO : MSOM_ERR_ARG;
  return scatter_global(m, field, h);
}

static bool file_exists(const char *path) {
  struct stat sb;
  return stat(path, &sb) == 0;
}

extern "C" int msom_read_inputs(msom_t *m, const char *dir) {
  MSQG_ONLY(m);
  if (!m) return MSOM_ERR_ARG;
  char name[512];
  const char *d = dir ? dir : ".";
  const int nl = m->nl, N = m->gnx;
  int r;
  const bool say = !m->quiet && m->rank == 0;
  if (say) fprintf(stdout, "Read input files:\n");
  snprintf(name, sizeof name, "%s/dh_%dl.bin", d, nl);
  if (FILE *fp = fopen(name, "r")) {
    std::vector<float> dh(nl);
    size_t got = fread(dh.data(), sizeof(float), nl, fp);
    fclose(fp);
    if (got != (size_t)nl) { msom_set_error("short read on %s", name); return MSOM_ERR_IO; }
    for (int l = 0; l < nl; l++) m->dhf[l] = dh[l];
    if (say) fprintf(stdout, "%s .. ok\n", name);
  }
  struct { const char *fmt; int field; } files[] = {
      {"%s/psipg_%dl_N%d.bas", MSOM_PSIPG}, {"%s/frpg_%dl_N%d.bas", MSOM_FR}, {"%s/rdpg_%dl_N%d.bas", MSOM_RD},
      {"%s/qforc_%dl_N%d.bas", MSOM_QFORC}};
  for (auto &f : files) {
    snprintf(name, sizeof name, f.fmt, d, nl, N);
    if (file_exists(name)) {
      if ((r = msom_read_bas(m, f.field, name))) return r;
      if (say) fprintf(stdout, "%s .. ok\n", name);
    }
  }
  snprintf(name, sizeof name, "%s/topo.bas", d);
  if (file_exists(name)) {
    if ((r = msom_read_bas(m, MSOM_TOPO, name))) return r;
    if (say) fprintf(stdout, "%s .. ok\n", name);
  }
  if (m->p.nptr > 0) {
    snprintf(name, sizeof name, "%s/ptr0.bas", d);
    if (file_exists(name)) {
      if ((r = msom_read_bas(m, MSOM_PTR, name))) return r;
      if (say) fprintf(stdout, "%s .. ok\n", name);
    }
    snprintf(name, sizeof name, "%s/ptr_relax.bas", d);
    if (file_exists(name) && (r = msom_read_bas(m, MSOM_PTR_RELAX, name))) return r;
  }
  snprintf(name, sizeof name, "%s/p0.bas", d);
  if (file_exists(name)) {
    if ((r = msom_read_bas(m, MSOM_PSI, name))) return r;
    if (say) fprintf(stdout, "%s .. ok\n", name);
  }
  m->const_set = 0;
  return MSOM_OK;
}

static int backup_config(msom *m, const char *dpath) {
  const bool root = m->rank == 0;
  if (root) fprintf(stdout, "Backup config\n");
// ... 145 lines not shown
  msom_params_defaults(&p);
  msom_params_parse_text(&p, params_text);
  msom *m = create_common(p, px, py, rank, id128);
  if (m) m->params_text = params_text;
  return m;
}
extern "C" int msom_tile_info(msom_t *m, int *px, int *py, int *ix, int *iy, int *nx_local, int *ny_local) {
  MSQG_ONLY(m);
  if (!m) return MSOM_ERR_ARG;
  if (px) *px = m->px;
  if (py) *py = m->py;
  if (ix) *ix = m->ix;
  if (iy) *iy = m->iy;
  if (nx_local) *nx_local = m->nx;
  if (ny_local) *ny_local = m->ny;
  return MSOM_OK;
}


extern "C" int msom_dbg_nlevels(msom_t *m) { return m ? m->nlev : MSOM_ERR_ARG; }
extern "C" int msom_dbg_level_dims(msom_t *m, int lev, int *nx, int *ny) {
  if (!m || lev < 0 || lev >= m->nlev) return MSOM_ERR_ARG;
  *nx = m->sg[lev].nx; *ny = m->sg[lev].ny;
  return MSOM_OK;
}
static int split_upload(msom *m, double *sp, const SplitGeom &sg, const double *a, int nl, int bc) {
  HIPCHK(hipMemcpyAsync(m->staging, a, (size_t)nl * sg.nx * sg.ny * sizeof(double), hipMemcpyDefault, m->st));
  HIPCHK(hipMemsetAsync(sp, 0, sg.ls * nl * sizeof(double), m->st));
  launch_split_pack(m->st, m->staging, sp, sg, nl, bc, m->walls);
  return MSOM_OK;
}
static int split_download(msom *m, const double *sp, const SplitGeom &sg, double *a, int nl) {
  launch_split_unpack(m->st, sp, sg, m->staging, nl);
  HIPCHK(hipMemcpyAsync(a, m->staging, (size_t)nl * sg.nx * sg.ny * sizeof(double), hipMemcpyDefault, m->st));
  return sync_stream(m);
}
extern "C" int msom_dbg_relax(msom_t *m, int lev, double *da, const double *res, int nsweeps) {
  MSQG_ONLY(m);
  if (m) m->res_ready = -1;
  NEED_CONST(m);
  if (lev < 0 || lev >= m->nlev || !da || !res) return MSOM_ERR_ARG;
  int r;
  if ((r = split_upload(m, m->da[lev], m->sg[lev], da, m->nl, BC_DIRICHLET0))) return r;
  if ((r = split_upload(m, m->res[lev], m->sg[lev], res, m->nl, BC_NEUMANN))) return r;
  STICKY(m, exch_split(m, m->da[lev], m->sg[lev], m->nl, 0));
  const int prof = m->profile;
  m->profile = 0;
  {
    Lev L = tile_lev(m, lev);
    relax_sweeps(m, L, nullptr, nsweeps, 0);
  }
  m->profile = prof;
  return split_download(m, m->da[lev], m->sg[lev], da, m->nl);
}
extern "C" int msom_dbg_residual(msom_t *m, const double *a, const double *b, double *res, double *maxres) {
  MSQG_ONLY(m);
  if (m) m->res_ready = -1;
  NEED_CONST(m);
  int r;
  if ((r = upload(m, MSOM_TMP, a))) return r;
  if ((r = upload(m, MSOM_QPRED, b))) return r;
  HIPCHK(hipMemsetAsync(m->d_scal, 0, 8 * sizeof(double), m->st));
  residual(m, m->f[MSOM_TMP], m->f[MSOM_QPRED], SC_RES0, 0);
  HIPCHK(hipMemcpyAsync(m->h_scal + SC_RES0, m->d_scal + SC_RES0, sizeof(double), hipMemcpyDeviceToHost, m->st));
  if ((r = split_download(m, m->res[0], m->sg[0], res, m->nl))) return r;
  if (maxres) *maxres = m->h_scal[SC_RES0];
  return MSOM_OK;
}
extern "C" int msom_dbg_helm_relax(msom_t *m, int lev, double *da, const double *res, int nhalf, const int *count_per_mode) {
  MSQG_ONLY(m);
  if (m) m->res_ready = -1;
  NEED_CONST(m);
  if (lev < 0 || lev >= m->nlev || !da || !res || nhalf < 0) return MSOM_ERR_ARG;
  int r;
  if ((r = helm_ensure(m))) return r;
  if ((r = split_upload(m, m->da[lev], m->sg[lev], da, m->nl, BC_DIRICHLET0))) return r;
  if ((r = split_upload(m, m->res[lev], m->sg[lev], res, m->nl, BC_NEUMANN))) return r;
  HelmCount cnt = {};
  for (int k = 0; k < m->nl; k++) cnt.n[k] = count_per_mode ? count_per_mode[k] : (nhalf + 1) / 2;
  if ((r = helm_relax_level(m, lev, nhalf, cnt, nullptr))) return r;
  return split_download(m, m->da[lev], m->sg[lev], da, m->nl);
}
extern "C" int msom_dbg_helm_residual(msom_t *m, const double *a, const double *b, double *res, double *maxres_per_mode) {
  MSQG_ONLY(m);
  if (m) m->res_ready = -1;
  NEED_CONST(m);
  if (!a || !b || !res) return MSOM_ERR_ARG;
  int r;
  if ((r = helm_ensure(m))) return r;
  const size_t n = (size_t)m->nl * m->nx * m->ny * sizeof(double);
  HIPCHK(hipMemcpyAsync(m->staging, a, n, hipMemcpyDefault, m->st));
  launch_pack(m->st, m->staging, m->f[MSOM_TMP], m->g, m->nl);
  helm_fill(m, m->f[MSOM_TMP]);
  HIPCHK(hipMemcpyAsync(m->staging, b, n, hipMemcpyDefault, m->st));
  launch_pack(m->st, m->staging, m->helm_qm, m->g, m->nl);
  HIPCHK(hipMemsetAsync(m->helm_scal, 0, HS_COUNT * sizeof(double), m->st));
  if ((r = helm_residual(m, m->f[MSOM_TMP], m->helm_qm, HS_RES0, 0))) return r;
  double hs[HS_COUNT];
  if ((r = helm_read(m, hs))) return r;
  if ((r = split_download(m, m->res[0], m->sg[0], res, m->nl))) return r;
  if (maxres_per_mode) for (int k = 0; k < m->nl; k++) maxres_per_mode[k] = hs[HS_RES0 + k];
  return MSOM_OK;
}
extern "C" int msom_dbg_restrict(msom_t *m, int lev_fine, const double *fine, double *coarse) {
  MSQG_ONLY(m);
  if (m) m->res_ready = -1;
// ... 155 lines not shown
```

Baseline: 17.63 billion grid-point-updates/s.

## Emit multigrid initial residual as by-product of fused tendency+advance pass

The lpw tendency+advance kernel now also computes the next inversion's residual (q minus the elliptic operator of psi), its max, the bsum partials and the restricted coarse residual. The rhs_resid option becomes auto-on for large grids with rhs_variant 6, so the solver can skip a separate residual kernel pass over the fine grid. In exchange the residual variant uses R=2 rows per block, an extra shared-memory slot and more registers, which may lower throughput of the tendency kernel. Many API entry points now invalidate res_ready so a stale residual is never reused.

```diff
diff --git a/include/msom.h b/include/msom.h
--- a/include/msom.h
+++ b/include/msom.h
@@ -165,6 +165,7 @@
 int msom_dbg_level_dims(msom_t *m, int lev, int *nx, int *ny);
 int msom_dbg_relax(msom_t *m, int lev, double *da, const double *res, int nsweeps);
 int msom_dbg_residual(msom_t *m, const double *a, const double *b, double *res, double *maxres);
+int msom_dbg_rhs_resid(msom_t *m, int fused, double dt, double *res0, double *res1, double *maxres, double *bsum);
 int msom_dbg_helm_relax(msom_t *m, int lev, double *da, const double *res, int nhalf, const int *count_per_mode);
 int msom_dbg_helm_residual(msom_t *m, const double *a, const double *b, double *res, double *maxres_per_mode);
 int msom_dbg_restrict(msom_t *m, int lev_fine, const double *fine, double *coarse);
diff --git a/msom_amd/api.py b/msom_amd/api.py
--- a/msom_amd/api.py
+++ b/msom_amd/api.py
@@ -107,6 +107,7 @@
         "msom_dbg_level_dims": (ci, [vp, ci, C.POINTER(ci), C.POINTER(ci)]),
         "msom_dbg_relax": (ci, [vp, ci, vp, vp, ci]),
         "msom_dbg_residual": (ci, [vp, vp, vp, vp, _dp]),
+        "msom_dbg_rhs_resid": (ci, [vp, ci, cd, vp, vp, _dp, _dp]),
         "msom_dbg_restrict": (ci, [vp, ci, vp, vp]),
         "msom_dbg_prolong": (ci, [vp, ci, vp, vp]),
         "msom_dbg_op": (ci, [vp, cs, ci, ci, cd, cd]),
@@ -523,6 +524,14 @@
         self._chk(self.L.msom_dbg_residual(self.h, _ptr(a), _ptr(b), _ptr(res), C.byref(m)))
         return res, m.value
 
+    def dbg_rhs_resid(self, fused, dt):
+        nl = int(self.param("nl"))
+        r0 = np.empty((nl, int(self.param("split_ls_0"))))
+        r1 = np.empty((nl, int(self.param("split_ls_1"))))
+        mx, bs = C.c_double(), C.c_double()
+        self._chk(self.L.msom_dbg_rhs_resid(self.h, int(bool(fused)), float(dt), _ptr(r0), _ptr(r1), C.byref(mx), C.byref(bs)))
+        return r0, r1, mx.value, bs.value
+
     def restrict(self, lev_fine, fine):
         fine = _f64(fine)
         nl, ny, nx = fine.shape
diff --git a/msom_amd/csrc/kernels.h b/msom_amd/csrc/kernels.h
--- a/msom_amd/csrc/kernels.h
+++ b/msom_amd/csrc/kernels.h
@@ -132,7 +132,8 @@
                     const NatGeom &g, int nl, int walls, int uniformS, const double *Su, int have_qforc, double D, double beta, double iRe, double iRe4,
                     double cs, double cb, double slip_c, const LayerCoef &lc, const double *q_in, double *q_out, double dt, int stoch = 0,
                     const double *q_stage = nullptr, const double *noise = nullptr, double crelax = 0., double dts = 0., int region = 0,
-                    const double *dt_ptr = nullptr);
+                    const double *dt_ptr = nullptr, const RhsResid *rr = nullptr);
+int rhs_lpw_blocks(const KernelOpts &o, const NatGeom &g, int nl);
 
 #define MGC_MAXLEV 8
 #define MGC_MAXDIM 32
diff --git a/msom_amd/csrc/kernels_fused.hip b/msom_amd/csrc/kernels_fused.hip
--- a/msom_amd/csrc/kernels_fused.hip
+++ b/msom_amd/csrc/kernels_fused.hip
@@ -562,7 +562,7 @@
                       const LayerCoef &lc, int variant, const double *q_in, double *q_out, double dt, const RhsResid *rr, int region, const double *dt_ptr) {
   if (variant == 6) {
     launch_rhs_lpw(st, o, psi, S, qforc, wind, dq, g, nl, walls, uniformS, Su, have_qforc, D, beta, iRe, iRe4, cs, cb, slip_c, lc, q_in, q_out, dt,
-                   0, nullptr, nullptr, 0., 0., region, dt_ptr);
+                   0, nullptr, nullptr, 0., 0., region, dt_ptr, q_out ? rr : nullptr);
     return;
   }
   RhsArgs a;
diff --git a/msom_amd/csrc/kernels_lpw.hip b/msom_amd/csrc/kernels_lpw.hip
--- a/msom_amd/csrc/kernels_lpw.hip
+++ b/msom_amd/csrc/kernels_lpw.hip
@@ -4,6 +4,7 @@
 
 #define LPW_W 58
 #define LPW_R 4
+#define LPW_R_RES 2
 #ifdef MSOM_STRICT
 #define LPW_NV 3
 #define LPW_MAXW 8
@@ -24,13 +25,14 @@
   int noedge_off;
   int region;
   int dbg;
+  RhsResid rr;
   double D, beta, iRe, iRe4, cs, cb, slip_c;
   LayerCoef lc;
   double Su[MSOM_MAXNL];
 };
 
-template <int R, bool UNI, bool QF, bool ADV, bool STOCH, bool EDGE>
-__device__ __forceinline__ void lpw_body(const LpwArgs &a, double (&ring)[2][LPW_MAXW][R][LPW_NV][64]) {
+template <int R, bool UNI, bool QF, bool ADV, bool STOCH, bool EDGE, bool RES, int NV>
+__device__ __forceinline__ void lpw_body(const LpwArgs &a, double (&ring)[2][LPW_MAXW][R][NV][64], double &res_m, double &res_bs) {
   const int lane = threadIdx.x & 63;
   const int wv = __builtin_amdgcn_readfirstlane((int)(threadIdx.x >> 6));
   const int nl = a.nl, nx = a.g.nx, ny = a.g.ny;
@@ -41,6 +43,8 @@
   const int gi = x0 - 3 + lane, gic = min(gi, nx + 2);
   const double dtv = a.dt_ptr ? *a.dt_ptr : a.dt;
   const double D = a.D, D2 = D * D, rD2 = 1. / D2, D12 = 12. * D * D, rD12 = 1. / D12, D2x = 2 * D, rD2x = 1. / D2x;
+  const double rD = 1. / D;
+  const bool oddx = !(lane & 1);
   const bool lower = l + 1 < nl, upper = l > 0;
   const int lW = ((a.walls & WALL_W) && x0 == 0) ? 2 : -1;
   const int eL = nx - x0 + 3;
@@ -75,6 +79,9 @@
   double tlA[R];
 #endif
   double pnext[R], qnext[R], qreg[R], fqreg[R], qsreg[STOCH ? R : 1], nzreg[STOCH ? R : 1];
+  double xdA[R], ydA[R];
+#pragma unroll
+  for (int r = 0; r < R; r++) xdA[r] = ydA[r] = 0.;
 #pragma unroll
   for (int r = 0; r < R; r++) {
 #ifdef MSOM_STRICT
@@ -147,6 +154,19 @@
     const double jd = (lower && !STOCH) ? mjac9(p, p1, D12, rD12) : 0.;
     const double zc = Z[1], tc = T[1];
     const double lapT = lap5(tc, TL[0], TR[0], T[2], T[0]);
+    if (RES) {
+      const double dW = P[1] - PL[1], dE = PR[1] - P[1], dS = P[1] - P[0], dN = P[2] - P[1];
+#ifdef MSOM_STRICT
+      xdA[r] = (dW / D - dE / D) / D;
+      ydA[r] = (dS / D - dN / D) / D;
+#else
+      const double fa = oddx ? dW : dE, fb = oddx ? dE : dW;
+      const double x = fma(rD, fb, -(rD * fa));
+      xdA[r] = oddx ? -x : x;
+      ydA[r] = fma(rD, dS, -(rD * dN));
+#endif
+      ring[b][wv][r][NV - 1][lane] = Q[1] - P[1];
+    }
 #ifdef MSOM_STRICT
     abA[r] = adv + be; jdA[r] = jd; lapTA[r] = lapT; zcA[r] = zc; tcA[r] = tc;
     ring[b][wv][r][0][lane] = zc;
@@ -209,6 +229,22 @@
 #endif
   };
 
+  auto resid = [&](int b, int r, double s0, double s1, double q) -> double {
+    double re = q;
+#ifdef MSOM_STRICT
+    if (upper) re = re + s0 * ring[b][wv - 1][r][NV - 1][lane] * idh0;
+    if (lower) re = re - s1 * ring[b][wv][r][NV - 1][lane] * idh1;
+    re += xdA[r];
+    re += ydA[r];
+#else
+    if (upper) re = fma(idh0, s0 * ring[b][wv - 1][r][NV - 1][lane], re);
+    if (lower) re = fma(-(ring[b][wv][r][NV - 1][lane] * s1), idh1, re);
+    re = fma(rD, xdA[r], re);
+    re = fma(rD, ydA[r], re);
+#endif
+    return re;
+  };
+
 #pragma unroll
   for (int r = 0; r < R; r++) {
     pnext[r] = ld(pP, y0 + r + 3);
@@ -248,6 +284,30 @@
 #pragma unroll
       for (int r = 0; r < R; r++)
         if (out_ok && jb + r < y1 && !(a.dbg & 1)) outp[nat_idx(a.g, l, jb + r, gic)] = val[r];
+      if (RES) {
+        double re[R];
+#pragma unroll
+        for (int r = 0; r < R; r++) {
+          re[r] = resid(b ^ 1, r, s0[r], s1[r], val[r]);
+          if (out_ok && jb + r < y1) {
+            res_m = fmax(res_m, fabs(re[r]));
+            res_bs += val[r];
+            if (!(a.dbg & 1)) a.rr.res[split_idx(a.rr.sg, l, jb + r, gi)] = re[r];
+          }
+        }
+#pragma unroll
+        for (int r = 0; r + 1 < R; r += 2) {
+          const double o0 = lane_above(re[r]), o1 = lane_above(re[r + 1]);
+          if (out_ok && !oddx && jb + r + 1 < y1 && !(a.dbg & 1)) {
+            double sum = 0.;
+            sum += re[r];
+            sum += re[r + 1];
+            sum += o0;
+            sum += o1;
+            a.rr.res_c[split_idx(a.rr.cg, l, (jb + r) >> 1, gi >> 1)] = sum / 4;
+          }
+        }
+      }
     }
     if (k < nblk) {
       const int j0 = y0 + k * R;
@@ -274,9 +334,12 @@
   }
 }
 
-template <int R, bool UNI, bool QF, bool ADV, bool STOCH = false>
+template <int R, bool UNI, bool QF, bool ADV, bool STOCH = false, bool RES = false>
 __global__ void __launch_bounds__(64 * LPW_MAXW) k_rhs_lpw(LpwArgs a) {
-  __shared__ double ring[2][LPW_MAXW][R][LPW_NV][64];
+  static_assert(!RES || (ADV && !STOCH && R % 2 == 0), "the residual by-product rides in the plain tendency + advance pass");
+  constexpr int NV = LPW_NV + (RES ? 1 : 0);
+  __shared__ double ring[2][LPW_MAXW][R][NV][64];
+  double res_m = 0., res_bs = 0.;
   const int wv = __builtin_amdgcn_readfirstlane((int)(threadIdx.x >> 6));
   const int nx = a.g.nx, ny = a.g.ny;
   const int strip = blockIdx.x * a.NS + wv / a.nl, nstrips = (nx + LPW_W - 1) / LPW_W;
@@ -288,15 +351,67 @@
     const bool inner = strip < nstrips && x0 - 3 >= 0 && x0 + 60 < nx && y0 - 3 >= 0 && y0 + nblk * R + R + 2 < ny;
     if ((a.region == 1) != inner) return;
   }
-  if (xwall || ywall || a.noedge_off) lpw_body<R, UNI, QF, ADV, STOCH, true>(a, ring);
-  else lpw_body<R, UNI, QF, ADV, STOCH, false>(a, ring);
+  if (xwall || ywall || a.noedge_off) lpw_body<R, UNI, QF, ADV, STOCH, true, RES, NV>(a, ring, res_m, res_bs);
+  else lpw_body<R, UNI, QF, ADV, STOCH, false, RES, NV>(a, ring, res_m, res_bs);
+  if (RES) {
+    const int lane = threadIdx.x & 63, nw = blockDim.x >> 6;
+    for (int o = 32; o > 0; o >>= 1) {
+      res_m = fmax(res_m, __shfl_xor(res_m, o, 64));
+      res_bs += __shfl_xor(res_bs, o, 64);
+    }
+    double *red = &ring[0][0][0][0][0];
+    if (lane == 0) { red[wv] = res_m; red[LPW_MAXW + wv] = res_bs; }
+    __syncthreads();
+    if (threadIdx.x == 0) {
+      double mm = red[0], ss = red[LPW_MAXW];
+      for (int k = 1; k < nw; k++) { mm = fmax(mm, red[k]); ss += red[LPW_MAXW + k]; }
+      atomicMax((unsigned long long *)a.rr.res_max, (unsigned long long)__double_as_longlong(mm));
+      a.rr.bsum_partial[blockIdx.y * gridDim.x + blockIdx.x] = ss;
+    }
+  }
+}
+
+static void lpw_shape(const KernelOpts &o, const NatGeom &g, int nl, bool res, int &NS, int &H) {
+  const int strips = (g.nx + LPW_W - 1) / LPW_W;
+  H = o.rhs_dbg >> 8;
+  NS = LPW_MAXW / nl < 1 ? 1 : LPW_MAXW / nl;
+  if (NS > strips) NS = strips;
+  if (H <= 0) {
+    const int ncu = device_cu_count();
+    const int wgx = (strips + NS - 1) / NS;
+    double best = -1.;
+    for (int h = 64; h >= 8; h -= 8) {
+      const double r = (double)wgx * ((g.ny + h - 1) / h) / ncu, cost = (r <= 3. ? ceil(r) : r + 0.5) * (h + 6);
+      if (best < 0. || cost < best) { best = cost; H = h; }
+    }
+  }
+  if (H < 8) H = 8;
+  if (res) H = (H + 1) & ~1;
+}
+int rhs_lpw_blocks(const KernelOpts &o, const NatGeom &g, int nl) {
+  int NS, H;
+  lpw_shape(o, g, nl, true, NS, H);
+  const int strips = (g.nx + LPW_W - 1) / LPW_W;
+  return ((strips + NS - 1) / NS) * ((g.ny + H - 1) / H);
 }
 
 void launch_rhs_lpw(hipStream_t st, const KernelOpts &o, const double *psi, const double *S, const double *qforc, const double *wind, double *dq,
                     const NatGeom &g, int nl, int walls, int uniformS, const double *Su, int have_qforc, double D, double beta, double iRe, double iRe4,
                     double cs, double cb, double slip_c, const LayerCoef &lc, const double *q_in, double *q_out, double dt, int stoch,
-                    const double *q_stage, const double *noise, double crelax, double dts, int region, const double *dt_ptr) {
+                    const double *q_stage, const double *noise, double crelax, double dts, int region, const double *dt_ptr, const RhsResid *rr) {
   LpwArgs a;
+  const bool res = rr != nullptr;
+  if (res && (stoch || !q_out || region || (g.nx & 1) || (g.ny & 1) || !rr->res_c)) {
+    fprintf(stderr, "msom: launch_rhs_lpw: the residual by-product needs the plain tendency + advance pass on one tile with even sides\n");
+    abort();
+  }
+  if (res) {
+    a.rr = *rr;
+    (void)hipMemsetAsync(rr->res_max, 0, sizeof(double), st);
+  } else {
+    a.rr.res = a.rr.res_c = a.rr.res_max = a.rr.bsum_partial = nullptr;
+    a.rr.sg = SplitGeom(); a.rr.cg = SplitGeom();
+  }
   a.region = region;
   a.dt_ptr = dt_ptr;
   a.q_stage = q_stage; a.noise = noise; a.crelax = crelax; a.dts = dts;
@@ -307,19 +422,8 @@
   a.D = D; a.beta = beta; a.iRe = iRe; a.iRe4 = iRe4; a.cs = cs; a.cb = cb; a.slip_c = slip_c; a.lc = lc;
   for (int l = 0; l < MSOM_MAXNL; l++) a.Su[l] = Su ? Su[l] : 0.;
   const int strips = (g.nx + LPW_W - 1) / LPW_W;
-  int H = o.rhs_dbg >> 8;
-  a.NS = LPW_MAXW / nl < 1 ? 1 : LPW_MAXW / nl;
-  if (a.NS > strips) a.NS = strips;
-  if (H <= 0) {
-    const int ncu = device_cu_count();
-    const int wgx = (strips + a.NS - 1) / a.NS;
-    double best = -1.;
-    for (int h = 64; h >= 8; h -= 8) {
-      const double r = (double)wgx * ((g.ny + h - 1) / h) / ncu, cost = (r <= 3. ? ceil(r) : r + 0.5) * (h + 6);
-      if (best < 0. || cost < best) { best = cost; H = h; }
-    }
-  }
-  if (H < 8) H = 8;
+  int H;
+  lpw_shape(o, g, nl, res, a.NS, H);
   a.H = H;
   const dim3 gr((strips + a.NS - 1) / a.NS, (g.ny + H - 1) / H), bl(64 * nl * a.NS);
   if (stoch && !q_out) {
@@ -330,6 +434,7 @@
     with_bool(have_qforc, [&](auto Q) {
       constexpr bool UNI = decltype(U)::value, QF = decltype(Q)::value;
       if (stoch) hipLaunchKernelGGL((k_rhs_lpw<LPW_R, UNI, QF, true, true>), gr, bl, 0, st, a);
+      else if (res) hipLaunchKernelGGL((k_rhs_lpw<LPW_R_RES, UNI, QF, true, false, true>), gr, bl, 0, st, a);
       else if (q_out) hipLaunchKernelGGL((k_rhs_lpw<LPW_R, UNI, QF, true>), gr, bl, 0, st, a);
       else hipLaunchKernelGGL((k_rhs_lpw<LPW_R, UNI, QF, false>), gr, bl, 0, st, a);
     });
diff --git a/msom_amd/csrc/msom_api.hip b/msom_amd/csrc/msom_api.hip
--- a/msom_amd/csrc/msom_api.hip
+++ b/msom_amd/csrc/msom_api.hip
@@ -28,6 +28,7 @@
     }                                                                                      \
   } while (0)
 
+#define RHS_RESID_MIN 23
 enum { SC_BSUM = 2, SC_KE = 3, SC_SCRATCH = 4, SC_RES0 = 6, SC_RES1 = 7, SC_UMAX = 8 , SC_RESF = 8 + MSOM_MAXNL , SC_LSUM = 32 , SC_SPEC = 48 , SC_COUNT = 64 };
 static_assert(SC_RESF < SC_LSUM && SC_LSUM + MSOM_MAXNL <= SC_SPEC && SC_SPEC + 4 <= SC_COUNT, "scalar slots overlap");
 
@@ -134,7 +135,8 @@
   int mgc_lean = 0;
   int res_ready = -1;
   int adv_fused = 1;
-  int rhs_resid = 0;
+  int rhs_resid = -1;
+  int rr_nparts = 0;
   int bfn_begun = 0;
   int bfn_obs_set = 0, bfn_gain_set = 0;
   double *bfn_partial = nullptr;
@@ -511,7 +513,10 @@
   }
   HIPCHK(hipMalloc(&m->staging, (size_t)m->nl * (m->p.nptr > 1 ? m->p.nptr : 1) * m->nx * m->ny * sizeof(double)));
   HIPCHK(hipMalloc(&m->partial, ((size_t)partial_count(m->g) * m->nl + 64) * sizeof(double)));
-  HIPCHK(hipMalloc(&m->partial_rr, ((size_t)rhs_pipe_blocks(m->g) + 64) * sizeof(double)));
+  {
+    const size_t lpw = (size_t)((m->g.nx + 57) / 58) * ((m->g.ny + 7) / 8), pipe = (size_t)rhs_pipe_blocks(m->g);
+    HIPCHK(hipMalloc(&m->partial_rr, ((lpw > pipe ? lpw : pipe) + 64) * sizeof(double)));
+  }
   {
     size_t nb = (size_t)rhs_fused_blocks(m->g);
     if (nb < 2048) nb = 2048;
@@ -708,6 +713,7 @@
   return nullptr;
 }
 extern "C" int msom_set_option(msom_t *m, const char *key, double v) {
+  if (m) m->res_ready = -1;
   if (!m || !key) return MSOM_ERR_ARG;
   if (m->model) return nq_set_option(m, key, v);
   clear_graphs(m);
@@ -805,6 +811,7 @@
 static bool fine_visit_fused(const msom *m);
 static int level_path(const msom *m, int k);
 static bool restrict2_ok(const msom *m);
+static bool rhs_resid_emits(const msom *m);
 extern "C" double msom_get_param(msom_t *m, const char *key) {
   if (!m || !key) return NAN;
   if (!strcmp(key, "model")) return m->model;
@@ -849,6 +856,10 @@
   if (!strcmp(key, "resmax_marching")) return m->uniformS && m->nl <= MSOM_FASTNL && m->g.nx >= 64 && m->g.ny >= 16 && m->opt.resmax_rows >= 0;
   if (!strcmp(key, "march_visit_ring")) return !fine_visit_fused(m) ? -1 : (m->opt.march_visit_ring >= 2 ? 2 : (m->opt.march_visit_ring == 1 ? 1 : 0));
   if (const int *o = kernel_opt(m->opt, key)) return *o;
+  if (!strcmp(key, "rhs_resid")) return rhs_resid_emits(m);
+  if (!strncmp(key, "split_ls_", 9)) { const int k = atoi(key + 9); return k >= 0 && k < m->nlev ? (double)m->sg[k].ls : NAN; }
+  if (!strncmp(key, "split_rp_", 9)) { const int k = atoi(key + 9); return k >= 0 && k < m->nlev ? (double)m->sg[k].rp : NAN; }
+  if (!strcmp(key, "split_pad")) return MSOM_SP;
   if (!strcmp(key, "restrict2")) return restrict2_ok(m);
   if (!strcmp(key, "mg_coarse_lean")) return m->mgc_first >= 0 && m->mgc_lean;
   if (!strcmp(key, "march_levels")) return march_levels(m);
@@ -1125,6 +1136,7 @@
 }
 
 extern "C" int msom_set_const(msom_t *m) {
+  if (m) m->res_ready = -1;
   if (!m) return MSOM_ERR_ARG;
   if (m->model) return nq_set_const(m);
   m->s_zero = 0;
@@ -1185,6 +1197,14 @@
 
 enum { RP_COLOUR = 0, RP_BLOCK2 = 1, RP_BLOCK8 = 2, RP_MARCH = 3, RP_COARSE = 4, RP_GATHERED = 8 };
 static bool layered_fusions(const msom *m) { return !m->mode_pv_invert; }
+static bool rhs_resid_on(const msom *m) {
+  return m->rhs_resid > 0 || (m->rhs_resid < 0 && m->rhs_variant == 6 && (size_t)m->g.nx * m->g.ny * m->nl >= ((size_t)1 << RHS_RESID_MIN));
+}
+static bool rhs_resid_emits(const msom *m) {
+  return rhs_resid_on(m) && m->fused && m->adv_fused && m->nl <= MSOM_FASTNL && !m->have_pg && !m->have_zpg && !m->flag_topo && !m->stochastic &&
+         layered_fusions(m) && (m->rhs_variant == 1 || m->rhs_variant == 6) && m->mg_fused && m->nlev > 1 && m->bc != BC_PERIODIC && m->nranks == 1 &&
+         !(m->g.nx & 1) && !(m->g.ny & 1);
+}
 static int sweep_path(const msom *m, const Lev &L) {
   const SplitGeom &g = *L.sg;
   if (!layered_fusions(m)) return RP_COLOUR;
@@ -1548,7 +1568,7 @@
   m->res_ready = -1;
   if (have_res) {
     HIPCHK(hipMemcpyAsync(m->d_scal + SC_RES0, m->d_scal + SC_RESF, sizeof(double), hipMemcpyDeviceToDevice, m->st));
-    launch_sum_final(m->st, m->partial_rr, m->d_scal + SC_BSUM, rhs_pipe_blocks(m->g));
+    launch_sum_final(m->st, m->partial_rr, m->d_scal + SC_BSUM, m->rr_nparts);
   } else if (fused) {
     residual2(m, 2 | 4, b, SC_RES0, 1);
     launch_sum_final(m->st, m->partial, m->d_scal + SC_BSUM, residual2_blocks(m->g));
@@ -1824,14 +1844,14 @@
 #ifdef MSOM_STRICT
   const bool stoch_fused = false;
 #else
-  const bool stoch_fused = m->stochastic && m->stoch_fused && m->adv_fused && adv_out >= 0 && m->rhs_variant == 6 && !m->rhs_resid;
+  const bool stoch_fused = m->stochastic && m->stoch_fused && m->adv_fused && adv_out >= 0 && m->rhs_variant == 6;
 #endif
   if (m->fused && m->nl <= MSOM_FASTNL && !m->have_pg && !m->have_zpg && !m->flag_topo && (!m->stochastic || stoch_fused) &&
       (m->nranks == 1 || (m->nx >= 4 && m->ny >= 4))) {
     if (m->bc == BC_PERIODIC && m->nranks == 1) launch_fill_periodic(m->st, m->f[MSOM_PSI], m->g, nl, 3);
     if (!m->adv_fused) adv_out = -1;
-    const int variant = (m->rhs_resid && m->rhs_variant == 6) ? 1 : m->rhs_variant;
-    const bool use_rr = adv_out >= 0 && layered_fusions(m) && m->rhs_resid && variant == 1 && m->mg_fused && m->nlev > 1 && m->bc != BC_PERIODIC;
+    const int variant = m->rhs_variant;
+    const bool use_rr = adv_out >= 0 && rhs_resid_emits(m);
     RhsResid rr;
     if (use_rr) {
       rr.res = m->res[0]; rr.res_c = m->res[1]; rr.res_max = m->d_scal + SC_RESF; rr.bsum_partial = m->partial_rr;
@@ -1875,7 +1895,10 @@
                        variant == 6 ? m->dt_dev : nullptr);
     });
     prof_end(m, m->prof_rhs);
-    if (use_rr) m->res_ready = adv_out;
+    if (use_rr) {
+      m->res_ready = adv_out;
+      m->rr_nparts = variant == 6 ? rhs_lpw_blocks(m->opt, m->g, nl) : rhs_pipe_blocks(m->g);
+    }
     if (advanced && adv_out >= 0) *advanced = 1;
     return MSOM_OK;
   }
@@ -2029,6 +2052,7 @@
   } while (0)
 
 extern "C" double msom_update(msom_t *m, const double *q, double *dqdt, double dtmax) {
+  if (m) m->res_ready = -1;
   if (!m) return -1;
   if (m->model) return nq_update(m, q, dqdt, dtmax);
   if (!m->const_set && msom_set_const(m)) return -1;
@@ -2044,6 +2068,7 @@
 }
 
 extern "C" int msom_advance(msom_t *m, double *qout, const double *qin, const double *dqdt, double dt) {
+  if (m) m->res_ready = -1;
   if (m && m->model) return nq_advance(m, qout, qin, dqdt, dt);
   NEED_CONST(m);
   int in = MSOM_Q, out = MSOM_Q, r;
@@ -2058,6 +2083,7 @@
 }
 
 extern "C" int msom_invertq(msom_t *m, const double *q, double *psi, msom_mgstats *st) {
+  if (m) m->res_ready = -1;
   if (m && m->model) return nq_invertq(m, q, psi, st);
   NEED_CONST(m);
   int qf = MSOM_Q, r;
@@ -2073,6 +2099,7 @@
 }
 
 extern "C" int msom_comp_q(msom_t *m, const double *psi, double *q) {
+  if (m) m->res_ready = -1;
   if (m && m->model) return nq_comp_q_api(m, psi, q);
   NEED_CONST(m);
   int r;
@@ -2109,6 +2136,7 @@
 
 extern "C" int pystep_bfn(msom_t *m, double *varin_py, int len1, int len2, int len3, double *tend_py, int len4, int len5, int len6,
                           double direction, int vartype) {
+  if (m) m->res_ready = -1;
   MSQG_ONLY(m);
   NEED_CONST(m);
   if (check_shape(m, len1, len2, len3) || check_shape(m, len4, len5, len6)) return MSOM_ERR_ARG;
@@ -2137,12 +2165,14 @@
   NEED_CONST(m);
   if (check_shape(m, len7, len8, len9) || check_shape(m, len10, len11, len12)) return MSOM_ERR_ARG;
   int r;
+  m->res_ready = -1;
   HIPCHK(hipMemsetAsync(m->f[MSOM_PSI], 0, m->g.ls * m->nl * sizeof(double), m->st));
   if ((r = upload(m, MSOM_Q, qo_py))) return r;
   if ((r = invertq(m, m->f[MSOM_Q]))) return r;
   return download(m, MSOM_PSI, po_py);
 }
 extern "C" int pyp2q(msom_t *m, double *po_py, int len13, int len14, int len15, double *qo_py, int len16, int len17, int len18) {
+  if (m) m->res_ready = -1;
   MSQG_ONLY(m);
   NEED_CONST(m);
   if (check_shape(m, len13, len14, len15) || check_shape(m, len16, len17, len18)) return MSOM_ERR_ARG;
@@ -2152,6 +2182,7 @@
 
 static int ensure_field(msom *m, int field);
 extern "C" int msom_bfn_begin(msom_t *m) {
+  if (m) m->res_ready = -1;
   MSQG_ONLY(m);
   NEED_CONST(m);
   int r;
@@ -2256,6 +2287,7 @@
 }
 
 extern "C" int msom_stats_accumulate(msom_t *m, double w) {
+  if (m) m->res_ready = -1;
   MSQG_ONLY(m);
   if (!m) return MSOM_ERR_ARG;
   if (!std::isfinite(w)) { msom_set_error("msom_stats_accumulate: w = %g", w); return MSOM_ERR_ARG; }
@@ -2305,6 +2337,7 @@
 }
 
 extern "C" int msom_time_filter(msom_t *m, double dt) {
+  if (m) m->res_ready = -1;
   MSQG_ONLY(m);
   if (!m) return MSOM_ERR_ARG;
   if (!std::isfinite(dt)) { msom_set_error("msom_time_filter: dt = %g", dt); return MSOM_ERR_ARG; }
@@ -2346,6 +2379,7 @@
   } while (0)
 
 extern "C" int msom_modes_compute(msom_t *m) {
+  if (m) m->res_ready = -1;
   MSQG_ONLY(m);
   NEED_CONST(m);
   const int nl = m->nl, na = nl * nl + nl;
@@ -2407,6 +2441,7 @@
 }
 
 extern "C" int msom_modes_project(msom_t *m, int to_modes, const double *in, double *out) {
+  if (m) m->res_ready = -1;
   MSQG_ONLY(m);
   if (!m || !in || !out) return MSOM_ERR_ARG;
   NEED_MODES(m, "msom_modes_project");
@@ -2445,6 +2480,7 @@
 }
 
 extern "C" int msom_modes_set_rd(msom_t *m, int mode) {
+  if (m) m->res_ready = -1;
   MSQG_ONLY(m);
   if (!m || mode < 1 || mode > m->nl - 1) return MSOM_ERR_ARG;
   NEED_MODES(m, "msom_modes_set_rd");
@@ -2705,7 +2741,7 @@
 }
 
 static bool spec_ok(msom *m) {
-  return layered_fusions(m) && m->async_solve && m->nranks == 1 && m->fused && m->adv_fused && m->rhs_variant == 6 && !m->rhs_resid && m->mg_fused && m->nlev > 1 &&
+  return layered_fusions(m) && m->async_solve && m->nranks == 1 && m->fused && m->adv_fused && m->rhs_variant == 6 && m->mg_fused && m->nlev > 1 &&
          m->nl <= MSOM_FASTNL && !m->have_pg && !m->have_zpg && !m->flag_topo && !m->stochastic && m->p.nptr == 0 && m->p.nitermin >= 1 && !m->dbg_nosync;
 }
 
@@ -2736,6 +2772,7 @@
   m->spec_hook = nullptr;
   const bool hit1 = spec && m->spec_valid && !spec_rc;
   m->dt_dev = nullptr;
+  if (!hit1) m->res_ready = -1;
   if (d < 0) return m->sticky ? m->sticky : MSOM_ERR_HIP;
   if (hit1) {
     m->dt = m->h_scal[SC_SPEC + 1];
@@ -2773,8 +2810,12 @@
   const double d2 = solve_and_dt(m, MSOM_QPRED, m->dt);
   m->spec_hook = nullptr;
   if (d2 < 0) return m->sticky ? m->sticky : MSOM_ERR_HIP;
-  if (spec && m->spec_valid && !spec_rc) std::swap(m->f[MSOM_Q], m->q_alt);
-  else {
+  const bool rr2 = m->res_ready == MSOM_Q;
+  m->res_ready = -1;
+  if (spec && m->spec_valid && !spec_rc) {
+    std::swap(m->f[MSOM_Q], m->q_alt);
+    if (rr2) m->res_ready = MSOM_Q;
+  } else {
     if ((r = rhs_terms(m, MSOM_QPRED, MSOM_DQ, 1, p.iRe, p.iRe4, p.Eks, p.Ekb, MSOM_Q, MSOM_Q, m->dt, &advanced))) return r;
     if (!advanced && (r = advance_qg(m, MSOM_Q, MSOM_Q, MSOM_DQ, m->dt))) return r;
   }
@@ -3365,6 +3406,7 @@
   return m->sticky;
 }
 extern "C" int msom_energy_tend(msom_t *m, double dt) {
+  if (m) m->res_ready = -1;
   MSQG_ONLY(m);
   NEED_CONST(m);
   int r;
@@ -3384,6 +3426,7 @@
   return sync_stream(m);
 }
 extern "C" int msom_filter_de(msom_t *m, int pm_field, double dtflt) {
+  if (m) m->res_ready = -1;
   MSQG_ONLY(m);
   NEED_CONST(m);
   if (pm_field < 0 || pm_field >= MSOM_NFIELDS || m->flayers[pm_field] != m->nl) { msom_set_error("bad field id %d", pm_field); return MSOM_ERR_ARG; }
@@ -3402,6 +3445,7 @@
                          double *de_vd_py, int len7, int len8, int len9, double *de_j1_py, int len10, int len11, int len12,
                          double *de_j2_py, int len13, int len14, int len15, double *de_j3_py, int len16, int len17, int len18,
                          double *de_ft_py, int len19, int len20, int len21, int onlyKE) {
+  if (m) m->res_ready = -1;
   MSQG_ONLY(m);
   NEED_CONST(m);
   if (check_shape(m, len1, len2, len3) || check_shape(m, len4, len5, len6) || check_shape(m, len7, len8, len9) || check_shape(m, len10, len11, len12) ||
@@ -3500,6 +3544,7 @@
   return msom_bas_write(path, h.data(), m->flayers[field], m->gnx, m->p.L0) ? MSOM_ERR_IO : MSOM_OK;
 }
 extern "C" int msom_read_bas(msom_t *m, int field, const char *path) {
+  if (m) m->res_ready = -1;
   MSQG_ONLY(m);
   if (check_field(m, field) || !path) return MSOM_ERR_ARG;
   if (m->gnx != m->gny) { msom_set_error(".bas input needs a square grid"); return MSOM_ERR_STATE; }
@@ -3521,6 +3566,7 @@
   return msom_nc_append(path, m->nl, m->gny, m->gnx, 2, names, m->t, f) < 0 ? MSOM_ERR_IO : MSOM_OK;
 }
 extern "C" int msom_read_nc(msom_t *m, int field, const char *path, const char *varname, int record) {
+  if (m) m->res_ready = -1;
   if (check_field(m, field) || !path || !varname) return MSOM_ERR_ARG;
   std::vector<double> h((size_t)m->flayers[field] * m->gnx * m->gny);
   int r = msom_nc_read(path, varname, record, m->flayers[field], m->gny, m->gnx, h.data(), nullptr);
@@ -3534,6 +3580,7 @@
 }
 
 extern "C" int msom_read_inputs(msom_t *m, const char *dir) {
+  if (m) m->res_ready = -1;
   MSQG_ONLY(m);
   if (!m) return MSOM_ERR_ARG;
   char name[512];
@@ -3785,6 +3832,40 @@
   }
   m->profile = prof;
   return split_download(m, m->da[lev], m->sg[lev], da, m->nl);
+}
+extern "C" int msom_dbg_rhs_resid(msom_t *m, int fused, double dt, double *res0, double *res1, double *maxres, double *bsum) {
+  MSQG_ONLY(m);
+  if (m) m->res_ready = -1;
+  NEED_CONST(m);
+  if (!res0 || !res1 || m->nlev < 2) return MSOM_ERR_ARG;
+  const Params &p = m->p;
+  for (int k = 0; k < 2; k++) HIPCHK(hipMemsetAsync(m->res[k], 0xFF, m->sg[k].ls * m->nl * sizeof(double), m->st));
+  HIPCHK(hipMemsetAsync(m->d_scal, 0, (SC_UMAX + MSOM_MAXNL) * sizeof(double), m->st));
+  const int keep = m->rhs_resid;
+  m->rhs_resid = fused ? 1 : 0;
+  int adv = 0;
+  int r = rhs_terms(m, MSOM_Q, MSOM_DQ, 1, p.iRe, p.iRe4, p.Eks, p.Ekb, MSOM_QPRED, MSOM_Q, dt, &adv);
+  m->rhs_resid = keep;
+  if (r) return r;
+  const bool emitted = m->res_ready == MSOM_QPRED;
+  m->res_ready = -1;
+  if (!adv || (fused && !emitted)) { msom_set_error("msom_dbg_rhs_resid: this handle's tendency pass does not %s", adv ? "emit the residual" : "advance"); return MSOM_ERR_CONFIG; }
+  int slot = SC_RESF;
+  if (fused) launch_sum_final(m->st, m->partial_rr, m->d_scal + SC_BSUM, m->rr_nparts);
+  else {
+    residual2(m, 2 | 4, m->f[MSOM_QPRED], SC_RES0, 1);
+    launch_sum_final(m->st, m->partial, m->d_scal + SC_BSUM, residual2_blocks(m->g));
+    slot = SC_RES0;
+  }
+  double h[2] = {0., 0.};
+  HIPCHK(hipMemcpyAsync(&h[0], m->d_scal + slot, sizeof(double), hipMemcpyDeviceToHost, m->st));
+  HIPCHK(hipMemcpyAsync(&h[1], m->d_scal + SC_BSUM, sizeof(double), hipMemcpyDeviceToHost, m->st));
+  HIPCHK(hipMemcpyAsync(res0, m->res[0], m->sg[0].ls * m->nl * sizeof(double), hipMemcpyDeviceToHost, m->st));
+  HIPCHK(hipMemcpyAsync(res1, m->res[1], m->sg[1].ls * m->nl * sizeof(double), hipMemcpyDeviceToHost, m->st));
+  if ((r = sync_stream(m))) return r;
+  if (maxres) *maxres = h[0];
+  if (bsum) *bsum = h[1];
+  return MSOM_OK;
 }
 extern "C" int msom_dbg_residual(msom_t *m, const double *a, const double *b, double *res, double *maxres) {
   MSQG_ONLY(m);
```

Measured after the change: 18.87 billion grid-point-updates/s (median of 6 runs). 7.0% higher.
